# yahoo/TensorFlowOnSpark

Hardware: AMD Instinct MI355X
Metric: images/sec (whole node) ResNet-50 sync-SGD InputMode.SPARK (higher is better)
Workload: dtype bf16; 1 GPU; model=resnet50, global_batch=1024, per_gpu_batch=1024, parallelism=dp1

## Files before the change

csrc/bindings.cpp:

```cpp
#include <torch/extension.h>
#include <c10/hip/HIPStream.h>
#include <hip/hip_runtime.h>
#include <climits>

extern "C" {
int tfosr_bn_fast_blocks(long, int, int, int);
void tfosr_bn_apply_dual(const void*, const void*, void*, unsigned char*,
                         const float*, const float*, const float*, const float*,
                         const float*, const float*, const float*, const float*,
                         int, long, int, hipStream_t);
void tfosr_bn_bwd_stats_dual(const void*, const void*, const void*,
                             const unsigned char*, const float*, const float*,
                             const float*, const float*, float*, int, int, long,
                             int, hipStream_t);
void tfosr_bn_bwd_merge_dual(const float*, int, float*, float*, float*, float*,
                             int, hipStream_t);
void tfosr_bn_bwd_dx_dual(const void*, const void*, const void*,
                          const unsigned char*, void*, void*, const float*,
                          const float*, const float*, const float*, const float*,
                          const float*, const float*, const float*, const float*,
                          int, long, int, hipStream_t);
void tfosr_bn_stats(const void*, int, int, float*, int, int, int, long, hipStream_t);
void tfosr_bn_finalize(const float*, int, const void*, int, int, long,
                       float*, float*, float*, float*,
                       long, int, float, float, hipStream_t);
void tfosr_bn_apply(const void*, const void*, void*, unsigned char*,
                    const float*, const float*,
                    const float*, const float*, int, int, int, long, int, long,
                    hipStream_t);
void tfosr_bn_bwd_stats(const void*, const void*, const void*,
                        const unsigned char*, void*,
                        const float*, const float*, float*, int, int, int,
                        int, int, int, long, hipStream_t);
void tfosr_bn_bwd_merge(const float*, int, float*, float*, int, hipStream_t);
void tfosr_bn_bwd_dx(const void*, const void*, const void*,
                     const unsigned char*, const float*,
                     const float*, const float*, const float*, const float*,
                     void*, int, int, int, long, int, long, hipStream_t);
int tfosr_xent_dense_grid(int, int, long, long, int, int);
void tfosr_xent_dense_fwd(int, const void*, const long*, float*, float*, float*,
                          int*, int, long, long, int, long, float, int,
                          hipStream_t);
void tfosr_xent_dense_finalize(const float*, const int*, int, int, float*, int*,
                               hipStream_t);
void tfosr_xent_dense_bwd(int, const void*, const float*, const long*,
                          const float*, const float*, const int*, int, void*,
                          int, long, long, int, long, float, int, hipStream_t);
void tfosr_nhwc_pack(const void*, void*, const float*, const float*, float, int,
                     int, long, int, long, hipStream_t);
void tfosr_sgd_step(float*, const float*, float*, float, float, float, int, long,
                    hipStream_t);
void tfosr_adam_step(float*, const float*, float*, float*, float, float, float,
                     float, float, int, int, long, hipStream_t);
void tfosr_gemm_bt(const void*, const void*, void*, int, int, int, int,
                   hipStream_t);
void tfosr_gemm_bt_acc(const void*, const void*, void*, int, int, int, int,
                       int, hipStream_t);
void tfosr_mfma_probe(const short*, const short*, float*, hipStream_t);
void tfosr_maxpool_fwd(const void*, void*, unsigned char*, int, int, int, int,
                       int, int, int, int, int, int, hipStream_t);
void tfosr_maxpool_bwd(const void*, const unsigned char*, void*, int, int, int,
                       int, int, int, int, int, int, int, hipStream_t);
void tfosr_conv3x3(const void*, const void*, const void*, void*, int, int, int,
                   int, int, int, int, int, int, int, hipStream_t);
void tfosr_conv_mfma(const void*, const void*, const void*, void*, int, int,
                     int, int, int, int, int, int, int, int, int, int, int,
                     int, int, hipStream_t);
void tfosr_conv_wrw(const void*, const void*, float*, int, int, int, int, int,
                    int, int, int, int, int, hipStream_t);
int tfosr_wrw2_split(int, int, long);
void tfosr_conv_wrw2(const void*, const void*, const void*, float*, float*,
                     int, int, int, int, int, int, int, int, int, int, int,
                     int, int, hipStream_t);
void tfosr_conv_stem(const void*, const void*, const void*, void*, int, int,
                     int, int, int, int, hipStream_t);
void tfosr_conv_par(const void*, const void*, const void*, void*, int, int,
                    int, int, int, int, int, int, int, unsigned long, int,
                    int, int, long, int, hipStream_t);
void tfosr_pack_bf16(const void*, const void*, int, void*, long, hipStream_t);
}

namespace tfosr {
uint32_t crc32c(const uint8_t*, size_t, uint32_t);
struct ScanResult {
  std::string buffer;
  std::vector<std::pair<size_t, size_t>> records;
};
ScanResult scan_file(const std::string&, bool);
void write_file(const std::string&, const std::vector<std::string>&, bool);
}

namespace {

hipStream_t cur_stream() {
  return c10::hip::getCurrentHIPStream().stream();
}

struct BNLayout {
  bool nhwc;
  int N, C;
  long HW;
};

BNLayout bn_layout(const at::Tensor& x) {
  TORCH_CHECK(x.dim() == 4, "expected 4-D NCHW tensor");
  BNLayout l;
  l.N = x.size(0);
  l.C = x.size(1);
  l.HW = (long)x.size(2) * x.size(3);
  if (x.is_contiguous(at::MemoryFormat::ChannelsLast)) {
    l.nhwc = true;
  } else {
    TORCH_CHECK(x.is_contiguous(), "input must be contiguous (NCHW or channels_last)");
    l.nhwc = false;
  }
  return l;
}

int dtype_flag(const at::Tensor& x) {
  TORCH_CHECK(x.is_cuda(), "bn: input must be a GPU tensor");
  if (x.scalar_type() == at::kBFloat16) return 1;
  TORCH_CHECK(x.scalar_type() == at::kFloat, "expected float32 or bfloat16");
  return 0;
}


void bn_check_channel_vec(const at::Tensor& t, const at::Tensor& x, int C,
                          const char* name) {
  TORCH_CHECK(t.device() == x.device(), "bn: ", name, " must be on ", x.device(),
              ", got ", t.device());
  TORCH_CHECK(t.scalar_type() == at::kFloat, "bn: ", name, " must be float32");
  TORCH_CHECK(t.dim() == 1 && t.size(0) == C, "bn: ", name,
              " must have shape [", C, "]");
  TORCH_CHECK(t.is_contiguous(), "bn: ", name, " must be contiguous");
}

void bn_check_like(const at::Tensor& t, const at::Tensor& x, bool nhwc,
                   bool same_layout, const char* name) {
  TORCH_CHECK(t.device() == x.device(), "bn: ", name, " must be on ", x.device(),
              ", got ", t.device());
  TORCH_CHECK(t.scalar_type() == x.scalar_type(), "bn: ", name,
              " must have the input's dtype");
  TORCH_CHECK(t.sizes() == x.sizes(), "bn: ", name,
              " must have the input's shape");
  if (same_layout) {
    TORCH_CHECK(nhwc ? t.is_contiguous(at::MemoryFormat::ChannelsLast)
                     : t.is_contiguous(),
                "bn: ", name, " must have the input's memory layout");
  }
}

std::vector<at::Tensor> bn_fwd_train(at::Tensor x, c10::optional<at::Tensor> res,
                                     at::Tensor w, at::Tensor b, at::Tensor rm,
                                     at::Tensor rv, double momentum, double eps,
                                     bool relu) {
  auto l = bn_layout(x);
  int bf = dtype_flag(x);
  const void* res_ptr = nullptr;
  if (res.has_value()) {
    bn_check_like(*res, x, l.nhwc, true, "res");
    res_ptr = res->data_ptr();
  }
  bn_check_channel_vec(w, x, l.C, "weight");
  bn_check_channel_vec(b, x, l.C, "bias");
  bn_check_channel_vec(rm, x, l.C, "running_mean");
  bn_check_channel_vec(rv, x, l.C, "running_var");
  auto opts = x.options().dtype(at::kFloat);
  long M = (long)l.N * l.HW;
  int nb = tfosr_bn_fast_blocks(M * l.C, l.C, bf, l.nhwc);
  auto ws = nb > 0 ? at::empty({(long)nb * 2 * l.C}, opts)
                   : at::zeros({2L * l.C}, opts);
  auto save_mean = at::empty({l.C}, opts);
  auto save_rstd = at::empty({l.C}, opts);
  auto y = at::empty_like(x);
  at::Tensor mask;
  unsigned char* mask_ptr = nullptr;
  if (relu && nb > 0) {
    long nvec = M * l.C / (bf ? 8 : 4);
    mask = at::empty({nvec}, x.options().dtype(at::kByte));
    mask_ptr = mask.data_ptr<unsigned char>();
  } else {
    mask = at::empty({0}, x.options().dtype(at::kByte));
  }
  auto s = cur_stream();
  tfosr_bn_stats(x.data_ptr(), bf, l.nhwc, ws.data_ptr<float>(), nb,
                 l.N, l.C, l.HW, s);
  tfosr_bn_finalize(ws.data_ptr<float>(), nb, x.data_ptr(), bf, l.nhwc, l.HW,
                    save_mean.data_ptr<float>(), save_rstd.data_ptr<float>(),
                    rm.data_ptr<float>(), rv.data_ptr<float>(), M, l.C,
                    (float)momentum, (float)eps, s);
  tfosr_bn_apply(x.data_ptr(), res_ptr, y.data_ptr(), mask_ptr,
                 save_mean.data_ptr<float>(),
                 save_rstd.data_ptr<float>(), w.data_ptr<float>(),
                 b.data_ptr<float>(), bf, l.nhwc, relu, M * l.C, l.C, l.HW, s);
  return {y, save_mean, save_rstd, mask};
}

at::Tensor bn_fwd_eval(at::Tensor x, c10::optional<at::Tensor> res, at::Tensor w,
                       at::Tensor b, at::Tensor rm, at::Tensor rv, double eps,
                       bool relu) {
  auto l = bn_layout(x);
  int bf = dtype_flag(x);
  const void* res_ptr = nullptr;
  if (res.has_value()) {
    bn_check_like(*res, x, l.nhwc, true, "res");
    res_ptr = res->data_ptr();
  }
  bn_check_channel_vec(w, x, l.C, "weight");
  bn_check_channel_vec(b, x, l.C, "bias");
  bn_check_channel_vec(rm, x, l.C, "running_mean");
  bn_check_channel_vec(rv, x, l.C, "running_var");
  auto rstd = at::rsqrt(rv + eps);
  auto y = at::empty_like(x);
  tfosr_bn_apply(x.data_ptr(), res_ptr, y.data_ptr(), nullptr,
                 rm.data_ptr<float>(),
                 rstd.data_ptr<float>(), w.data_ptr<float>(), b.data_ptr<float>(),
                 bf, l.nhwc, relu, (long)l.N * l.HW * l.C, l.C, l.HW,
                 cur_stream());
  return y;
}

std::vector<at::Tensor> bn_bwd(at::Tensor x, at::Tensor dy, at::Tensor y,
                               at::Tensor mask, at::Tensor w,
                               at::Tensor save_mean,
                               at::Tensor save_rstd, bool relu, bool grad_res) {
  auto l = bn_layout(x);
  int bf = dtype_flag(x);
  bn_check_like(dy, x, l.nhwc, false, "dy");
  bn_check_like(y, x, l.nhwc, true, "y");
  bn_check_channel_vec(w, x, l.C, "weight");
  bn_check_channel_vec(save_mean, x, l.C, "save_mean");
  bn_check_channel_vec(save_rstd, x, l.C, "save_rstd");
  dy = l.nhwc ? dy.contiguous(at::MemoryFormat::ChannelsLast) : dy.contiguous();
  auto opts = x.options().dtype(at::kFloat);
  long total = (long)l.N * l.HW * l.C;
  int nb = tfosr_bn_fast_blocks(total, l.C, bf, l.nhwc);
  auto ws = nb > 0 ? at::empty({(long)nb * 2 * l.C}, opts)
                   : at::zeros({2L * l.C}, opts);
  auto dg = at::empty({l.C}, opts);
  auto db = at::empty({l.C}, opts);
  auto dx = at::empty_like(x);
  at::Tensor gout;
  void* gout_ptr = nullptr;
  if (grad_res) {
    gout = at::empty_like(x);
    gout_ptr = gout.data_ptr();
  }
  auto s = cur_stream();
  const unsigned char* mask_ptr =
      mask.numel() ? mask.data_ptr<unsigned char>() : nullptr;
  TORCH_CHECK(!(relu && nb > 0) || mask_ptr != nullptr,
              "fast-path relu backward requires the forward bitmask");
  if (relu && nb > 0) {
    TORCH_CHECK(mask.device() == x.device() && mask.scalar_type() == at::kByte &&
                    mask.is_contiguous() && mask.numel() == total / (bf ? 8 : 4),
                "bn: mask must be the contiguous uint8 bitmask bn_fwd_train "
                "returned for this input");
  }
  tfosr_bn_bwd_stats(x.data_ptr(), dy.data_ptr(), y.data_ptr(), mask_ptr,
                     gout_ptr,
                     save_mean.data_ptr<float>(), save_rstd.data_ptr<float>(),
                     ws.data_ptr<float>(), nb, bf, l.nhwc,
                     relu, l.N, l.C, l.HW, s);
  tfosr_bn_bwd_merge(ws.data_ptr<float>(), nb, dg.data_ptr<float>(),
                     db.data_ptr<float>(), l.C, s);
  if (grad_res) {
    tfosr_bn_bwd_dx(x.data_ptr(), gout.data_ptr(), y.data_ptr(), nullptr,
                    save_mean.data_ptr<float>(), save_rstd.data_ptr<float>(),
                    w.data_ptr<float>(), dg.data_ptr<float>(), db.data_ptr<float>(),
                    dx.data_ptr(), bf, l.nhwc, 0, total, l.C, l.HW, s);
    return {dx, dg, db, gout};
  }
  tfosr_bn_bwd_dx(x.data_ptr(), dy.data_ptr(), y.data_ptr(), mask_ptr,
                  save_mean.data_ptr<float>(), save_rstd.data_ptr<float>(),
                  w.data_ptr<float>(), dg.data_ptr<float>(), db.data_ptr<float>(),
                  dx.data_ptr(), bf, l.nhwc, relu, total, l.C, l.HW, s);
  return {dx, dg, db};
}

bool bn_dual_eligible(const at::Tensor& xa, const at::Tensor& xb) {
  if (!xa.is_cuda() || !xb.is_cuda() || xa.dim() != 4) return false;
  if (xa.scalar_type() != at::kBFloat16 && xa.scalar_type() != at::kFloat)
    return false;
  if (xb.scalar_type() != xa.scalar_type() || xb.device() != xa.device() ||
      xb.sizes() != xa.sizes())
    return false;
  if (!xa.is_contiguous(at::MemoryFormat::ChannelsLast) ||
      !xb.is_contiguous(at::MemoryFormat::ChannelsLast))
    return false;
  return tfosr_bn_fast_blocks(xa.numel(), (int)xa.size(1),
                              xa.scalar_type() == at::kBFloat16, 1) > 0;
}

std::vector<at::Tensor> bn_dual_fwd_train(
    at::Tensor xa, at::Tensor xb, at::Tensor w_a, at::Tensor b_a,
    at::Tensor rm_a, at::Tensor rv_a, at::Tensor w_b, at::Tensor b_b,
    at::Tensor rm_b, at::Tensor rv_b, double momentum, double eps) {
  TORCH_CHECK(bn_dual_eligible(xa, xb),
              "bn_dual: needs two same-shape channels_last GPU tensors on the "
              "NHWC fast path");
  auto l = bn_layout(xa);
  int bf = dtype_flag(xa);
  const at::Tensor* vecs[] = {&w_a, &b_a, &rm_a, &rv_a, &w_b, &b_b, &rm_b, &rv_b};
  for (auto* t : vecs) bn_check_channel_vec(*t, xa, l.C, "per-channel vector");
  auto opts = xa.options().dtype(at::kFloat);
  long M = (long)l.N * l.HW;
  long total = M * l.C;
  int nb = tfosr_bn_fast_blocks(total, l.C, bf, 1);
  auto ws = at::empty({(long)nb * 2 * l.C}, opts);
  auto mean_a = at::empty({l.C}, opts), rstd_a = at::empty({l.C}, opts);
  auto mean_b = at::empty({l.C}, opts), rstd_b = at::empty({l.C}, opts);
  auto y = at::empty_like(xa);
  auto mask = at::empty({total / (bf ? 8 : 4)}, xa.options().dtype(at::kByte));
  auto s = cur_stream();
  auto f = [](at::Tensor& t) { return t.data_ptr<float>(); };
  tfosr_bn_stats(xa.data_ptr(), bf, 1, f(ws), nb, l.N, l.C, l.HW, s);
  tfosr_bn_finalize(f(ws), nb, xa.data_ptr(), bf, 1, l.HW, f(mean_a), f(rstd_a),
                    f(rm_a), f(rv_a), M, l.C, (float)momentum, (float)eps, s);
  tfosr_bn_stats(xb.data_ptr(), bf, 1, f(ws), nb, l.N, l.C, l.HW, s);
  tfosr_bn_finalize(f(ws), nb, xb.data_ptr(), bf, 1, l.HW, f(mean_b), f(rstd_b),
                    f(rm_b), f(rv_b), M, l.C, (float)momentum, (float)eps, s);
  tfosr_bn_apply_dual(xa.data_ptr(), xb.data_ptr(), y.data_ptr(),
                      mask.data_ptr<unsigned char>(), f(mean_a), f(rstd_a),
                      f(w_a), f(b_a), f(mean_b), f(rstd_b), f(w_b), f(b_b), bf,
                      total, l.C, s);
  return {y, mean_a, rstd_a, mean_b, rstd_b, mask};
}

std::vector<at::Tensor> bn_dual_bwd(at::Tensor xa, at::Tensor xb, at::Tensor dy,
                                    at::Tensor mask, at::Tensor w_a,
                                    at::Tensor mean_a, at::Tensor rstd_a,
                                    at::Tensor w_b, at::Tensor mean_b,
                                    at::Tensor rstd_b) {
  TORCH_CHECK(bn_dual_eligible(xa, xb),
              "bn_dual: needs two same-shape channels_last GPU tensors on the "
              "NHWC fast path");
  auto l = bn_layout(xa);
  int bf = dtype_flag(xa);
  bn_check_like(dy, xa, true, false, "dy");
  dy = dy.contiguous(at::MemoryFormat::ChannelsLast);
  const at::Tensor* vecs[] = {&w_a, &mean_a, &rstd_a, &w_b, &mean_b, &rstd_b};
  for (auto* t : vecs) bn_check_channel_vec(*t, xa, l.C, "per-channel vector");
  long total = (long)l.N * l.HW * l.C;
  TORCH_CHECK(mask.device() == xa.device() && mask.scalar_type() == at::kByte &&
                  mask.is_contiguous() && mask.numel() == total / (bf ? 8 : 4),
              "bn_dual: mask must be the contiguous uint8 bitmask "
              "bn_dual_fwd_train returned for these inputs");
  auto opts = xa.options().dtype(at::kFloat);
  int nb = tfosr_bn_fast_blocks(total, l.C, bf, 1);
  auto ws = at::empty({(long)nb * 3 * l.C}, opts);
  auto dg_a = at::empty({l.C}, opts), dg_b = at::empty({l.C}, opts);
  auto db_a = at::empty({l.C}, opts), db_b = at::empty({l.C}, opts);
  auto dxa = at::empty_like(xa), dxb = at::empty_like(xb);
  auto s = cur_stream();
  auto f = [](at::Tensor& t) { return t.data_ptr<float>(); };
  const unsigned char* mask_ptr = mask.data_ptr<unsigned char>();
  tfosr_bn_bwd_stats_dual(xa.data_ptr(), xb.data_ptr(), dy.data_ptr(), mask_ptr,
                          f(mean_a), f(rstd_a), f(mean_b), f(rstd_b), f(ws), nb,
                          bf, total, l.C, s);
  tfosr_bn_bwd_merge_dual(f(ws), nb, f(dg_a), f(dg_b), f(db_a), f(db_b), l.C, s);
  tfosr_bn_bwd_dx_dual(xa.data_ptr(), xb.data_ptr(), dy.data_ptr(), mask_ptr,
                       dxa.data_ptr(), dxb.data_ptr(), f(mean_a), f(rstd_a),
                       f(w_a), f(dg_a), f(mean_b), f(rstd_b), f(w_b), f(dg_b),
                       f(db_a), bf, total, l.C, s);
  return {dxa, dxb, dg_a, dg_b, db_a, db_b};
}

void bn_stage(int family, at::Tensor x, c10::optional<at::Tensor> other,
              c10::optional<at::Tensor> out, c10::optional<at::Tensor> mask,
              at::Tensor ws, std::vector<at::Tensor> p, bool relu) {
  auto l = bn_layout(x);
  int bf = dtype_flag(x);
  long total = (long)l.N * l.HW * l.C;
  int nb = tfosr_bn_fast_blocks(total, l.C, bf, l.nhwc);
  TORCH_CHECK(nb > 0, "bn_stage: shape is not on the NHWC fast path");
  const size_t need[4] = {0, 4, 2, 5};
  TORCH_CHECK(family >= 0 && family < 4, "bn_stage: family must be 0..3");
  TORCH_CHECK(p.size() == need[family], "bn_stage: family ", family, " takes ",
              need[family], " per-channel vectors");
  for (auto& t : p) bn_check_channel_vec(t, x, l.C, "per-channel vector");
  TORCH_CHECK(ws.device() == x.device() && ws.scalar_type() == at::kFloat &&
                  ws.is_contiguous() && ws.numel() >= (long)nb * 2 * l.C,
              "bn_stage: ws must hold bn_fast_blocks() * 2C floats");
  const void* other_ptr = nullptr;
  if (other.has_value()) {
    bn_check_like(*other, x, l.nhwc, true, "other");
    other_ptr = other->data_ptr();
  }
  void* out_ptr = nullptr;
  if (out.has_value()) {
    bn_check_like(*out, x, l.nhwc, true, "out");
    out_ptr = out->data_ptr();
  }
  unsigned char* mask_ptr = nullptr;
  if (mask.has_value()) {
    TORCH_CHECK(mask->device() == x.device() && mask->scalar_type() == at::kByte &&
                    mask->is_contiguous() && mask->numel() == total / (bf ? 8 : 4),
                "bn_stage: mask must be a contiguous uint8 tensor, one byte "
                "per 16 B vector");
    mask_ptr = mask->data_ptr<unsigned char>();
  }
  if (family != 0 && family != 1)
    TORCH_CHECK(other_ptr != nullptr, "bn_stage: dy is required");
  if (family == 1 || family == 3)
    TORCH_CHECK(out_ptr != nullptr, "bn_stage: out is required");
  if (family >= 2)
    TORCH_CHECK(!relu || mask_ptr != nullptr, "bn_stage: relu needs the mask");
  auto f = [&](size_t i) { return p[i].data_ptr<float>(); };
  auto s = cur_stream();
  switch (family) {
    case 0:
      tfosr_bn_stats(x.data_ptr(), bf, 1, ws.data_ptr<float>(), nb, l.N, l.C,
                     l.HW, s);
      break;
    case 1:
      tfosr_bn_apply(x.data_ptr(), other_ptr, out_ptr, mask_ptr, f(0), f(1),
                     f(2), f(3), bf, 1, relu, total, l.C, l.HW, s);
      break;
    case 2:
      tfosr_bn_bwd_stats(x.data_ptr(), other_ptr, nullptr, mask_ptr, out_ptr,
                         f(0), f(1), ws.data_ptr<float>(), nb, bf, 1, relu,
                         l.N, l.C, l.HW, s);
      break;
    default:
      tfosr_bn_bwd_dx(x.data_ptr(), other_ptr, nullptr, mask_ptr, f(0), f(1),
                      f(2), f(3), f(4), out_ptr, bf, 1, relu, total, l.C, l.HW,
                      s);
  }
}


enum { XENT_ROWS = 0, XENT_STRIDED = 1, XENT_TILE = 2 };
enum { XENT_NONE = 0, XENT_SUM = 1, XENT_MEAN = 2 };

struct XentLayout {
  int family;
  long P, S;
  int C;
};

XentLayout xent_layout(const at::Tensor& logits, const at::Tensor& target) {
  TORCH_CHECK(logits.is_cuda(), "xent: logits must be a GPU tensor");
  TORCH_CHECK(logits.scalar_type() == at::kFloat ||
                  logits.scalar_type() == at::kBFloat16,
              "xent: logits must be float32 or bfloat16");
  TORCH_CHECK(logits.dim() >= 2, "xent: logits must be (P, C) or (N, C, d1, ...)");
  TORCH_CHECK(target.device() == logits.device(),
              "xent: target must be on ", logits.device());
  TORCH_CHECK(target.scalar_type() == at::kLong, "xent: target must be int64");
  TORCH_CHECK(target.is_contiguous(), "xent: target must be contiguous");
  TORCH_CHECK(target.dim() == logits.dim() - 1 &&
                  target.size(0) == logits.size(0),
              "xent: target must have the logits' shape without the class dim");
  for (int64_t d = 2; d < logits.dim(); ++d)
    TORCH_CHECK(target.size(d - 1) == logits.size(d),
                "xent: target must have the logits' shape without the class dim");
  TORCH_CHECK(logits.size(1) >= 1 && logits.size(1) < (1L << 24),
              "xent: bad class count");
  XentLayout l;
  l.C = (int)logits.size(1);
  l.P = target.numel();
  l.S = 1;
  bool rows;
  if (logits.dim() == 2) {
    TORCH_CHECK(logits.is_contiguous(), "xent: 2-D logits must be contiguous");
    rows = true;
  } else if (logits.is_contiguous()) {
    rows = false;
    for (int64_t d = 2; d < logits.dim(); ++d) l.S *= logits.size(d);
  } else {
    TORCH_CHECK(logits.dim() == 4 &&
                    logits.is_contiguous(at::MemoryFormat::ChannelsLast),
                "xent: N-D logits must be contiguous or 4-D channels_last");
    rows = true;
  }
  l.family = rows ? (l.C >= 64 ? XENT_ROWS : XENT_TILE) : XENT_STRIDED;
  return l;
}

void xent_check_rowvec(const at::Tensor& t, const at::Tensor& logits, long P,
                       const char* name) {
  TORCH_CHECK(t.device() == logits.device() && t.scalar_type() == at::kFloat &&
                  t.is_contiguous() && t.numel() == P,
              "xent: ", name, " must be contiguous float32 with one value per "
              "row, on the logits' device");
}

std::vector<at::Tensor> xent_dense_fwd(at::Tensor logits, at::Tensor target,
                                       long ignore_index, double label_smoothing,
                                       long reduction, long max_grid) {
  auto l = xent_layout(logits, target);
  TORCH_CHECK(reduction >= XENT_NONE && reduction <= XENT_MEAN,
              "xent: reduction must be 0 (none), 1 (sum) or 2 (mean)");
  TORCH_CHECK(label_smoothing >= 0.0 && label_smoothing <= 1.0,
              "xent: label_smoothing must be in [0, 1]");
  TORCH_CHECK(max_grid >= 0, "xent: max_grid must be >= 0");
  int bf = dtype_flag(logits);
  auto fopts = logits.options().dtype(at::kFloat);
  auto iopts = logits.options().dtype(at::kInt);
  auto lse = at::empty({l.P}, fopts);
  auto s = cur_stream();
  if (reduction == XENT_NONE) {
    auto loss = at::empty(target.sizes(), fopts);
    tfosr_xent_dense_fwd(l.family, logits.data_ptr(), target.data_ptr<long>(),
                         loss.data_ptr<float>(), lse.data_ptr<float>(), nullptr,
                         nullptr, bf, l.P, l.S, l.C, ignore_index,
                         (float)label_smoothing, (int)max_grid, s);
    return {loss, lse, at::empty({0}, iopts)};
  }
  auto loss = at::zeros({}, fopts);
  auto nvalid = at::zeros({1}, iopts);
  if (l.P > 0) {
    int nb = tfosr_xent_dense_grid(l.family, bf, l.P, l.S, l.C, (int)max_grid);
    auto part_loss = at::empty({2L * nb}, fopts);
    auto part_cnt = at::empty({nb}, iopts);
    tfosr_xent_dense_fwd(l.family, logits.data_ptr(), target.data_ptr<long>(),
                         nullptr, lse.data_ptr<float>(),
                         part_loss.data_ptr<float>(), part_cnt.data_ptr<int>(),
                         bf, l.P, l.S, l.C, ignore_index,
                         (float)label_smoothing, (int)max_grid, s);
    tfosr_xent_dense_finalize(part_loss.data_ptr<float>(),
                              part_cnt.data_ptr<int>(), nb,
                              reduction == XENT_MEAN, loss.data_ptr<float>(),
                              nvalid.data_ptr<int>(), s);
  }
  return {loss, lse, nvalid};
}

at::Tensor xent_dense_bwd(at::Tensor logits, at::Tensor lse, at::Tensor target,
                          at::Tensor gout, c10::optional<at::Tensor> nvalid,
                          long ignore_index, double label_smoothing,
                          long reduction, long max_grid) {
  auto l = xent_layout(logits, target);
  TORCH_CHECK(reduction >= XENT_NONE && reduction <= XENT_MEAN,
              "xent: reduction must be 0 (none), 1 (sum) or 2 (mean)");
  TORCH_CHECK(max_grid >= 0, "xent: max_grid must be >= 0");
  int bf = dtype_flag(logits);
  xent_check_rowvec(lse, logits, l.P, "lse");
  const float* grows = nullptr;
  const float* gscalar = nullptr;
  const int* nv = nullptr;
  if (reduction == XENT_NONE) {
    xent_check_rowvec(gout, logits, l.P, "gout");
    grows = gout.data_ptr<float>();
  } else {
    TORCH_CHECK(gout.device() == logits.device() &&
                    gout.scalar_type() == at::kFloat && gout.numel() == 1,
                "xent: gout must be a one-element float32 device tensor");
    TORCH_CHECK(nvalid.has_value() && nvalid->device() == logits.device() &&
                    nvalid->scalar_type() == at::kInt && nvalid->numel() == 1,
                "xent: n_valid must be the int32[1] tensor the forward returned");
    gscalar = gout.data_ptr<float>();
    nv = nvalid->data_ptr<int>();
  }
  auto dlogits = at::empty_like(logits);
  tfosr_xent_dense_bwd(l.family, logits.data_ptr(), lse.data_ptr<float>(),
                       target.data_ptr<long>(), grows, gscalar, nv,
                       reduction == XENT_MEAN, dlogits.data_ptr(), bf, l.P, l.S,
                       l.C, ignore_index, (float)label_smoothing, (int)max_grid,
                       cur_stream());
  return dlogits;
}

std::vector<at::Tensor> softmax_xent_fwd(at::Tensor logits, at::Tensor target) {
  TORCH_CHECK(logits.dim() == 2 && logits.is_contiguous());
  TORCH_CHECK(target.scalar_type() == at::kLong && target.is_cuda() &&
              target.is_contiguous() && target.numel() == logits.size(0));
  long N = logits.size(0);
  int C = logits.size(1);
  auto opts = logits.options().dtype(at::kFloat);
  auto loss = at::empty({N}, opts);
  auto lse = at::empty({N}, opts);
  tfosr_xent_dense_fwd(XENT_ROWS, logits.data_ptr(), target.data_ptr<long>(),
                       loss.data_ptr<float>(), lse.data_ptr<float>(), nullptr,
                       nullptr, dtype_flag(logits), N, 1, C, -100, 0.f, 0,
                       cur_stream());
  return {loss, lse};
}

at::Tensor softmax_xent_bwd(at::Tensor logits, at::Tensor lse, at::Tensor target,
                            at::Tensor gout) {
  TORCH_CHECK(logits.dim() == 2 && logits.is_contiguous());
  TORCH_CHECK(target.scalar_type() == at::kLong && target.is_cuda() &&
              target.is_contiguous() && target.numel() == logits.size(0));
  long N = logits.size(0);
  int C = logits.size(1);
  gout = gout.contiguous();
  xent_check_rowvec(lse, logits, N, "lse");
  xent_check_rowvec(gout, logits, N, "gout");
  auto dlogits = at::empty_like(logits);
  tfosr_xent_dense_bwd(XENT_ROWS, logits.data_ptr(), lse.data_ptr<float>(),
                       target.data_ptr<long>(), gout.data_ptr<float>(), nullptr,
                       nullptr, 0, dlogits.data_ptr(), dtype_flag(logits), N, 1,
                       C, -100, 0.f, 0, cur_stream());
  return dlogits;
}

at::Tensor nhwc_pack(at::Tensor x, at::Tensor mean, at::Tensor std_, double scale,
                     bool out_bf16, bool channels_last) {
  TORCH_CHECK(x.dim() == 4 && x.scalar_type() == at::kByte && x.is_contiguous(),
              "nhwc_pack expects contiguous uint8 NHWC");
  TORCH_CHECK(x.is_cuda(), "nhwc_pack: images must be on the GPU");
  for (int d = 0; d < 4; ++d)
    TORCH_CHECK(x.size(d) <= INT_MAX, "nhwc_pack: dimension ", d, " too large");
  int N = x.size(0), H = x.size(1), W = x.size(2), C = x.size(3);
  long HW = (long)H * W;
  auto check_stat = [&](const at::Tensor& t, const char* name) {
    TORCH_CHECK(t.scalar_type() == at::kFloat && t.is_contiguous() &&
                    t.device() == x.device() && t.numel() == C,
                "nhwc_pack: ", name, " must be a contiguous fp32 tensor of C = ",
                C, " elements on the images' device");
  };
  check_stat(mean, "mean");
  check_stat(std_, "std");
  auto opts = x.options().dtype(out_bf16 ? at::kBFloat16 : at::kFloat);
  at::Tensor out;
  if (channels_last) {
    out = at::empty({N, C, H, W}, opts, at::MemoryFormat::ChannelsLast);
  } else {
    out = at::empty({N, C, H, W}, opts);
  }
  tfosr_nhwc_pack(x.data_ptr(), out.data_ptr(), mean.data_ptr<float>(),
                  std_.data_ptr<float>(), (float)scale, out_bf16, channels_last,
                  (long)N * C * HW, C, HW, cur_stream());
  return out;
}

void check_flat_state(const char* op, const at::Tensor& p,
                      std::initializer_list<const at::Tensor*> others) {
  TORCH_CHECK(p.is_cuda() && p.scalar_type() == at::kFloat && p.is_contiguous(),
              op, " expects contiguous fp32 params on the GPU");
  for (const at::Tensor* t : others)
    TORCH_CHECK(t->scalar_type() == at::kFloat && t->is_contiguous() &&
                    t->device() == p.device() && t->numel() == p.numel(),
                op, ": every tensor must be contiguous fp32 with the params' ",
                p.numel(), " elements on the params' device");
}

std::pair<long, long> check_pool_geometry(const char* op, const at::Tensor& t,
                                          long C, long N, long H, long W,
                                          long K, long S, long P) {
  TORCH_CHECK(t.is_cuda(), op, " expects a GPU tensor");
  TORCH_CHECK(t.scalar_type() == at::kBFloat16 || t.scalar_type() == at::kFloat,
              op, " expects bf16 or fp32");
  const long V = t.scalar_type() == at::kBFloat16 ? 8 : 4;
  TORCH_CHECK(C >= V && C % V == 0, op, ": C must be a multiple of ", V,
              " for this dtype, got ", C);
  TORCH_CHECK(K >= 1 && S >= 1 && K * K <= 256, op,
              ": need K >= 1, S >= 1 and K*K <= 256 (the saved tap index is "
              "one byte), got K=", K, " S=", S);
  TORCH_CHECK(P >= 0 && P <= K / 2, op, ": need 0 <= P <= K/2, got P=", P);
  TORCH_CHECK(N >= 0 && H >= 1 && W >= 1 && H <= INT_MAX && W <= INT_MAX &&
              N <= INT_MAX && C <= INT_MAX && S <= INT_MAX,
              op, ": empty or oversized dimension");
  TORCH_CHECK(H + 2 * P >= K && W + 2 * P >= K, op,
              ": the window does not fit the padded input");
  const long OH = (H + 2 * P - K) / S + 1, OW = (W + 2 * P - K) / S + 1;
  const long limit = 0xFFFFFFFFL - 2048L * 256L;
  auto fits = [&](long h, long w) {
    long n = N;
    for (long f : {h, w, C / V}) {
      if (n > limit / f) return false;
      n *= f;
    }
    return true;
  };
  TORCH_CHECK(fits(H, W) && fits(OH, OW), op,
              ": tensor too large for the kernels' 32-bit thread index");
  return {OH, OW};
}

void sgd_step(at::Tensor p, at::Tensor g, at::Tensor m, double lr, double mu,
              double wd, bool nesterov) {
  check_flat_state("sgd_step", p, {&g, &m});
  tfosr_sgd_step(p.data_ptr<float>(), g.data_ptr<float>(), m.data_ptr<float>(),
                 (float)lr, (float)mu, (float)wd, nesterov, p.numel(),
                 cur_stream());
}

at::Tensor gemm_bt(at::Tensor a, at::Tensor b, bool out_bf16) {
  TORCH_CHECK(a.dim() == 2 && b.dim() == 2 && a.size(1) == b.size(1),
              "gemm_bt: A[M,K], B[N,K]");
  TORCH_CHECK(a.scalar_type() == at::kBFloat16 && b.scalar_type() == at::kBFloat16);
  int M = a.size(0), N = b.size(0), K = a.size(1);
  if (K % 32 != 0) {
    int Kp = (K + 31) / 32 * 32;
    auto ap = at::zeros({M, Kp}, a.options());
    auto bp = at::zeros({N, Kp}, b.options());
    ap.narrow(1, 0, K).copy_(a);
    bp.narrow(1, 0, K).copy_(b);
    a = ap; b = bp; K = Kp;
  }
  a = a.contiguous();
  b = b.contiguous();
  auto out = at::empty({M, N}, a.options().dtype(out_bf16 ? at::kBFloat16
                                                          : at::kFloat));
  tfosr_gemm_bt(a.data_ptr(), b.data_ptr(), out.data_ptr(), out_bf16, M, N, K,
                cur_stream());
  return out;
}

at::Tensor gemm_bf16(at::Tensor a, at::Tensor b) {
  return gemm_bt(a, b.t().contiguous(), false);
}

at::Tensor mfma_probe(at::Tensor a, at::Tensor b) {
  TORCH_CHECK(a.sizes() == at::IntArrayRef({64, 8}) &&
              b.sizes() == at::IntArrayRef({64, 8}));
  auto c = at::empty({64, 4}, a.options().dtype(at::kFloat));
  tfosr_mfma_probe(a.contiguous().data_ptr<short>(),
                   b.contiguous().data_ptr<short>(), c.data_ptr<float>(),
                   cur_stream());
  return c;
}

}

#define TFOSR_API_VERSION 6

static constexpr long kMaxTapReach = 1L << 20;

PYBIND11_MODULE(TORCH_EXTENSION_NAME, m) {
  m.def("api_version", []() { return TFOSR_API_VERSION; });
  m.def("bn_fwd_train", &bn_fwd_train);
  m.def("bn_fwd_eval", &bn_fwd_eval);
  m.def("bn_bwd", &bn_bwd);
  m.def("bn_dual_eligible", &bn_dual_eligible);
  m.def("bn_dual_fwd_train", &bn_dual_fwd_train);
  m.def("bn_dual_bwd", &bn_dual_bwd);
  m.def("bn_fast_blocks", [](long total, int C, bool bf16, bool nhwc) {
    return tfosr_bn_fast_blocks(total, C, bf16, nhwc);
  });
  m.def("bn_stage", &bn_stage);
  m.def("softmax_xent_fwd", &softmax_xent_fwd);
  m.def("softmax_xent_bwd", &softmax_xent_bwd);
  m.def("xent_dense_fwd", &xent_dense_fwd, py::arg("logits"), py::arg("target"),
        py::arg("ignore_index") = -100, py::arg("label_smoothing") = 0.0,
        py::arg("reduction") = 0, py::arg("max_grid") = 0);
  m.def("xent_dense_bwd", &xent_dense_bwd, py::arg("logits"), py::arg("lse"),
        py::arg("target"), py::arg("gout"), py::arg("nvalid") = py::none(),
        py::arg("ignore_index") = -100, py::arg("label_smoothing") = 0.0,
        py::arg("reduction") = 0, py::arg("max_grid") = 0);
  m.def("nhwc_pack", &nhwc_pack);
  m.def("sgd_step", &sgd_step);
  m.def("adam_step", [](at::Tensor p, at::Tensor g, at::Tensor m, at::Tensor v,
                        double lr, double b1, double b2, double eps, double wd,
                        long step, bool decoupled) {
    check_flat_state("adam_step", p, {&g, &m, &v});
    TORCH_CHECK(step >= 1 && step <= INT_MAX,
                "adam_step: step counts from 1, got ", step);
    tfosr_adam_step(p.data_ptr<float>(), g.data_ptr<float>(),
                    m.data_ptr<float>(), v.data_ptr<float>(), lr, b1, b2, eps,
                    wd, (int)step, decoupled, p.numel(), cur_stream());
  });
  m.def("gemm_bt", &gemm_bt, py::arg("a"), py::arg("b"), py::arg("out_bf16") = false);
  m.def("gemm_bf16", &gemm_bf16);
  m.def("mfma_probe", &mfma_probe);
  m.def("maxpool_fwd", [](at::Tensor x, long K, long S, long P) {
    TORCH_CHECK(x.dim() == 4 && x.is_contiguous(at::MemoryFormat::ChannelsLast),
                "maxpool_fwd expects channels_last");
    auto ohw = check_pool_geometry("maxpool_fwd", x, x.size(1), x.size(0),
                                   x.size(2), x.size(3), K, S, P);
    int N = x.size(0), C = x.size(1), H = x.size(2), W = x.size(3);
    int OH = (int)ohw.first, OW = (int)ohw.second;
    auto y = at::empty({N, C, OH, OW}, x.options(),
                       at::MemoryFormat::ChannelsLast);
    auto idx = at::empty({N, OH, OW, C}, x.options().dtype(at::kByte));
    tfosr_maxpool_fwd(x.data_ptr(), y.data_ptr(), idx.data_ptr<unsigned char>(),
                      x.scalar_type() == at::kBFloat16, N, C, H, W, OH, OW,
                      K, S, P, cur_stream());
    return std::vector<at::Tensor>{y, idx};
  });
  m.def("conv3x3_fwd", [](at::Tensor x, at::Tensor w9, long Cout, long S,
                          long P) {
    TORCH_CHECK(x.dim() == 4 && x.is_contiguous(at::MemoryFormat::ChannelsLast),
                "conv3x3_fwd expects channels_last input");
    TORCH_CHECK(x.scalar_type() == at::kBFloat16 &&
                w9.scalar_type() == at::kBFloat16);
    int N = x.size(0), Cin = x.size(1), H = x.size(2), W = x.size(3);
    TORCH_CHECK(Cin % 32 == 0, "conv3x3 requires Cin % 32 == 0");
    TORCH_CHECK(w9.size(1) == 9 * Cin);
    int OH = (H + 2 * P - 3) / S + 1, OW = (W + 2 * P - 3) / S + 1;
    auto y = at::empty({N, Cout, OH, OW}, x.options(),
                       at::MemoryFormat::ChannelsLast);
    auto guard = at::zeros({64}, x.options());
    tfosr_conv3x3(x.data_ptr(), w9.contiguous().data_ptr(), guard.data_ptr(),
                  y.data_ptr(), 1, N, H, W, Cin, Cout, OH, OW,
                  S, P, cur_stream());
    return y;
  });
  m.def("conv_mfma", [](at::Tensor x, at::Tensor wk, long Cout, long fh,
                        long fw, long S, long P, long D, long OH, long OW,
                        long fd, bool out_f32) {
    TORCH_CHECK(x.dim() == 4 && x.is_contiguous(at::MemoryFormat::ChannelsLast),
                "conv_mfma expects channels_last input");
    TORCH_CHECK(x.scalar_type() == at::kBFloat16 &&
                wk.scalar_type() == at::kBFloat16);
    TORCH_CHECK(fh >= 1 && fw >= 1 && fh * fw <= 49, "bad filter dims");
    TORCH_CHECK(D == 1 || D == 2, "input dilation must be 1 or 2");
    TORCH_CHECK(fd >= 1, "conv_mfma: filter dilation fd must be >= 1, got ",
                fd);
    TORCH_CHECK(fd == 1 || D == 1,
                "conv_mfma: filter dilation fd > 1 requires input dilation "
                "D == 1");
    TORCH_CHECK(fd <= kMaxTapReach && fd * (fh - 1) <= kMaxTapReach &&
                    fd * (fw - 1) <= kMaxTapReach,
                "conv_mfma: fd, fd*(fh-1) and fd*(fw-1) must be <= ",
                kMaxTapReach);
    long taps = fh * fw;
    int N = x.size(0), Cin = x.size(1), H = x.size(2), W = x.size(3);
    TORCH_CHECK(Cin % 32 == 0, "conv_mfma requires Cin % 32 == 0");
    TORCH_CHECK(wk.size(1) == taps * Cin);
    if (OH < 0) {
      long HV = (H - 1) * D + 1, WV = (W - 1) * D + 1;
      long nh = HV + 2 * P - fd * (fh - 1) - 1;
      long nw = WV + 2 * P - fd * (fw - 1) - 1;
      TORCH_CHECK(nh >= 0 && nw >= 0,
                  "conv_mfma: the dilated filter does not fit the padded "
                  "input");
      OH = nh / S + 1;
      OW = nw / S + 1;
    }
    auto y = at::empty({N, Cout, OH, OW},
                       x.options().dtype(out_f32 ? at::kFloat : at::kBFloat16),
                       at::MemoryFormat::ChannelsLast);
    auto guard = at::zeros({64}, x.options());
    tfosr_conv_mfma(x.data_ptr(), wk.contiguous().data_ptr(), guard.data_ptr(),
                    y.data_ptr(), out_f32 ? 0 : 1, N, H, W, Cin,
                    Cout, OH, OW, S, P, taps, fw, D, 0, (int)fd, cur_stream());
    return y;
  }, py::arg("x"), py::arg("wk"), py::arg("Cout"), py::arg("fh"),
     py::arg("fw"), py::arg("S"), py::arg("P"), py::arg("D"), py::arg("OH"),
     py::arg("OW"), py::arg("fd") = 1, py::arg("out_f32") = false);
  m.def("conv_mfma_acc", [](at::Tensor x, at::Tensor wk, at::Tensor out,
                            long fh, long fw, long S, long P, long D) {
    TORCH_CHECK(x.is_contiguous(at::MemoryFormat::ChannelsLast) &&
                out.is_contiguous(at::MemoryFormat::ChannelsLast));
    TORCH_CHECK(x.scalar_type() == at::kBFloat16 &&
                wk.scalar_type() == at::kBFloat16 &&
                out.scalar_type() == at::kBFloat16);
    int N = x.size(0), Cin = x.size(1), H = x.size(2), W = x.size(3);
    TORCH_CHECK(Cin % 32 == 0, "conv_mfma requires Cin % 32 == 0");
    long taps = fh * fw;
    TORCH_CHECK(wk.size(1) == taps * Cin);
    long Cout = out.size(1), OH = out.size(2), OW = out.size(3);
    TORCH_CHECK(out.size(0) == N);
    auto guard = at::zeros({64}, x.options());
    tfosr_conv_mfma(x.data_ptr(), wk.contiguous().data_ptr(), guard.data_ptr(),
                    out.data_ptr(), 1, N, H, W, Cin, Cout, OH, OW,
                    S, P, taps, fw, D, 1, 1, cur_stream());
    return out;
  });
  m.def("gemm_bt_acc", [](at::Tensor a, at::Tensor b, at::Tensor c) {
    TORCH_CHECK(a.dim() == 2 && b.dim() == 2 && c.dim() == 2,
                "gemm_bt_acc: A[M,K], B[N,K], C[M,N] must be 2-D");
    TORCH_CHECK(a.is_cuda(), "gemm_bt_acc: a must be a GPU tensor");
    TORCH_CHECK(b.device() == a.device() && c.device() == a.device(),
                "gemm_bt_acc: b and c must be on ", a.device());
    TORCH_CHECK(a.is_contiguous() && b.is_contiguous() && c.is_contiguous(),
                "gemm_bt_acc: a, b and c must be contiguous");
    TORCH_CHECK(a.scalar_type() == at::kBFloat16 &&
                    b.scalar_type() == at::kBFloat16 &&
                    c.scalar_type() == at::kBFloat16,
                "gemm_bt_acc: a, b and c must be bfloat16");
    long M = a.size(0), K = a.size(1), Nn = b.size(0);
    TORCH_CHECK(b.size(1) == K && c.size(0) == M && c.size(1) == Nn,
                "gemm_bt_acc: A[M,K], B[N,K], C[M,N]");
    TORCH_CHECK(K % 32 == 0, "gemm_bt_acc: K must be a multiple of 32");
    tfosr_gemm_bt_acc(a.data_ptr(), b.data_ptr(), c.data_ptr(),
                      1, M, Nn, K, 1, cur_stream());
    return c;
  });
  m.def("conv_wrw2", [](at::Tensor dy, at::Tensor x, long R, long S_f,
                        long stride, long P, long fd) {
    TORCH_CHECK(dy.is_contiguous(at::MemoryFormat::ChannelsLast) &&
                x.is_contiguous(at::MemoryFormat::ChannelsLast));
    TORCH_CHECK(dy.scalar_type() == at::kBFloat16 &&
                x.scalar_type() == at::kBFloat16);
    int N = x.size(0), Cin = x.size(1), H = x.size(2), W = x.size(3);
    int Cout = dy.size(1), OH = dy.size(2), OW = dy.size(3);
    TORCH_CHECK(Cin % 8 == 0 && Cout % 8 == 0,
                "conv_wrw2 needs channel counts % 8 == 0");
    long taps = R * S_f;
    TORCH_CHECK(taps == 1 || taps == 9, "conv_wrw2 supports 1x1 and 3x3");
    TORCH_CHECK(fd >= 1, "conv_wrw2: filter dilation fd must be >= 1, got ",
                fd);
    TORCH_CHECK(taps != 1 || fd == 1,
                "conv_wrw2: a 1x1 filter has no dilation, fd must be 1");
    TORCH_CHECK(fd <= kMaxTapReach && fd * (R - 1) <= kMaxTapReach &&
                    fd * (S_f - 1) <= kMaxTapReach,
                "conv_wrw2: fd, fd*(R-1) and fd*(S_f-1) must be <= ",
                kMaxTapReach);
    long M = (long)N * OH * OW;
    int split = tfosr_wrw2_split(Cout, Cin, M);
    long K = taps * (long)Cin;
    auto ws = at::empty({(long)split, (long)Cout * K},
                        x.options().dtype(at::kFloat));
    auto dW = at::empty({(long)Cout, K}, x.options().dtype(at::kFloat));
    auto guard = at::zeros({64}, x.options());
    tfosr_conv_wrw2(dy.data_ptr(), x.data_ptr(), guard.data_ptr(),
                    ws.data_ptr<float>(), dW.data_ptr<float>(), N, H, W, Cin,
                    Cout, OH, OW, R, S_f, stride, P, split, (int)fd,
                    cur_stream());
    return dW;
  }, py::arg("dy"), py::arg("x"), py::arg("R"), py::arg("S_f"),
     py::arg("stride"), py::arg("P"), py::arg("fd") = 1);
  m.def("pack_bf16", [](at::Tensor descs, at::Tensor cum, long ndesc,
                        at::Tensor arena, long total) {
    TORCH_CHECK(descs.is_cuda() && cum.is_cuda() && arena.is_cuda() &&
                    descs.device() == arena.device() &&
                    cum.device() == arena.device(),
                "pack_bf16 expects descs, cum and arena on one GPU");
    TORCH_CHECK(arena.scalar_type() == at::kBFloat16 && arena.is_contiguous(),
                "pack_bf16 expects a contiguous bf16 arena");
    TORCH_CHECK(ndesc >= 0 && ndesc <= INT_MAX, "pack_bf16: bad ndesc ", ndesc);
    TORCH_CHECK(descs.scalar_type() == at::kByte && descs.is_contiguous() &&
                    descs.numel() == ndesc * 80,
                "pack_bf16: descs must hold ndesc * 80 contiguous bytes");
    TORCH_CHECK(cum.scalar_type() == at::kLong && cum.is_contiguous() &&
                    cum.numel() == ndesc + 1,
                "pack_bf16: cum must hold ndesc + 1 contiguous int64");
    TORCH_CHECK(total >= 0 && arena.numel() >= total,
                "pack_bf16: arena holds ", arena.numel(), " elements, total is ",
                total);
    if (total == 0) return;
    TORCH_CHECK(ndesc >= 1, "pack_bf16: no descriptor for ", total, " elements");
    tfosr_pack_bf16(descs.data_ptr(), cum.data_ptr(), (int)ndesc,
                    arena.data_ptr(), total, cur_stream());
  });
  m.def("conv_par", [](at::Tensor x, at::Tensor wk, at::Tensor out,
                       std::vector<long> taps_r, std::vector<long> taps_s,
                       long P, bool accum) {
    TORCH_CHECK(x.is_contiguous(at::MemoryFormat::ChannelsLast) &&
                out.is_contiguous(at::MemoryFormat::ChannelsLast));
    TORCH_CHECK(x.scalar_type() == at::kBFloat16 &&
                wk.scalar_type() == at::kBFloat16 &&
                out.scalar_type() == at::kBFloat16);
    int N = x.size(0), Cin = x.size(1), H = x.size(2), W = x.size(3);
    TORCH_CHECK(Cin % 32 == 0);
    long ntaps = (long)taps_r.size();
    TORCH_CHECK(ntaps >= 1 && ntaps <= 8 && taps_s.size() == (size_t)ntaps);
    TORCH_CHECK(wk.size(1) == ntaps * Cin);
    long Cout = out.size(1), OHr = out.size(2), OWr = out.size(3);
    long oh0 = ((P - taps_r[0]) % 2 + 2) % 2;
    long ow0 = ((P - taps_s[0]) % 2 + 2) % 2;
    long OHs = (OHr - oh0 + 1) / 2, OWs = (OWr - ow0 + 1) / 2;
    if (OHs <= 0 || OWs <= 0) return out;
    unsigned long pack = 0;
    for (long i = 0; i < ntaps; ++i)
      pack |= ((unsigned long)((taps_r[i] << 4) | taps_s[i])) << (i * 8);
    auto guard = at::zeros({64}, x.options());
    tfosr_conv_par(x.data_ptr(), wk.contiguous().data_ptr(), guard.data_ptr(),
                   out.data_ptr(), N, H, W, Cin, (int)Cout, (int)OHs,
                   (int)OWs, (int)P, (int)ntaps, pack, (int)oh0, (int)ow0,
                   (int)OWr, OHr * OWr, accum ? 1 : 0, cur_stream());
    return out;
  });
  m.def("conv_stem", [](at::Tensor x4, at::Tensor w224, long Cout) {
    TORCH_CHECK(x4.is_contiguous(at::MemoryFormat::ChannelsLast) &&
                x4.size(1) == 4, "conv_stem expects NHWC4 padded input");
    TORCH_CHECK(x4.scalar_type() == at::kBFloat16 &&
                w224.scalar_type() == at::kBFloat16);
    TORCH_CHECK(w224.size(1) == 224);
    int N = x4.size(0), Hp = x4.size(2), Wp = x4.size(3);
    int OH = (Hp - 7) / 2 + 1, OW = (Wp - 7) / 2 + 1;
    auto y = at::empty({N, Cout, OH, OW}, x4.options(),
                       at::MemoryFormat::ChannelsLast);
    auto guard = at::zeros({64}, x4.options());
    tfosr_conv_stem(x4.data_ptr(), w224.contiguous().data_ptr(),
                    guard.data_ptr(), y.data_ptr(), N, Hp, Wp, Cout, OH, OW,
                    cur_stream());
    return y;
  });
  m.def("conv_stem_wrw", [](at::Tensor dy, at::Tensor x4) {
    TORCH_CHECK(dy.is_contiguous(at::MemoryFormat::ChannelsLast) &&
                x4.is_contiguous(at::MemoryFormat::ChannelsLast));
    TORCH_CHECK(dy.scalar_type() == at::kBFloat16 &&
                x4.scalar_type() == at::kBFloat16 && x4.size(1) == 4);
    int N = x4.size(0), Hp = x4.size(2), Wp = x4.size(3);
    int Cout = dy.size(1), OH = dy.size(2), OW = dy.size(3);
    long M = (long)N * OH * OW;
    int split = tfosr_wrw2_split(Cout, 32, M);
    long K = 7L * 32;
    auto ws = at::empty({(long)split, (long)Cout * K},
                        x4.options().dtype(at::kFloat));
    auto dW = at::empty({(long)Cout, K}, x4.options().dtype(at::kFloat));
    auto guard = at::zeros({64}, x4.options());
    tfosr_conv_wrw2(dy.data_ptr(), x4.data_ptr(), guard.data_ptr(),
                    ws.data_ptr<float>(), dW.data_ptr<float>(), N, Hp, Wp,
                    32, Cout, OH, OW, 7, 1,
                    2, 0, split, 1, cur_stream());
    return dW;
  });
  m.def("conv_wrw", [](at::Tensor dy, at::Tensor x, long R, long S, long P) {
    TORCH_CHECK(dy.is_contiguous(at::MemoryFormat::ChannelsLast) &&
                x.is_contiguous(at::MemoryFormat::ChannelsLast));
    TORCH_CHECK(dy.scalar_type() == at::kBFloat16 &&
                x.scalar_type() == at::kBFloat16);
    int N = x.size(0), Cin = x.size(1), H = x.size(2), W = x.size(3);
    int Cout = dy.size(1), OH = dy.size(2), OW = dy.size(3);
    auto dW = at::zeros({Cout, R * S * (long)Cin},
                        x.options().dtype(at::kFloat));
    tfosr_conv_wrw(dy.data_ptr(), x.data_ptr(), dW.data_ptr<float>(), N, H, W,
                   Cin, Cout, OH, OW, R, S, P, cur_stream());
    return dW;
  });
  m.def("maxpool_bwd", [](at::Tensor dy, at::Tensor idx, long H, long W,
                          long K, long S, long P) {
    TORCH_CHECK(dy.dim() == 4, "maxpool_bwd expects a 4-D gradient");
    auto ohw = check_pool_geometry("maxpool_bwd", dy, dy.size(1), dy.size(0),
                                   H, W, K, S, P);
    TORCH_CHECK(dy.size(2) == ohw.first && dy.size(3) == ohw.second,
                "maxpool_bwd: a ", H, "x", W, " input pooled with K=", K,
                " S=", S, " P=", P, " gives ", ohw.first, "x", ohw.second,
                ", the gradient is ", dy.size(2), "x", dy.size(3));
    TORCH_CHECK(idx.scalar_type() == at::kByte && idx.is_contiguous() &&
                    idx.device() == dy.device() && idx.dim() == 4 &&
                    idx.size(0) == dy.size(0) && idx.size(1) == dy.size(2) &&
                    idx.size(2) == dy.size(3) && idx.size(3) == dy.size(1),
                "maxpool_bwd: idx must be the contiguous uint8 (N, OH, OW, C) "
                "tensor maxpool_fwd returned, on the gradient's device");
    dy = dy.contiguous(at::MemoryFormat::ChannelsLast);
    int N = dy.size(0), C = dy.size(1), OH = dy.size(2), OW = dy.size(3);
    auto dx = at::empty({N, C, H, W}, dy.options(),
                        at::MemoryFormat::ChannelsLast);
    tfosr_maxpool_bwd(dy.data_ptr(), idx.data_ptr<unsigned char>(),
                      dx.data_ptr(), dy.scalar_type() == at::kBFloat16,
                      N, C, H, W, OH, OW, K, S, P, cur_stream());
    return dx;
  });

  m.def("crc32c", [](py::bytes data) {
    std::string s = data;
    return tfosr::crc32c((const uint8_t*)s.data(), s.size(), 0);
  });
  m.def("tfrecord_read_file", [](const std::string& path, bool verify) {
    auto res = tfosr::scan_file(path, verify);
    py::list out;
    for (auto& [off, len] : res.records)
      out.append(py::bytes(res.buffer.data() + off, len));
    return out;
  }, py::arg("path"), py::arg("verify") = false);
  m.def("tfrecord_write_file",
        [](const std::string& path, const std::vector<std::string>& recs,
           bool append) { tfosr::write_file(path, recs, append); },
        py::arg("path"), py::arg("records"), py::arg("append") = false);
}
```

csrc/bn_relu.hip:

```cpp
#include "tfosr_common.h"

typedef unsigned int u32;


template <typename T>
struct VecIO;

template <>
struct VecIO<bf16_t> {
  static constexpr int V = 8;
  using vec_t = s8v;
  __device__ static void load(const bf16_t* p, float* out) {
    vec_t v = *(const vec_t*)p;
    #pragma unroll
    for (int j = 0; j < 8; ++j) {
      union { short s; bf16_t b; } u;
      u.s = v[j];
      out[j] = (float)u.b;
    }
  }
  __device__ static void store(bf16_t* p, const float* in) {
    vec_t v;
    #pragma unroll
    for (int j = 0; j < 8; ++j) {
      union { short s; bf16_t b; } u;
      u.b = (bf16_t)in[j];
      v[j] = u.s;
    }
    *(vec_t*)p = v;
  }
};

template <>
struct VecIO<float> {
  static constexpr int V = 4;
  using vec_t = f4v;
  __device__ static void load(const float* p, float* out) {
    f4v v = *(const f4v*)p;
    #pragma unroll
    for (int j = 0; j < 4; ++j) out[j] = v[j];
  }
  __device__ static void store(float* p, const float* in) {
    f4v v;
    #pragma unroll
    for (int j = 0; j < 4; ++j) v[j] = in[j];
    *(f4v*)p = v;
  }
};


template <int V>
__device__ __forceinline__ u32 channel_slot(u32 C) {
  return ((blockIdx.x * blockDim.x + threadIdx.x) * (u32)V) % C;
}

#define TFOSR_BN_SHIFT_PIXELS 32

template <typename T>
__device__ __forceinline__ float channel_shift(const T* __restrict__ x, int c,
                                               int C, long HW, bool nhwc,
                                               int n) {
  float s = 0.f;
  for (int m = 0; m < n; ++m)
    s += (float)x[nhwc ? (long)m * C + c : ((m / HW) * C + c) * HW + m % HW];
  return s / (float)n;
}

template <typename T>
__global__ void stats_nhwc_fast(const T* __restrict__ x,
                                float* __restrict__ partials, u32 nvec, u32 C) {
  extern __shared__ float lds[];
  constexpr int V = VecIO<T>::V;
  const u32 c0 = channel_slot<V>(C);
  for (u32 i = threadIdx.x; i < 2 * C; i += blockDim.x) lds[i] = 0.f;
  __syncthreads();
  float s[V], q[V], v[V], k[V];
  VecIO<T>::load(x + c0, k);
  #pragma unroll
  for (int j = 0; j < V; ++j) { s[j] = 0.f; q[j] = 0.f; }
  const u32 stride = gridDim.x * blockDim.x;
  for (u32 i = blockIdx.x * blockDim.x + threadIdx.x; i < nvec; i += stride) {
    VecIO<T>::load(x + (size_t)i * V, v);
    #pragma unroll
    for (int j = 0; j < V; ++j) { float d = v[j] - k[j]; s[j] += d; q[j] += d * d; }
  }
  #pragma unroll
  for (int j = 0; j < V; ++j) {
    atomicAdd(&lds[c0 + j], s[j]);
    atomicAdd(&lds[C + c0 + j], q[j]);
  }
  __syncthreads();
  float* out = partials + (size_t)blockIdx.x * 2 * C;
  for (u32 i = threadIdx.x; i < 2 * C; i += blockDim.x) out[i] = lds[i];
}

__global__ void stats_merge_finalize(const float* __restrict__ partials,
                                     int nblocks, u32 C,
                                     const void* __restrict__ x, int is_bf16,
                                     int is_nhwc, long HW, int nshift,
                                     float* __restrict__ save_mean,
                                     float* __restrict__ save_rstd,
                                     float* __restrict__ running_mean,
                                     float* __restrict__ running_var,
                                     long M, float momentum, float eps) {
  __shared__ float scratch[8];
  const u32 c = blockIdx.x;
  float s = 0.f, q = 0.f;
  for (int b = threadIdx.x; b < nblocks; b += blockDim.x) {
    s += partials[(size_t)b * 2 * C + c];
    q += partials[(size_t)b * 2 * C + C + c];
  }
  s = block_sum<256>(s, scratch);
  __syncthreads();
  q = block_sum<256>(q, scratch);
  if (threadIdx.x != 0) return;
  const float shift =
      is_bf16 ? channel_shift((const bf16_t*)x, (int)c, (int)C, HW, is_nhwc, nshift)
              : channel_shift((const float*)x, (int)c, (int)C, HW, is_nhwc, nshift);
  float dmean = s / (float)M;
  float var = fmaxf(q / (float)M - dmean * dmean, 0.f);
  float mean = shift + dmean;
  save_mean[c] = mean;
  save_rstd[c] = rsqrtf(var + eps);
  if (running_mean != nullptr) {
    float unbiased = (M > 1) ? var * (float)M / (float)(M - 1) : var;
    running_mean[c] = (1.f - momentum) * running_mean[c] + momentum * mean;
    running_var[c] = (1.f - momentum) * running_var[c] + momentum * unbiased;
  }
}

template <typename T, bool RELU, bool ADD>
__global__ void bn_apply_fast(const T* __restrict__ x, const T* __restrict__ res,
                              T* __restrict__ y, unsigned char* __restrict__ mask,
                              const float* __restrict__ mean,
                              const float* __restrict__ rstd,
                              const float* __restrict__ w,
                              const float* __restrict__ b, u32 nvec, u32 C) {
  constexpr int V = VecIO<T>::V;
  const u32 c0 = channel_slot<V>(C);
  float sc[V], mu[V], sh[V], v[V], r[V];
  #pragma unroll
  for (int j = 0; j < V; ++j) {
    sc[j] = w[c0 + j] * rstd[c0 + j];
    mu[j] = mean[c0 + j];
    sh[j] = b[c0 + j];
  }
  const u32 stride = gridDim.x * blockDim.x;
  for (u32 i = blockIdx.x * blockDim.x + threadIdx.x; i < nvec; i += stride) {
    VecIO<T>::load(x + (size_t)i * V, v);
    if (ADD) VecIO<T>::load(res + (size_t)i * V, r);
    unsigned char m = 0;
    #pragma unroll
    for (int j = 0; j < V; ++j) {
      float o = (v[j] - mu[j]) * sc[j] + sh[j];
      if (ADD) o += r[j];
      if (RELU) {
        if (o > 0.f) m |= (1u << j);
        o = fmaxf(o, 0.f);
      }
      v[j] = o;
    }
    VecIO<T>::store(y + (size_t)i * V, v);
    if (RELU && mask != nullptr) mask[i] = m;
  }
}

template <typename T, bool RELU, bool WRITE_G>
__global__ void bwd_stats_fast(const T* __restrict__ x, const T* __restrict__ dy,
                               const unsigned char* __restrict__ mask,
                               T* __restrict__ gout,
                               const float* __restrict__ mean,
                               const float* __restrict__ rstd,
                               float* __restrict__ partials, u32 nvec, u32 C) {
  extern __shared__ float lds[];
  constexpr int V = VecIO<T>::V;
  const u32 c0 = channel_slot<V>(C);
  for (u32 i = threadIdx.x; i < 2 * C; i += blockDim.x) lds[i] = 0.f;
  __syncthreads();
  float sg[V], sb[V], xv[V], dv[V];
  float mu[V], rs[V];
  #pragma unroll
  for (int j = 0; j < V; ++j) {
    sg[j] = 0.f; sb[j] = 0.f;
    mu[j] = mean[c0 + j]; rs[j] = rstd[c0 + j];
  }
  const u32 stride = gridDim.x * blockDim.x;
  for (u32 i = blockIdx.x * blockDim.x + threadIdx.x; i < nvec; i += stride) {
    VecIO<T>::load(x + (size_t)i * V, xv);
    VecIO<T>::load(dy + (size_t)i * V, dv);
    unsigned char m = RELU ? mask[i] : 0;
    #pragma unroll
    for (int j = 0; j < V; ++j) {
      float g = RELU ? (((m >> j) & 1) ? dv[j] : 0.f) : dv[j];
      sb[j] += g;
      sg[j] += g * (xv[j] - mu[j]) * rs[j];
      dv[j] = g;
    }
    if (WRITE_G) VecIO<T>::store(gout + (size_t)i * V, dv);
  }
  #pragma unroll
  for (int j = 0; j < V; ++j) {
    atomicAdd(&lds[c0 + j], sg[j]);
    atomicAdd(&lds[C + c0 + j], sb[j]);
  }
  __syncthreads();
  float* out = partials + (size_t)blockIdx.x * 2 * C;
  for (u32 i = threadIdx.x; i < 2 * C; i += blockDim.x) out[i] = lds[i];
}

__global__ void bwd_stats_merge(const float* __restrict__ partials, int nblocks,
                                u32 C, float* __restrict__ dg,
                                float* __restrict__ db) {
  __shared__ float scratch[8];
  const u32 c = blockIdx.x;
  float sg = 0.f, sb = 0.f;
  for (int b = threadIdx.x; b < nblocks; b += blockDim.x) {
    sg += partials[(size_t)b * 2 * C + c];
    sb += partials[(size_t)b * 2 * C + C + c];
  }
  sg = block_sum<256>(sg, scratch);
  __syncthreads();
  sb = block_sum<256>(sb, scratch);
  if (threadIdx.x == 0) {
    dg[c] = sg;
    db[c] = sb;
  }
}

template <typename T, bool RELU>
__global__ void bwd_dx_fast(const T* __restrict__ x, const T* __restrict__ dy,
                            const unsigned char* __restrict__ mask,
                            T* __restrict__ dx,
                            const float* __restrict__ mean,
                            const float* __restrict__ rstd,
                            const float* __restrict__ w,
                            const float* __restrict__ dg,
                            const float* __restrict__ db,
                            u32 nvec, u32 C, float invM) {
  constexpr int V = VecIO<T>::V;
  const u32 c0 = channel_slot<V>(C);
  float sc[V], mu[V], rs[V], dgm[V], dbm[V], xv[V], dv[V];
  #pragma unroll
  for (int j = 0; j < V; ++j) {
    mu[j] = mean[c0 + j]; rs[j] = rstd[c0 + j];
    sc[j] = w[c0 + j] * rs[j];
    dgm[j] = dg[c0 + j] * invM;
    dbm[j] = db[c0 + j] * invM;
  }
  const u32 stride = gridDim.x * blockDim.x;
  for (u32 i = blockIdx.x * blockDim.x + threadIdx.x; i < nvec; i += stride) {
    VecIO<T>::load(x + (size_t)i * V, xv);
    VecIO<T>::load(dy + (size_t)i * V, dv);
    unsigned char m = RELU ? mask[i] : 0;
    #pragma unroll
    for (int j = 0; j < V; ++j) {
      float g = RELU ? (((m >> j) & 1) ? dv[j] : 0.f) : dv[j];
      float xhat = (xv[j] - mu[j]) * rs[j];
      dv[j] = sc[j] * (g - dbm[j] - xhat * dgm[j]);
    }
    VecIO<T>::store(dx + (size_t)i * V, dv);
  }
}


template <typename T>
__global__ void bn_apply_dual_fast(const T* __restrict__ xa,
                                   const T* __restrict__ xb, T* __restrict__ y,
                                   unsigned char* __restrict__ mask,
                                   const float* __restrict__ mean_a,
                                   const float* __restrict__ rstd_a,
                                   const float* __restrict__ w_a,
                                   const float* __restrict__ b_a,
                                   const float* __restrict__ mean_b,
                                   const float* __restrict__ rstd_b,
                                   const float* __restrict__ w_b,
                                   const float* __restrict__ b_b,
                                   u32 nvec, u32 C) {
  constexpr int V = VecIO<T>::V;
  const u32 c0 = channel_slot<V>(C);
  float sca[V], mua[V], sha[V], scb[V], mub[V], shb[V], va[V], vb[V];
  #pragma unroll
  for (int j = 0; j < V; ++j) {
    sca[j] = w_a[c0 + j] * rstd_a[c0 + j];
    mua[j] = mean_a[c0 + j];
    sha[j] = b_a[c0 + j];
    scb[j] = w_b[c0 + j] * rstd_b[c0 + j];
    mub[j] = mean_b[c0 + j];
    shb[j] = b_b[c0 + j];
  }
  const u32 stride = gridDim.x * blockDim.x;
  for (u32 i = blockIdx.x * blockDim.x + threadIdx.x; i < nvec; i += stride) {
    VecIO<T>::load(xa + (size_t)i * V, va);
    VecIO<T>::load(xb + (size_t)i * V, vb);
    unsigned char m = 0;
    #pragma unroll
    for (int j = 0; j < V; ++j) {
      float o = (va[j] - mua[j]) * sca[j] + sha[j];
      o += (vb[j] - mub[j]) * scb[j] + shb[j];
      if (o > 0.f) m |= (1u << j);
      va[j] = fmaxf(o, 0.f);
    }
    VecIO<T>::store(y + (size_t)i * V, va);
    mask[i] = m;
  }
}

template <typename T>
__global__ void bwd_stats_dual_fast(const T* __restrict__ xa,
                                    const T* __restrict__ xb,
                                    const T* __restrict__ dy,
                                    const unsigned char* __restrict__ mask,
                                    const float* __restrict__ mean_a,
                                    const float* __restrict__ rstd_a,
                                    const float* __restrict__ mean_b,
                                    const float* __restrict__ rstd_b,
                                    float* __restrict__ partials, u32 nvec,
                                    u32 C) {
  extern __shared__ float lds[];
  constexpr int V = VecIO<T>::V;
  const u32 c0 = channel_slot<V>(C);
  for (u32 i = threadIdx.x; i < 3 * C; i += blockDim.x) lds[i] = 0.f;
  __syncthreads();
  float sga[V], sgb[V], sb[V], av[V], bv[V], dv[V];
  float mua[V], rsa[V], mub[V], rsb[V];
  #pragma unroll
  for (int j = 0; j < V; ++j) {
    sga[j] = 0.f; sgb[j] = 0.f; sb[j] = 0.f;
    mua[j] = mean_a[c0 + j]; rsa[j] = rstd_a[c0 + j];
    mub[j] = mean_b[c0 + j]; rsb[j] = rstd_b[c0 + j];
  }
  const u32 stride = gridDim.x * blockDim.x;
  for (u32 i = blockIdx.x * blockDim.x + threadIdx.x; i < nvec; i += stride) {
    VecIO<T>::load(xa + (size_t)i * V, av);
    VecIO<T>::load(xb + (size_t)i * V, bv);
    VecIO<T>::load(dy + (size_t)i * V, dv);
    unsigned char m = mask[i];
    #pragma unroll
    for (int j = 0; j < V; ++j) {
      float g = ((m >> j) & 1) ? dv[j] : 0.f;
      sb[j] += g;
      sga[j] += g * (av[j] - mua[j]) * rsa[j];
      sgb[j] += g * (bv[j] - mub[j]) * rsb[j];
    }
  }
  #pragma unroll
  for (int j = 0; j < V; ++j) {
    atomicAdd(&lds[c0 + j], sga[j]);
    atomicAdd(&lds[C + c0 + j], sgb[j]);
    atomicAdd(&lds[2 * C + c0 + j], sb[j]);
  }
  __syncthreads();
  float* out = partials + (size_t)blockIdx.x * 3 * C;
  for (u32 i = threadIdx.x; i < 3 * C; i += blockDim.x) out[i] = lds[i];
}

__global__ void bwd_stats_dual_merge(const float* __restrict__ partials,
                                     int nblocks, u32 C,
                                     float* __restrict__ dg_a,
                                     float* __restrict__ dg_b,
                                     float* __restrict__ db_a,
                                     float* __restrict__ db_b) {
  __shared__ float scratch[8];
  const u32 c = blockIdx.x;
  float sa = 0.f, sg = 0.f, sb = 0.f;
  for (int b = threadIdx.x; b < nblocks; b += blockDim.x) {
    sa += partials[(size_t)b * 3 * C + c];
    sg += partials[(size_t)b * 3 * C + C + c];
    sb += partials[(size_t)b * 3 * C + 2 * C + c];
  }
  sa = block_sum<256>(sa, scratch);
  __syncthreads();
  sg = block_sum<256>(sg, scratch);
  __syncthreads();
  sb = block_sum<256>(sb, scratch);
  if (threadIdx.x == 0) {
    dg_a[c] = sa;
    dg_b[c] = sg;
    db_a[c] = sb;
    db_b[c] = sb;
  }
}

template <typename T>
__global__ void bwd_dx_dual_fast(const T* __restrict__ xa,
                                 const T* __restrict__ xb,
                                 const T* __restrict__ dy,
                                 const unsigned char* __restrict__ mask,
                                 T* __restrict__ dxa, T* __restrict__ dxb,
                                 const float* __restrict__ mean_a,
                                 const float* __restrict__ rstd_a,
                                 const float* __restrict__ w_a,
                                 const float* __restrict__ dg_a,
                                 const float* __restrict__ mean_b,
                                 const float* __restrict__ rstd_b,
                                 const float* __restrict__ w_b,
                                 const float* __restrict__ dg_b,
                                 const float* __restrict__ db,
                                 u32 nvec, u32 C, float invM) {
  constexpr int V = VecIO<T>::V;
  const u32 c0 = channel_slot<V>(C);
  float sca[V], mua[V], rsa[V], dga[V], scb[V], mub[V], rsb[V], dgb[V], dbm[V];
  float av[V], bv[V], dv[V];
  #pragma unroll
  for (int j = 0; j < V; ++j) {
    mua[j] = mean_a[c0 + j]; rsa[j] = rstd_a[c0 + j];
    sca[j] = w_a[c0 + j] * rsa[j];
    dga[j] = dg_a[c0 + j] * invM;
    mub[j] = mean_b[c0 + j]; rsb[j] = rstd_b[c0 + j];
    scb[j] = w_b[c0 + j] * rsb[j];
    dgb[j] = dg_b[c0 + j] * invM;
    dbm[j] = db[c0 + j] * invM;
  }
  const u32 stride = gridDim.x * blockDim.x;
  for (u32 i = blockIdx.x * blockDim.x + threadIdx.x; i < nvec; i += stride) {
    VecIO<T>::load(xa + (size_t)i * V, av);
    VecIO<T>::load(xb + (size_t)i * V, bv);
    VecIO<T>::load(dy + (size_t)i * V, dv);
    unsigned char m = mask[i];
    #pragma unroll
    for (int j = 0; j < V; ++j) {
      float g = ((m >> j) & 1) ? dv[j] : 0.f;
      float xhat_a = (av[j] - mua[j]) * rsa[j];
      float xhat_b = (bv[j] - mub[j]) * rsb[j];
      av[j] = sca[j] * (g - dbm[j] - xhat_a * dga[j]);
      bv[j] = scb[j] * (g - dbm[j] - xhat_b * dgb[j]);
    }
    VecIO<T>::store(dxa + (size_t)i * V, av);
    VecIO<T>::store(dxb + (size_t)i * V, bv);
  }
}


#define TFOSR_BN_CHUNK 4096

template <bool NHWC>
__device__ __forceinline__ long pixel_index(long m, int c, int C, long HW) {
  return NHWC ? m * C + c : ((m / HW) * C + c) * HW + m % HW;
}

static inline dim3 generic_red_grid(long M, int C) {
  long chunks = (M + TFOSR_BN_CHUNK - 1) / TFOSR_BN_CHUNK;
  if (chunks > 1024) chunks = 1024;
  return dim3((unsigned)C, (unsigned)(chunks > 0 ? chunks : 1));
}

template <typename T, bool NHWC>
__global__ void stats_generic(const T* __restrict__ x, float* __restrict__ ws,
                              long M, int C, long HW) {
  __shared__ float scratch[8];
  __shared__ float shift;
  const int c = blockIdx.x;
  if (threadIdx.x == 0)
    shift = channel_shift(x, c, C, HW, NHWC,
                          M < TFOSR_BN_SHIFT_PIXELS ? (int)M : TFOSR_BN_SHIFT_PIXELS);
  __syncthreads();
  const float k = shift;
  float s = 0.f, q = 0.f;
  for (long m0 = (long)blockIdx.y * TFOSR_BN_CHUNK; m0 < M;
       m0 += (long)gridDim.y * TFOSR_BN_CHUNK) {
    const long m1 = m0 + TFOSR_BN_CHUNK < M ? m0 + TFOSR_BN_CHUNK : M;
    for (long m = m0 + threadIdx.x; m < m1; m += blockDim.x) {
      float d = (float)x[pixel_index<NHWC>(m, c, C, HW)] - k;
      s += d;
      q += d * d;
    }
  }
  s = block_sum<256>(s, scratch);
  __syncthreads();
  q = block_sum<256>(q, scratch);
  if (threadIdx.x == 0) {
    atomicAdd(&ws[c], s);
    atomicAdd(&ws[C + c], q);
  }
}

template <typename T, bool NHWC, bool RELU, bool ADD>
__global__ void bn_apply_generic(const T* __restrict__ x, const T* __restrict__ res,
                                 T* __restrict__ y,
                                 const float* __restrict__ mean,
                                 const float* __restrict__ rstd,
                                 const float* __restrict__ w,
                                 const float* __restrict__ b,
                                 long total, int C, long HW) {
  for (long idx = blockIdx.x * (long)blockDim.x + threadIdx.x; idx < total;
       idx += (long)gridDim.x * blockDim.x) {
    int c = NHWC ? (int)(idx % C) : (int)((idx / HW) % C);
    float o = ((float)x[idx] - mean[c]) * rstd[c] * w[c] + b[c];
    if (ADD) o += (float)res[idx];
    if (RELU) o = fmaxf(o, 0.f);
    y[idx] = (T)o;
  }
}

template <typename T, bool NHWC, bool RELU, bool WRITE_G>
__global__ void bwd_stats_generic(const T* __restrict__ x, const T* __restrict__ dy,
                                  const T* __restrict__ y, T* __restrict__ gout,
                                  const float* __restrict__ mean,
                                  const float* __restrict__ rstd,
                                  float* __restrict__ ws,
                                  long M, int C, long HW) {
  __shared__ float scratch[8];
  const int c = blockIdx.x;
  const float mu = mean[c], rs = rstd[c];
  float sg = 0.f, sb = 0.f;
  for (long m0 = (long)blockIdx.y * TFOSR_BN_CHUNK; m0 < M;
       m0 += (long)gridDim.y * TFOSR_BN_CHUNK) {
    const long m1 = m0 + TFOSR_BN_CHUNK < M ? m0 + TFOSR_BN_CHUNK : M;
    for (long m = m0 + threadIdx.x; m < m1; m += blockDim.x) {
      const long idx = pixel_index<NHWC>(m, c, C, HW);
      float g = (float)dy[idx];
      if (RELU) g = ((float)y[idx] > 0.f) ? g : 0.f;
      sb += g;
      sg += g * ((float)x[idx] - mu) * rs;
      if (WRITE_G) gout[idx] = (T)g;
    }
  }
  sg = block_sum<256>(sg, scratch);
  __syncthreads();
  sb = block_sum<256>(sb, scratch);
  if (threadIdx.x == 0) {
    atomicAdd(&ws[c], sg);
    atomicAdd(&ws[C + c], sb);
  }
}

template <typename T, bool NHWC, bool RELU>
__global__ void bwd_dx_generic(const T* __restrict__ x, const T* __restrict__ dy,
                               const T* __restrict__ y, T* __restrict__ dx,
                               const float* __restrict__ mean,
                               const float* __restrict__ rstd,
                               const float* __restrict__ w,
                               const float* __restrict__ dg,
                               const float* __restrict__ db,
                               long total, int C, long HW, float invM) {
  for (long idx = blockIdx.x * (long)blockDim.x + threadIdx.x; idx < total;
       idx += (long)gridDim.x * blockDim.x) {
    int c = NHWC ? (int)(idx % C) : (int)((idx / HW) % C);
    float g = (float)dy[idx];
    if (RELU) g = ((float)y[idx] > 0.f) ? g : 0.f;
    float xhat = ((float)x[idx] - mean[c]) * rstd[c];
    dx[idx] = (T)(w[c] * rstd[c] * (g - db[c] * invM - xhat * dg[c] * invM));
  }
}



static inline bool fast_ok(int is_nhwc, long total, int C, int vec) {
  return is_nhwc && total < (1L << 31) && C % vec == 0 && 2048 % C == 0;
}

static inline int grid_quantum(int C, int vec) {
  int row = 256 * vec;
  return C > row ? C / row : 1;
}

static inline int fast_grid(long nvec, int quantum) {
  long g = (nvec + 255) / 256;
  g = (g + quantum - 1) / quantum * quantum;
  if (g > TFOSR_MAX_GRID) g = TFOSR_MAX_GRID;
  return (int)(g > 0 ? g : quantum);
}

static inline int red_grid(long nvec, int quantum) {
  long g = nvec / (256 * 32);
  if (g < 64) g = 64;
  if (g > 1024) g = 1024;
  g -= g % quantum;
  return (int)g;
}

extern "C" {

int tfosr_bn_fast_blocks(long total, int C, int is_bf16, int is_nhwc) {
  int vec = is_bf16 ? 8 : 4;
  if (!fast_ok(is_nhwc, total, C, vec)) return 0;
  return red_grid(total / vec, grid_quantum(C, vec));
}

void tfosr_bn_stats(const void* x, int is_bf16, int is_nhwc, float* partials,
                    int nb, int N, int C, long HW, hipStream_t s) {
  const long total = (long)N * HW * C;
  if (nb > 0) {
    int vec = is_bf16 ? 8 : 4;
    u32 nvec = (u32)(total / vec);
    size_t lds = 2 * (size_t)C * sizeof(float);
    if (is_bf16)
      hipLaunchKernelGGL(stats_nhwc_fast<bf16_t>, dim3(nb), dim3(256), lds, s,
                         (const bf16_t*)x, partials, nvec, (u32)C);
    else
      hipLaunchKernelGGL(stats_nhwc_fast<float>, dim3(nb), dim3(256), lds, s,
                         (const float*)x, partials, nvec, (u32)C);
    return;
  }
  const long M = (long)N * HW;
  dim3 grid = generic_red_grid(M, C);
#define SG(T, L) hipLaunchKernelGGL((stats_generic<T, L>), grid, dim3(256), \
                                    0, s, (const T*)x, partials, M, C, HW)
  if (is_bf16) { if (is_nhwc) SG(bf16_t, true); else SG(bf16_t, false); }
  else { if (is_nhwc) SG(float, true); else SG(float, false); }
#undef SG
}

void tfosr_bn_finalize(const float* partials, int nb, const void* x,
                       int is_bf16, int is_nhwc, long HW, float* save_mean,
                       float* save_rstd, float* running_mean, float* running_var,
                       long M, int C, float momentum, float eps, hipStream_t s) {
  hipLaunchKernelGGL(stats_merge_finalize, dim3(C), dim3(256), 0, s,
                     partials, nb > 0 ? nb : 1, (u32)C, x, is_bf16, is_nhwc, HW,
                     nb > 0 ? 1 : (int)(M < TFOSR_BN_SHIFT_PIXELS ? M : TFOSR_BN_SHIFT_PIXELS),
                     save_mean, save_rstd,
                     running_mean, running_var, M, momentum, eps);
}

void tfosr_bn_apply(const void* x, const void* res, void* y, unsigned char* mask,
                    const float* mean,
                    const float* rstd, const float* w, const float* b,
                    int is_bf16, int is_nhwc, int relu, long total, int C,
                    long HW, hipStream_t s) {
  int vec = is_bf16 ? 8 : 4;
  const bool add = res != nullptr;
  if (fast_ok(is_nhwc, total, C, vec)) {
    u32 nvec = (u32)(total / vec);
    int grid = fast_grid(nvec, grid_quantum(C, vec));
#define APPLY_FAST(T, R, A) \
    hipLaunchKernelGGL((bn_apply_fast<T, R, A>), dim3(grid), dim3(256), 0, s, \
                       (const T*)x, (const T*)res, (T*)y, mask, mean, rstd, w, b, \
                       nvec, (u32)C)
    if (is_bf16) {
      if (relu) { if (add) APPLY_FAST(bf16_t, true, true); else APPLY_FAST(bf16_t, true, false); }
      else      { if (add) APPLY_FAST(bf16_t, false, true); else APPLY_FAST(bf16_t, false, false); }
    } else {
      if (relu) { if (add) APPLY_FAST(float, true, true); else APPLY_FAST(float, true, false); }
      else      { if (add) APPLY_FAST(float, false, true); else APPLY_FAST(float, false, false); }
    }
#undef APPLY_FAST
    return;
  }
  int grid = tfosr_grid(total, 256);
#define APPLY_GEN(T, L, R, A) \
  hipLaunchKernelGGL((bn_apply_generic<T, L, R, A>), dim3(grid), dim3(256), 0, s, \
                     (const T*)x, (const T*)res, (T*)y, mean, rstd, w, b, \
                     total, C, HW)
  if (is_bf16) {
    if (is_nhwc) { if (relu) { if (add) APPLY_GEN(bf16_t, true, true, true); else APPLY_GEN(bf16_t, true, true, false); }
                   else { if (add) APPLY_GEN(bf16_t, true, false, true); else APPLY_GEN(bf16_t, true, false, false); } }
    else { if (relu) { if (add) APPLY_GEN(bf16_t, false, true, true); else APPLY_GEN(bf16_t, false, true, false); }
           else { if (add) APPLY_GEN(bf16_t, false, false, true); else APPLY_GEN(bf16_t, false, false, false); } }
  } else {
    if (is_nhwc) { if (relu) { if (add) APPLY_GEN(float, true, true, true); else APPLY_GEN(float, true, true, false); }
                   else { if (add) APPLY_GEN(float, true, false, true); else APPLY_GEN(float, true, false, false); } }
    else { if (relu) { if (add) APPLY_GEN(float, false, true, true); else APPLY_GEN(float, false, true, false); }
           else { if (add) APPLY_GEN(float, false, false, true); else APPLY_GEN(float, false, false, false); } }
  }
#undef APPLY_GEN
}

void tfosr_bn_bwd_stats(const void* x, const void* dy, const void* y,
                        const unsigned char* mask, void* gout,
                        const float* mean, const float* rstd, float* partials,
                        int nb, int is_bf16, int is_nhwc, int relu, int N, int C,
                        long HW, hipStream_t s) {
  const long total = (long)N * HW * C;
  const bool wg = gout != nullptr;
  if (nb > 0) {
    int vec = is_bf16 ? 8 : 4;
    u32 nvec = (u32)(total / vec);
    size_t lds = 2 * (size_t)C * sizeof(float);
#define BS_FAST(T, R, W) \
    hipLaunchKernelGGL((bwd_stats_fast<T, R, W>), dim3(nb), dim3(256), lds, s, \
                       (const T*)x, (const T*)dy, mask, (T*)gout, \
                       mean, rstd, partials, nvec, (u32)C)
    if (is_bf16) {
      if (relu) { if (wg) BS_FAST(bf16_t, true, true); else BS_FAST(bf16_t, true, false); }
      else      { if (wg) BS_FAST(bf16_t, false, true); else BS_FAST(bf16_t, false, false); }
    } else {
      if (relu) { if (wg) BS_FAST(float, true, true); else BS_FAST(float, true, false); }
      else      { if (wg) BS_FAST(float, false, true); else BS_FAST(float, false, false); }
    }
#undef BS_FAST
    return;
  }
  const long M = (long)N * HW;
  dim3 grid = generic_red_grid(M, C);
#define BS_GEN(T, L, R, W) \
  hipLaunchKernelGGL((bwd_stats_generic<T, L, R, W>), grid, dim3(256), 0, s, \
                     (const T*)x, (const T*)dy, (const T*)y, (T*)gout, \
                     mean, rstd, partials, M, C, HW)
  if (is_bf16) {
    if (is_nhwc) { if (relu) { if (wg) BS_GEN(bf16_t, true, true, true); else BS_GEN(bf16_t, true, true, false); }
                   else { if (wg) BS_GEN(bf16_t, true, false, true); else BS_GEN(bf16_t, true, false, false); } }
    else { if (relu) { if (wg) BS_GEN(bf16_t, false, true, true); else BS_GEN(bf16_t, false, true, false); }
           else { if (wg) BS_GEN(bf16_t, false, false, true); else BS_GEN(bf16_t, false, false, false); } }
  } else {
    if (is_nhwc) { if (relu) { if (wg) BS_GEN(float, true, true, true); else BS_GEN(float, true, true, false); }
                   else { if (wg) BS_GEN(float, true, false, true); else BS_GEN(float, true, false, false); } }
    else { if (relu) { if (wg) BS_GEN(float, false, true, true); else BS_GEN(float, false, true, false); }
           else { if (wg) BS_GEN(float, false, false, true); else BS_GEN(float, false, false, false); } }
  }
#undef BS_GEN
}

void tfosr_bn_bwd_merge(const float* partials, int nb, float* dg, float* db,
                        int C, hipStream_t s) {
  hipLaunchKernelGGL(bwd_stats_merge, dim3(C), dim3(256), 0, s,
                     partials, nb > 0 ? nb : 1, (u32)C, dg, db);
}

void tfosr_bn_bwd_dx(const void* x, const void* dy, const void* y,
                     const unsigned char* mask,
                     const float* mean, const float* rstd, const float* w,
                     const float* dg, const float* db, void* dx, int is_bf16,
                     int is_nhwc, int relu, long total, int C, long HW,
                     hipStream_t s) {
  const float invM = 1.f / (float)(total / C);
  int vec = is_bf16 ? 8 : 4;
  if (fast_ok(is_nhwc, total, C, vec)) {
    u32 nvec = (u32)(total / vec);
    int grid = fast_grid(nvec, grid_quantum(C, vec));
#define DX_FAST(T, R) \
    hipLaunchKernelGGL((bwd_dx_fast<T, R>), dim3(grid), dim3(256), 0, s, \
                       (const T*)x, (const T*)dy, mask, (T*)dx, \
                       mean, rstd, w, dg, db, nvec, (u32)C, invM)
    if (is_bf16) { if (relu) DX_FAST(bf16_t, true); else DX_FAST(bf16_t, false); }
    else { if (relu) DX_FAST(float, true); else DX_FAST(float, false); }
#undef DX_FAST
    return;
  }
  int grid = tfosr_grid(total, 256);
#define DX_GEN(T, L, R) \
  hipLaunchKernelGGL((bwd_dx_generic<T, L, R>), dim3(grid), dim3(256), 0, s, \
                     (const T*)x, (const T*)dy, (const T*)y, (T*)dx, \
                     mean, rstd, w, dg, db, total, C, HW, invM)
  if (is_bf16) {
    if (is_nhwc) { if (relu) DX_GEN(bf16_t, true, true); else DX_GEN(bf16_t, true, false); }
    else { if (relu) DX_GEN(bf16_t, false, true); else DX_GEN(bf16_t, false, false); }
  } else {
    if (is_nhwc) { if (relu) DX_GEN(float, true, true); else DX_GEN(float, true, false); }
    else { if (relu) DX_GEN(float, false, true); else DX_GEN(float, false, false); }
  }
#undef DX_GEN
}


void tfosr_bn_apply_dual(const void* xa, const void* xb, void* y,
                         unsigned char* mask, const float* mean_a,
                         const float* rstd_a, const float* w_a,
                         const float* b_a, const float* mean_b,
                         const float* rstd_b, const float* w_b,
                         const float* b_b, int is_bf16, long total, int C,
                         hipStream_t s) {
  int vec = is_bf16 ? 8 : 4;
  u32 nvec = (u32)(total / vec);
  int grid = fast_grid(nvec, grid_quantum(C, vec));
#define APPLY_DUAL(T) \
  hipLaunchKernelGGL((bn_apply_dual_fast<T>), dim3(grid), dim3(256), 0, s, \
                     (const T*)xa, (const T*)xb, (T*)y, mask, mean_a, rstd_a, \
                     w_a, b_a, mean_b, rstd_b, w_b, b_b, nvec, (u32)C)
  if (is_bf16) APPLY_DUAL(bf16_t); else APPLY_DUAL(float);
#undef APPLY_DUAL
}

void tfosr_bn_bwd_stats_dual(const void* xa, const void* xb, const void* dy,
                             const unsigned char* mask, const float* mean_a,
                             const float* rstd_a, const float* mean_b,
                             const float* rstd_b, float* partials, int nb,
                             int is_bf16, long total, int C, hipStream_t s) {
  int vec = is_bf16 ? 8 : 4;
  u32 nvec = (u32)(total / vec);
  size_t lds = 3 * (size_t)C * sizeof(float);
#define BS_DUAL(T) \
  hipLaunchKernelGGL((bwd_stats_dual_fast<T>), dim3(nb), dim3(256), lds, s, \
                     (const T*)xa, (const T*)xb, (const T*)dy, mask, mean_a, \
                     rstd_a, mean_b, rstd_b, partials, nvec, (u32)C)
  if (is_bf16) BS_DUAL(bf16_t); else BS_DUAL(float);
#undef BS_DUAL
}

void tfosr_bn_bwd_merge_dual(const float* partials, int nb, float* dg_a,
                             float* dg_b, float* db_a, float* db_b, int C,
                             hipStream_t s) {
  hipLaunchKernelGGL(bwd_stats_dual_merge, dim3(C), dim3(256), 0, s,
                     partials, nb, (u32)C, dg_a, dg_b, db_a, db_b);
}

void tfosr_bn_bwd_dx_dual(const void* xa, const void* xb, const void* dy,
                          const unsigned char* mask, void* dxa, void* dxb,
                          const float* mean_a, const float* rstd_a,
                          const float* w_a, const float* dg_a,
                          const float* mean_b, const float* rstd_b,
                          const float* w_b, const float* dg_b, const float* db,
                          int is_bf16, long total, int C, hipStream_t s) {
  const float invM = 1.f / (float)(total / C);
  int vec = is_bf16 ? 8 : 4;
  u32 nvec = (u32)(total / vec);
  int grid = fast_grid(nvec, grid_quantum(C, vec));
#define DX_DUAL(T) \
  hipLaunchKernelGGL((bwd_dx_dual_fast<T>), dim3(grid), dim3(256), 0, s, \
                     (const T*)xa, (const T*)xb, (const T*)dy, mask, (T*)dxa, \
                     (T*)dxb, mean_a, rstd_a, w_a, dg_a, mean_b, rstd_b, w_b, \
                     dg_b, db, nvec, (u32)C, invM)
  if (is_bf16) DX_DUAL(bf16_t); else DX_DUAL(float);
#undef DX_DUAL
}

}
```

csrc/conv3x3_mfma.hip:

```cpp
#include "tfosr_common.h"

typedef short bf16x8 __attribute__((ext_vector_type(8)));
typedef float f32x4 __attribute__((ext_vector_type(4)));

#define C3_BK 32
#define C3_SWZ(l) ((l) ^ ((((l) >> 7) & 7) << 4))

__device__ __forceinline__ void c3_stage16(const char* src,
                                           __attribute__((address_space(3))) char* dst) {
  __builtin_amdgcn_global_load_lds(
      (const __attribute__((address_space(1))) void*)src,
      (__attribute__((address_space(3))) void*)dst, 16, 0, 0);
}

template <typename OT, int WRG, int WCG, int MI, int D = 1, bool ACC = false,
          bool PAR = false>
__global__ __launch_bounds__(512, 1) void conv3x3_kernel(
    const bf16_t* __restrict__ X, const bf16_t* __restrict__ W9,
    const bf16_t* __restrict__ guard, OT* __restrict__ C,
    int Nn, int H, int Wd, int Cin, int Cout, int OH, int OW, int S, int P,
    int taps, int fw, int pixst, unsigned long tap_pack, int oh0, int ow0,
    int OWr, long OHOWr, int fd) {
  constexpr int BM = WRG * MI * 16;
  constexpr int BN = WCG * 64;
  constexpr int ABYTES = BM * C3_BK * 2;
  constexpr int BBYTES = BN * C3_BK * 2;
  constexpr int ACHUNK = ABYTES / 16 / 512;
  constexpr int BCHUNK = BBYTES / 16 / 512;
  constexpr int SLOT = ABYTES + BBYTES;
  __shared__ char lds[4 * SLOT];
  __attribute__((address_space(3))) char* lds3 =
      (__attribute__((address_space(3))) char*)lds;

  const int K = taps * Cin;
  const long M = (long)Nn * OH * OW;
  const int ntn = (Cout + BN - 1) / BN;
  const int nwg = gridDim.x;
  int wgid = blockIdx.x;
  {
    const int q = nwg / 8, r = nwg % 8;
    const int xcd = wgid % 8, pos = wgid / 8;
    wgid = (xcd < r ? xcd * (q + 1) : r * (q + 1) + (xcd - r) * q) + pos;
  }
  const long tile_m = (long)(wgid / ntn) * BM;
  const long tile_n = (long)(wgid % ntn) * BN;

  const int t = threadIdx.x;
  const int lane = t & 63;
  const int wave = t >> 6;
  const int wr = wave / WCG, wc = wave % WCG;

  int a_ohS[ACHUNK], a_owS[ACHUNK];
  long a_pix[ACHUNK];
  int a_col[ACHUNK];
  long a_n[ACHUNK];
  #pragma unroll
  for (int u = 0; u < ACHUNK; ++u) {
    int d = (t + u * 512) * 16;
    int sl = C3_SWZ(d);
    long row = sl >> 6;
    long m = tile_m + row;
    bool ok = m < M;
    if (!ok) m = 0;
    long n = m / ((long)OH * OW);
    long rem = m - n * (long)OH * OW;
    int oh = (int)(rem / OW), ow = (int)(rem - (long)(rem / OW) * OW);
    a_n[u] = ok ? n : -1;
    a_ohS[u] = (PAR ? oh * 2 + oh0 : oh) * S - P;
    a_owS[u] = (PAR ? ow * 2 + ow0 : ow) * S - P;
    a_pix[u] = n * (long)H * Wd;
    a_col[u] = sl & 63;
  }
  long srcB[BCHUNK];
  const long Kb = (long)K * 2;
  #pragma unroll
  for (int u = 0; u < BCHUNK; ++u) {
    int d = (t + u * 512) * 16;
    int sl = C3_SWZ(d);
    long row = sl >> 6;
    srcB[u] = ((tile_n + row < Cout) ? (tile_n + row) : (Cout - 1)) * Kb
              + (sl & 63);
  }

  int t_rs = 0, t_s = 0, t_dh = 0, t_dw = 0, t_cin0 = 0;
  auto stage_tile = [&](int slot, int kt) {
    const int k0 = kt * C3_BK;
    const int dh = PAR ? (int)((tap_pack >> (t_rs * 8 + 4)) & 15) : t_dh;
    const int dw = PAR ? (int)((tap_pack >> (t_rs * 8)) & 15) : t_dw;
    const int cin0 = t_cin0;
    t_cin0 += C3_BK;
    if (t_cin0 == Cin) {
      t_cin0 = 0;
      ++t_rs;
      ++t_s;
      t_dw += fd;
      if (t_s == fw) {
        t_s = 0;
        t_dw = 0;
        t_dh += fd;
      }
    }
    __attribute__((address_space(3))) char* la = lds3 + slot * SLOT;
    __attribute__((address_space(3))) char* lb = la + ABYTES;
    #pragma unroll
    for (int u = 0; u < ACHUNK; ++u) {
      int ih = a_ohS[u] + dh, iw = a_owS[u] + dw;
      bool ok = a_n[u] >= 0 && ih >= 0 && iw >= 0;
      if (D > 1) {
        ok = ok && (ih % D == 0) && (iw % D == 0);
        ih /= D;
        iw /= D;
      }
      const char* src;
      if (ok && ih < H && iw < Wd) {
        long pix = a_pix[u] + (long)ih * Wd + iw;
        src = (const char*)X + (pix * (long)pixst + cin0) * 2 + a_col[u];
      } else {
        src = (const char*)guard + a_col[u];
      }
      c3_stage16(src, la + (t + u * 512) * 16);
    }
    const long kbyte = (long)k0 * 2;
    #pragma unroll
    for (int u = 0; u < BCHUNK; ++u)
      c3_stage16((const char*)W9 + srcB[u] + kbyte, lb + (t + u * 512) * 16);
  };

  f32x4 acc[MI][4];
  #pragma unroll
  for (int i = 0; i < MI; ++i)
    #pragma unroll
    for (int j = 0; j < 4; ++j) acc[i][j] = {0.f, 0.f, 0.f, 0.f};

  const int nkt = K / C3_BK;
  stage_tile(0, 0);
  if (1 < nkt) stage_tile(1, 1);
  if (2 < nkt) stage_tile(2, 2);

  const int frow = lane & 15;
  const int kslot = lane >> 4;
  constexpr int INFLIGHT = 2 * (ACHUNK + BCHUNK);

  for (int kt = 0; kt < nkt; ++kt) {
    if (kt + 2 < nkt)
      asm volatile("s_waitcnt vmcnt(%0)" ::"i"(INFLIGHT) : "memory");
    else
      asm volatile("s_waitcnt vmcnt(0)" ::: "memory");
    __builtin_amdgcn_sched_barrier(0);
    __syncthreads();
    if (kt + 3 < nkt) stage_tile((kt + 3) & 3, kt + 3);

    __attribute__((address_space(3))) char* la = lds3 + (kt & 3) * SLOT;
    __attribute__((address_space(3))) char* lb = la + ABYTES;

    bf16x8 afrag[MI], bfrag[4];
    #pragma unroll
    for (int nj = 0; nj < 4; ++nj) {
      int l = (wc * 64 + nj * 16 + frow) * 64 + kslot * 16;
      bfrag[nj] = *(__attribute__((address_space(3))) bf16x8*)(lb + C3_SWZ(l));
    }
    #pragma unroll
    for (int mi = 0; mi < MI; ++mi) {
      int l = (wr * MI * 16 + mi * 16 + frow) * 64 + kslot * 16;
      afrag[mi] = *(__attribute__((address_space(3))) bf16x8*)(la + C3_SWZ(l));
    }
    __builtin_amdgcn_s_setprio(1);
    #pragma unroll
    for (int mi = 0; mi < MI; ++mi)
      #pragma unroll
      for (int nj = 0; nj < 4; ++nj)
        acc[mi][nj] = __builtin_amdgcn_mfma_f32_16x16x32_bf16(
            afrag[mi], bfrag[nj], acc[mi][nj], 0, 0, 0);
    __builtin_amdgcn_s_setprio(0);
    __syncthreads();
  }

  const int ccol = lane & 15;
  const int crow0 = (lane >> 4) * 4;
  #pragma unroll
  for (int mi = 0; mi < MI; ++mi) {
    #pragma unroll
    for (int r = 0; r < 4; ++r) {
      long m = tile_m + wr * MI * 16 + mi * 16 + crow0 + r;
      if (m >= M) continue;
      if (PAR) {
        long n2 = m / ((long)OH * OW);
        long rem = m - n2 * (long)OH * OW;
        int oh = (int)(rem / OW), ow = (int)(rem - (long)(rem / OW) * OW);
        m = n2 * OHOWr + (long)(oh * 2 + oh0) * OWr + (ow * 2 + ow0);
      }
      #pragma unroll
      for (int nj = 0; nj < 4; ++nj) {
        long n = tile_n + wc * 64 + nj * 16 + ccol;
        if (n < Cout)
          C[m * Cout + n] = ACC
              ? (OT)((float)C[m * Cout + n] + acc[mi][nj][r])
              : (OT)acc[mi][nj][r];
      }
    }
  }
}

template <int D, bool ACC>
static void launch_conv(const void* X, const void* W9, const void* guard,
                        void* Y, int out_bf16, int N, int H, int W, int Cin,
                        int Cout, int OH, int OW, int S, int P, int taps,
                        int fw, int pixst, int fd, hipStream_t s) {
  const long M = (long)N * OH * OW;
  if (Cout >= 192) {
    int ntm = (int)((M + 255) / 256), ntn = (Cout + 255) / 256;
    dim3 grid(ntm * ntn);
    if (out_bf16)
      hipLaunchKernelGGL((conv3x3_kernel<bf16_t, 2, 4, 8, D, ACC>), grid,
                         dim3(512), 0, s, (const bf16_t*)X, (const bf16_t*)W9,
                         (const bf16_t*)guard, (bf16_t*)Y, N, H, W, Cin, Cout,
                         OH, OW, S, P, taps, fw, pixst, 0UL, 0, 0, OW, (long)OH * OW,
                         fd);
    else
      hipLaunchKernelGGL((conv3x3_kernel<float, 2, 4, 8, D, ACC>), grid,
                         dim3(512), 0, s, (const bf16_t*)X, (const bf16_t*)W9,
                         (const bf16_t*)guard, (float*)Y, N, H, W, Cin, Cout,
                         OH, OW, S, P, taps, fw, pixst, 0UL, 0, 0, OW, (long)OH * OW,
                         fd);
    return;
  }
  int ntm = (int)((M + 255) / 256), ntn = (Cout + 127) / 128;
  dim3 grid(ntm * ntn);
  if (out_bf16)
    hipLaunchKernelGGL((conv3x3_kernel<bf16_t, 4, 2, 4, D, ACC>), grid,
                       dim3(512), 0, s, (const bf16_t*)X, (const bf16_t*)W9,
                       (const bf16_t*)guard, (bf16_t*)Y, N, H, W, Cin, Cout,
                       OH, OW, S, P, taps, fw, pixst, 0UL, 0, 0, OW, (long)OH * OW,
                         fd);
  else
    hipLaunchKernelGGL((conv3x3_kernel<float, 4, 2, 4, D, ACC>), grid,
                       dim3(512), 0, s, (const bf16_t*)X, (const bf16_t*)W9,
                       (const bf16_t*)guard, (float*)Y, N, H, W, Cin, Cout,
                       OH, OW, S, P, taps, fw, pixst, 0UL, 0, 0, OW, (long)OH * OW,
                         fd);
}

extern "C" {

void tfosr_conv3x3(const void* X, const void* W9, const void* guard, void* Y,
                   int out_bf16, int N, int H, int W, int Cin, int Cout,
                   int OH, int OW, int S, int P, hipStream_t s) {
  launch_conv<1, false>(X, W9, guard, Y, out_bf16, N, H, W, Cin, Cout, OH, OW,
                        S, P, 9, 3, Cin, 1, s);
}

void tfosr_conv_mfma(const void* X, const void* W9, const void* guard, void* Y,
                     int out_bf16, int N, int H, int W, int Cin, int Cout,
                     int OH, int OW, int S, int P, int taps, int fw, int Dil,
                     int accum, int fd, hipStream_t s) {
  if (Dil == 2) {
    if (accum)
      launch_conv<2, true>(X, W9, guard, Y, out_bf16, N, H, W, Cin, Cout, OH,
                           OW, S, P, taps, fw, Cin, 1, s);
    else
      launch_conv<2, false>(X, W9, guard, Y, out_bf16, N, H, W, Cin, Cout, OH,
                            OW, S, P, taps, fw, Cin, 1, s);
  } else {
    if (accum)
      launch_conv<1, true>(X, W9, guard, Y, out_bf16, N, H, W, Cin, Cout, OH,
                           OW, S, P, taps, fw, Cin, 1, s);
    else
      launch_conv<1, false>(X, W9, guard, Y, out_bf16, N, H, W, Cin, Cout, OH,
                            OW, S, P, taps, fw, Cin, fd, s);
  }
}

void tfosr_conv_par(const void* X, const void* Wk, const void* guard, void* Y,
                    int N, int H, int W, int Cin, int Cout, int OHs, int OWs,
                    int P, int ntaps, unsigned long tap_pack, int oh0, int ow0,
                    int OWr, long OHOWr, int accum, hipStream_t s) {
  const long M = (long)N * OHs * OWs;
  if (Cout >= 192) {
    int ntm = (int)((M + 255) / 256), ntn = (Cout + 255) / 256;
    dim3 grid(ntm * ntn);
    if (accum)
      hipLaunchKernelGGL((conv3x3_kernel<bf16_t, 2, 4, 8, 2, true, true>),
                         grid, dim3(512), 0, s, (const bf16_t*)X,
                         (const bf16_t*)Wk, (const bf16_t*)guard, (bf16_t*)Y,
                         N, H, W, Cin, Cout, OHs, OWs, 1, P, ntaps, 1, Cin,
                         tap_pack, oh0, ow0, OWr, OHOWr, 1);
    else
      hipLaunchKernelGGL((conv3x3_kernel<bf16_t, 2, 4, 8, 2, false, true>),
                         grid, dim3(512), 0, s, (const bf16_t*)X,
                         (const bf16_t*)Wk, (const bf16_t*)guard, (bf16_t*)Y,
                         N, H, W, Cin, Cout, OHs, OWs, 1, P, ntaps, 1, Cin,
                         tap_pack, oh0, ow0, OWr, OHOWr, 1);
    return;
  }
  int ntm = (int)((M + 255) / 256), ntn = (Cout + 127) / 128;
  dim3 grid(ntm * ntn);
  if (accum)
    hipLaunchKernelGGL((conv3x3_kernel<bf16_t, 4, 2, 4, 2, true, true>), grid,
                       dim3(512), 0, s, (const bf16_t*)X, (const bf16_t*)Wk,
                       (const bf16_t*)guard, (bf16_t*)Y, N, H, W, Cin, Cout,
                       OHs, OWs, 1, P, ntaps, 1, Cin, tap_pack, oh0, ow0,
                       OWr, OHOWr, 1);
  else
    hipLaunchKernelGGL((conv3x3_kernel<bf16_t, 4, 2, 4, 2, false, true>), grid,
                       dim3(512), 0, s, (const bf16_t*)X, (const bf16_t*)Wk,
                       (const bf16_t*)guard, (bf16_t*)Y, N, H, W, Cin, Cout,
                       OHs, OWs, 1, P, ntaps, 1, Cin, tap_pack, oh0, ow0,
                       OWr, OHOWr, 1);
}

void tfosr_conv_stem(const void* X4, const void* W224, const void* guard,
                     void* Y, int N, int Hp, int Wp, int Cout, int OH, int OW,
                     hipStream_t s) {
  launch_conv<1, false>(X4, W224, guard, Y, 1, N, Hp, Wp, 32,
                        Cout, OH, OW, 2, 0, 7, 1, 4, 1, s);
}

}
```

csrc/gemm_mfma.hip:

```cpp
#include "tfosr_common.h"
#include <type_traits>
#include <cstdlib>
#include <cstring>

typedef short bf16x8 __attribute__((ext_vector_type(8)));
typedef float f32x4 __attribute__((ext_vector_type(4)));

#define BK 32
#define AS_LDS(T) __attribute__((address_space(3))) T
#define LDS_SWZ(l) ((l) ^ ((((l) >> 7) & 7) << 4))

__device__ __forceinline__ void stage16(const char* src,
                                        __attribute__((address_space(3))) char* dst) {
  __builtin_amdgcn_global_load_lds(
      (const __attribute__((address_space(1))) void*)src,
      (__attribute__((address_space(3))) void*)dst, 16, 0, 0);
}

template <typename OT, int WGM, int WGN, bool ACC = false>
__global__ __launch_bounds__(256, 2) void gemm_bt_kernel(
    const bf16_t* __restrict__ A, const bf16_t* __restrict__ B,
    OT* __restrict__ C, int M, int N, int K) {
  constexpr int BM = WGM * 64;
  constexpr int BN = WGN * 64;
  constexpr int ABYTES = BM * BK * 2;
  constexpr int BBYTES = BN * BK * 2;
  constexpr int ACHUNK = ABYTES / 16 / 256;
  constexpr int BCHUNK = BBYTES / 16 / 256;
  __shared__ char lds[2 * (ABYTES + BBYTES)];
  __attribute__((address_space(3))) char* lds3 =
      (__attribute__((address_space(3))) char*)lds;

  const int ntn = (N + BN - 1) / BN;
  const int nwg = gridDim.x;
  int wgid = blockIdx.x;
  {
    const int q = nwg / 8, r = nwg % 8;
    const int xcd = wgid % 8, pos = wgid / 8;
    wgid = (xcd < r ? xcd * (q + 1) : r * (q + 1) + (xcd - r) * q) + pos;
  }
  const long tile_m = (long)(wgid / ntn) * BM;
  const long tile_n = (long)(wgid % ntn) * BN;

  const int t = threadIdx.x;
  const int lane = t & 63;
  const int wave = t >> 6;
  const int wr = wave / WGN, wc = wave % WGN;

  long srcA[ACHUNK], srcB[BCHUNK];
  const long Kb = (long)K * 2;
  #pragma unroll
  for (int u = 0; u < ACHUNK; ++u) {
    int d = (t + u * 256) * 16;
    int sl = LDS_SWZ(d);
    long row = sl >> 6;
    srcA[u] = ((tile_m + row < M) ? (tile_m + row) : (M - 1)) * Kb + (sl & 63);
  }
  #pragma unroll
  for (int u = 0; u < BCHUNK; ++u) {
    int d = (t + u * 256) * 16;
    int sl = LDS_SWZ(d);
    long row = sl >> 6;
    srcB[u] = ((tile_n + row < N) ? (tile_n + row) : (N - 1)) * Kb + (sl & 63);
  }

  auto stage_tile = [&](int buf, int kt) {
    const long kbyte = (long)kt * BK * 2;
    __attribute__((address_space(3))) char* la = lds3 + buf * (ABYTES + BBYTES);
    __attribute__((address_space(3))) char* lb = la + ABYTES;
    #pragma unroll
    for (int u = 0; u < ACHUNK; ++u)
      stage16((const char*)A + srcA[u] + kbyte, la + (t + u * 256) * 16);
    #pragma unroll
    for (int u = 0; u < BCHUNK; ++u)
      stage16((const char*)B + srcB[u] + kbyte, lb + (t + u * 256) * 16);
  };

  f32x4 acc[4][4];
  #pragma unroll
  for (int i = 0; i < 4; ++i)
    #pragma unroll
    for (int j = 0; j < 4; ++j) acc[i][j] = {0.f, 0.f, 0.f, 0.f};

  const int nkt = K / BK;
  int cur = 0;
  stage_tile(0, 0);

  const int frow = lane & 15;
  const int kslot = lane >> 4;

  for (int kt = 0; kt < nkt; ++kt) {
    asm volatile("s_waitcnt vmcnt(0)" ::: "memory");
    __syncthreads();
    if (kt + 1 < nkt) stage_tile(cur ^ 1, kt + 1);

    __attribute__((address_space(3))) char* la = lds3 + cur * (ABYTES + BBYTES);
    __attribute__((address_space(3))) char* lb = la + ABYTES;

    bf16x8 afrag[4], bfrag[4];
    #pragma unroll
    for (int mi = 0; mi < 4; ++mi) {
      int l = (wr * 64 + mi * 16 + frow) * 64 + kslot * 16;
      afrag[mi] = *(__attribute__((address_space(3))) bf16x8*)(la + LDS_SWZ(l));
    }
    #pragma unroll
    for (int nj = 0; nj < 4; ++nj) {
      int l = (wc * 64 + nj * 16 + frow) * 64 + kslot * 16;
      bfrag[nj] = *(__attribute__((address_space(3))) bf16x8*)(lb + LDS_SWZ(l));
    }
    #pragma unroll
    for (int mi = 0; mi < 4; ++mi)
      #pragma unroll
      for (int nj = 0; nj < 4; ++nj)
        acc[mi][nj] = __builtin_amdgcn_mfma_f32_16x16x32_bf16(
            afrag[mi], bfrag[nj], acc[mi][nj], 0, 0, 0);

    cur ^= 1;
    __syncthreads();
  }

  const int ccol = lane & 15;
  const int crow0 = (lane >> 4) * 4;
  if constexpr (ACC && std::is_same<OT, bf16_t>::value) {
    __syncthreads();
    AS_LDS(char*) myl = lds3 + wave * 8192;
    #pragma unroll
    for (int mi = 0; mi < 4; ++mi)
      #pragma unroll
      for (int r = 0; r < 4; ++r)
        #pragma unroll
        for (int nj = 0; nj < 4; ++nj) {
          bf16_t v = (bf16_t)acc[mi][nj][r];
          short sv;
          __builtin_memcpy(&sv, &v, 2);
          *(AS_LDS(short*))(myl +
              ((mi * 16 + crow0 + r) * 64 + nj * 16 + ccol) * 2) = sv;
        }
    asm volatile("s_waitcnt lgkmcnt(0)" ::: "memory");
    typedef short s16x8 __attribute__((ext_vector_type(8)));
    #pragma unroll
    for (int i = 0; i < 8; ++i) {
      int c = i * 64 + lane;
      int row = c >> 3, col0 = (c & 7) * 8;
      long m = tile_m + wr * 64 + row;
      long n = tile_n + wc * 64 + col0;
      if (m >= M || n + 7 >= N) {
        if (m < M)
          for (int j = 0; j < 8 && n + j < N; ++j) {
            short sv = *(AS_LDS(short*))(myl + (row * 64 + col0 + j) * 2);
            bf16_t v;
            __builtin_memcpy(&v, &sv, 2);
            C[m * N + n + j] =
                (OT)((float)C[m * N + n + j] + (float)v);
          }
        continue;
      }
      s16x8 add = *(AS_LDS(s16x8*))(myl + (row * 64 + col0) * 2);
      s16x8 old = *(s16x8*)((char*)C + (m * N + n) * 2);
      s16x8 out;
      #pragma unroll
      for (int j = 0; j < 8; ++j) {
        short sa = add[j], sb = old[j];
        bf16_t a, b;
        __builtin_memcpy(&a, &sa, 2);
        __builtin_memcpy(&b, &sb, 2);
        bf16_t o = (bf16_t)((float)a + (float)b);
        short so;
        __builtin_memcpy(&so, &o, 2);
        out[j] = so;
      }
      *(s16x8*)((char*)C + (m * N + n) * 2) = out;
    }
    return;
  }
  #pragma unroll
  for (int mi = 0; mi < 4; ++mi) {
    #pragma unroll
    for (int r = 0; r < 4; ++r) {
      long m = tile_m + wr * 64 + mi * 16 + crow0 + r;
      if (m >= M) continue;
      #pragma unroll
      for (int nj = 0; nj < 4; ++nj) {
        long n = tile_n + wc * 64 + nj * 16 + ccol;
        if (n < N)
          C[m * N + n] = ACC ? (OT)((float)C[m * N + n] + acc[mi][nj][r])
                             : (OT)acc[mi][nj][r];
      }
    }
  }
}


#define B2_BM 256
#define B2_BN 256
#define B2_TILE_BYTES (B2_BM * BK * 2)
#define B2_SLOT (2 * B2_TILE_BYTES)

template <typename OT, bool ACC = false>
__global__ __launch_bounds__(512, 1) void gemm_bt256_kernel(
    const bf16_t* __restrict__ A, const bf16_t* __restrict__ B,
    OT* __restrict__ C, int M, int N, int K) {
  __shared__ char lds[4 * B2_SLOT];
  __attribute__((address_space(3))) char* lds3 =
      (__attribute__((address_space(3))) char*)lds;

  const int ntn = (N + B2_BN - 1) / B2_BN;
  const int nwg = gridDim.x;
  int wgid = blockIdx.x;
  {
    const int q = nwg / 8, r = nwg % 8;
    const int xcd = wgid % 8, pos = wgid / 8;
    wgid = (xcd < r ? xcd * (q + 1) : r * (q + 1) + (xcd - r) * q) + pos;
  }
  const long tile_m = (long)(wgid / ntn) * B2_BM;
  const long tile_n = (long)(wgid % ntn) * B2_BN;

  const int t = threadIdx.x;
  const int lane = t & 63;
  const int wave = t >> 6;
  const int wr = wave >> 2;
  const int wc = wave & 3;

  const long Kb = (long)K * 2;
  long srcA[2], srcB[2];
  #pragma unroll
  for (int u = 0; u < 2; ++u) {
    int d = (t + u * 512) * 16;
    int sl = LDS_SWZ(d);
    long row = sl >> 6;
    srcA[u] = ((tile_m + row < M) ? (tile_m + row) : (M - 1)) * Kb + (sl & 63);
    srcB[u] = ((tile_n + row < N) ? (tile_n + row) : (N - 1)) * Kb + (sl & 63);
  }

  auto stage_tile = [&](int slot, int kt) {
    const long kbyte = (long)kt * BK * 2;
    __attribute__((address_space(3))) char* la = lds3 + slot * B2_SLOT;
    __attribute__((address_space(3))) char* lb = la + B2_TILE_BYTES;
    #pragma unroll
    for (int u = 0; u < 2; ++u)
      stage16((const char*)A + srcA[u] + kbyte, la + (t + u * 512) * 16);
    #pragma unroll
    for (int u = 0; u < 2; ++u)
      stage16((const char*)B + srcB[u] + kbyte, lb + (t + u * 512) * 16);
  };

  f32x4 acc[8][4];
  #pragma unroll
  for (int i = 0; i < 8; ++i)
    #pragma unroll
    for (int j = 0; j < 4; ++j) acc[i][j] = {0.f, 0.f, 0.f, 0.f};

  const int nkt = K / BK;
  stage_tile(0, 0);
  if (1 < nkt) stage_tile(1, 1);
  if (2 < nkt) stage_tile(2, 2);

  const int frow = lane & 15;
  const int kslot = lane >> 4;

  for (int kt = 0; kt < nkt; ++kt) {
    if (kt + 2 < nkt)
      asm volatile("s_waitcnt vmcnt(8)" ::: "memory");
    else
      asm volatile("s_waitcnt vmcnt(0)" ::: "memory");
    __builtin_amdgcn_sched_barrier(0);
    __syncthreads();
    if (kt + 3 < nkt) stage_tile((kt + 3) & 3, kt + 3);

    __attribute__((address_space(3))) char* la = lds3 + (kt & 3) * B2_SLOT;
    __attribute__((address_space(3))) char* lb = la + B2_TILE_BYTES;

    bf16x8 afrag[8], bfrag[4];
    #pragma unroll
    for (int nj = 0; nj < 4; ++nj) {
      int l = (wc * 64 + nj * 16 + frow) * 64 + kslot * 16;
      bfrag[nj] = *(__attribute__((address_space(3))) bf16x8*)(lb + LDS_SWZ(l));
    }
    #pragma unroll
    for (int mi = 0; mi < 8; ++mi) {
      int l = (wr * 128 + mi * 16 + frow) * 64 + kslot * 16;
      afrag[mi] = *(__attribute__((address_space(3))) bf16x8*)(la + LDS_SWZ(l));
    }
    __builtin_amdgcn_s_setprio(1);
    #pragma unroll
    for (int mi = 0; mi < 8; ++mi)
      #pragma unroll
      for (int nj = 0; nj < 4; ++nj)
        acc[mi][nj] = __builtin_amdgcn_mfma_f32_16x16x32_bf16(
            afrag[mi], bfrag[nj], acc[mi][nj], 0, 0, 0);
    __builtin_amdgcn_s_setprio(0);
    __syncthreads();
  }

  const int ccol = lane & 15;
  const int crow0 = (lane >> 4) * 4;
  #pragma unroll
  for (int mi = 0; mi < 8; ++mi) {
    #pragma unroll
    for (int r = 0; r < 4; ++r) {
      long m = tile_m + wr * 128 + mi * 16 + crow0 + r;
      if (m >= M) continue;
      #pragma unroll
      for (int nj = 0; nj < 4; ++nj) {
        long n = tile_n + wc * 64 + nj * 16 + ccol;
        if (n < N)
          C[m * N + n] = ACC ? (OT)((float)C[m * N + n] + acc[mi][nj][r])
                             : (OT)acc[mi][nj][r];
      }
    }
  }
}

__global__ void mfma_probe_kernel(const short* __restrict__ a,
                                  const short* __restrict__ b,
                                  float* __restrict__ c) {
  int l = threadIdx.x;
  bf16x8 av = *(const bf16x8*)(a + l * 8);
  bf16x8 bv = *(const bf16x8*)(b + l * 8);
  f32x4 acc = {0.f, 0.f, 0.f, 0.f};
  acc = __builtin_amdgcn_mfma_f32_16x16x32_bf16(av, bv, acc, 0, 0, 0);
  #pragma unroll
  for (int r = 0; r < 4; ++r) c[l * 4 + r] = acc[r];
}

extern "C" {

void tfosr_gemm_bt_acc(const void*, const void*, void*, int, int, int, int,
                       int, hipStream_t);

void tfosr_gemm_bt(const void* A, const void* B, void* C, int out_bf16,
                   int M, int N, int K, hipStream_t s) {
  tfosr_gemm_bt_acc(A, B, C, out_bf16, M, N, K, 0, s);
}

void tfosr_gemm_bt_acc(const void* A, const void* B, void* C, int out_bf16,
                       int M, int N, int K, int accum, hipStream_t s) {
  static int use256 = -1;
  if (use256 < 0) {
    const char* e = getenv("TFOS_GEMM256");
    use256 = (e == nullptr || strcmp(e, "off") != 0) ? 1 : 0;
  }
  if (use256 && M >= 1024 && N >= 192 && K >= 1024) {
    int ntm = (M + B2_BM - 1) / B2_BM, ntn = (N + B2_BN - 1) / B2_BN;
    dim3 grid(ntm * ntn);
    if (out_bf16) {
      if (accum)
        hipLaunchKernelGGL((gemm_bt256_kernel<bf16_t, true>), grid, dim3(512),
                           0, s, (const bf16_t*)A, (const bf16_t*)B,
                           (bf16_t*)C, M, N, K);
      else
        hipLaunchKernelGGL((gemm_bt256_kernel<bf16_t, false>), grid, dim3(512),
                           0, s, (const bf16_t*)A, (const bf16_t*)B,
                           (bf16_t*)C, M, N, K);
    } else {
      hipLaunchKernelGGL((gemm_bt256_kernel<float, false>), grid, dim3(512), 0,
                         s, (const bf16_t*)A, (const bf16_t*)B, (float*)C, M,
                         N, K);
    }
    return;
  }
  const bool skinny = (N % 128 != 0) && (N % 64 == 0 || N <= 64);
  if (skinny) {
    int ntm = (M + 255) / 256, ntn = (N + 63) / 64;
    dim3 grid(ntm * ntn);
    if (out_bf16) {
      if (accum)
        hipLaunchKernelGGL((gemm_bt_kernel<bf16_t, 4, 1, true>), grid,
                           dim3(256), 0, s, (const bf16_t*)A,
                           (const bf16_t*)B, (bf16_t*)C, M, N, K);
      else
        hipLaunchKernelGGL((gemm_bt_kernel<bf16_t, 4, 1, false>), grid,
                           dim3(256), 0, s, (const bf16_t*)A,
                           (const bf16_t*)B, (bf16_t*)C, M, N, K);
    } else {
      hipLaunchKernelGGL((gemm_bt_kernel<float, 4, 1>), grid, dim3(256), 0, s,
                         (const bf16_t*)A, (const bf16_t*)B, (float*)C, M, N,
                         K);
    }
    return;
  }
  int ntm = (M + 127) / 128, ntn = (N + 127) / 128;
  dim3 grid(ntm * ntn);
  if (out_bf16) {
    if (accum)
      hipLaunchKernelGGL((gemm_bt_kernel<bf16_t, 2, 2, true>), grid, dim3(256),
                         0, s, (const bf16_t*)A, (const bf16_t*)B, (bf16_t*)C,
                         M, N, K);
    else
      hipLaunchKernelGGL((gemm_bt_kernel<bf16_t, 2, 2, false>), grid,
                         dim3(256), 0, s, (const bf16_t*)A, (const bf16_t*)B,
                         (bf16_t*)C, M, N, K);
  } else {
    hipLaunchKernelGGL((gemm_bt_kernel<float, 2, 2>), grid, dim3(256), 0, s,
                       (const bf16_t*)A, (const bf16_t*)B, (float*)C, M, N, K);
  }
}

void tfosr_mfma_probe(const short* a, const short* b, float* c, hipStream_t s) {
  hipLaunchKernelGGL(mfma_probe_kernel, dim3(1), dim3(64), 0, s, a, b, c);
}

}
```

tensorflowonspark_amd/ops/__init__.py:

```python

import glob
import logging
import os

import torch

logger = logging.getLogger(__name__)

API_VERSION = 6

_ext = None
_ext_checked = False


def _find_ext_path():
    here = os.path.dirname(os.path.abspath(__file__))
    for pat in ("tfosr_hip_ops*.so",):
        hits = glob.glob(os.path.join(here, pat))
        if hits:
            return hits[0]
    return None


def get_ext(required=False):
    global _ext, _ext_checked
    if not _ext_checked:
        _ext_checked = True
        path = _find_ext_path()
        if path is not None:
            try:
                import importlib.util
                spec = importlib.util.spec_from_file_location("tfosr_hip_ops", path)
                mod = importlib.util.module_from_spec(spec)
                spec.loader.exec_module(mod)
                got = mod.api_version() if hasattr(mod, "api_version") else 0
                if got != API_VERSION:
                    raise RuntimeError(
                        "tfosr_hip_ops.so is stale (api {} != {}): rebuild "
                        "with `python __graft_entry__.py`".format(
                            got, API_VERSION))
                _ext = mod
                logger.info("loaded HIP ops extension: %s", path)
            except Exception as e:
                logger.error("failed to load HIP ops extension %s: %s", path, e)
                _ext = None
    if required and _ext is None:
        if os.environ.get("TFOS_ALLOW_EAGER_FALLBACK"):
            return None
        raise RuntimeError(
            "tfosr_hip_ops extension not built but a CUDA tensor hit a fused op. "
            "Run __graft_entry__.build() (hipcc --offload-arch=gfx950) first, or "
            "set TFOS_ALLOW_EAGER_FALLBACK=1 to debug with eager PyTorch.")
    return _ext


def hip_available(x=None):
    if x is not None and not x.is_cuda:
        return False
    if not torch.cuda.is_available():
        return False
    return get_ext(required=True) is not None
```

tensorflowonspark_amd/ops/modules.py:

```python

import torch
import torch.nn as nn
import torch.nn.functional as F

from . import get_ext




def _use_wrw2(k, cin, cout):
    import os
    mode = os.environ.get("TFOS_WRW", "auto")
    if mode == "mfma2":
        return True
    if mode in ("miopen", "mfma"):
        return False
    return k == 3 and cin <= 64 and cout <= 64



class _FusedBNFn(torch.autograd.Function):

    @staticmethod
    def forward(ctx, x, res, weight, bias, running_mean, running_var,
# ... 602 lines not shown
    def forward(ctx, x, weight):
        Cout, Cin = weight.shape[0], weight.shape[1]
        wc = weight[:, :, 1, 1].contiguous().view(Cout, Cin, 1, 1)
        return _Conv1x1Fn.forward(ctx, x, wc)

    @staticmethod
    def backward(ctx, dy):
        dx, dwc = _Conv1x1Fn.backward(ctx, dy)
        dw = dwc.new_zeros(dwc.shape[0], dwc.shape[1], 3, 3)
        dw[:, :, 1, 1] = dwc[:, :, 0, 0]
        return dx, dw


class DilatedConv3x3(nn.Conv2d):

    def __init__(self, in_channels, out_channels, dilation=2, device=None,
                 dtype=None):
        if int(dilation) < 2:
            raise ValueError("DilatedConv3x3 needs dilation >= 2 "
                             "(use Conv3x3 for an undilated conv)")
        super().__init__(in_channels, out_channels, 3, stride=1,
                         padding=int(dilation), dilation=int(dilation),
                         bias=False, device=device, dtype=dtype)
        self._eligible = in_channels % 32 == 0 and out_channels % 32 == 0 \
            and out_channels >= 64

    def forward(self, x):
        if x.is_cuda and self._eligible and x.dtype == torch.bfloat16 \
                and x.dim() == 4:
            fd = self.dilation[0]
            route = _atrous_route(x.shape[0], x.shape[2], x.shape[3],
                                  self.in_channels, self.out_channels, fd)
            if route is not None and get_ext(required=True) is not None:
                x = x.contiguous(memory_format=torch.channels_last)
                collapse, fwd_in_tree, dgrad_in_tree = route
                if collapse:
                    return _AtrousCollapsedFn.apply(x, self.weight)
                return _AtrousConv3x3Fn.apply(x, self.weight, fd,
                                              fwd_in_tree, dgrad_in_tree)
        return super().forward(x)

    def __prepare_scriptable__(self):
        _SCRIPT_CLONE_KEEPALIVE.append(self)
        new = nn.Conv2d(self.in_channels, self.out_channels, 3, stride=1,
                        padding=self.padding, dilation=self.dilation,
                        bias=False)
        new.weight = self.weight
        new.train(self.training)
        return new




def _conv_parity_packed(x, packs, prefix, out, k, pp, accum=False):
    ext = get_ext(required=True)
    from .packplan import _class_taps
    for (ph, pw), (rl, sl) in _class_taps(k, pp).items():
        if not rl or not sl or ph >= out.shape[2] or pw >= out.shape[3]:
            continue
        wk = packs["{}_{}{}".format(prefix, ph, pw)]
        oc = wk.shape[-4] if wk.dim() == 4 else wk.shape[0]
        wk2 = wk.reshape(oc, -1)
        taps_r = [r for r in rl for _ in sl]
        taps_s = [s2 for _ in rl for s2 in sl]
        ext.conv_par(x, wk2, out, taps_r, taps_s, pp, accum)
    return out


def _conv_parity(x, wperm, out, k, pp, accum=False):
    ext = get_ext(required=True)
    OC = wperm.shape[0]
    KC = wperm.shape[3]
    for ph in (0, 1):
        for pw in (0, 1):
            taps = [(r, s) for r in range(k) for s in range(k)
                    if (ph - pp + r) % 2 == 0 and (pw - pp + s) % 2 == 0]
            if not taps or ph >= out.shape[2] or pw >= out.shape[3]:
                continue
            wk = torch.stack([wperm[:, r, s, :] for r, s in taps], dim=1) \
                .reshape(OC, len(taps) * KC).contiguous()
            ext.conv_par(x, wk, out,
                         [r for r, _ in taps], [s for _, s in taps],
                         pp, accum)
    return out



class _ConvT2dFn(torch.autograd.Function):

    @staticmethod
    def forward(ctx, x, weight, stride, padding, output_padding):
        ext = get_ext(required=True)
        Cin, Cout, KH, KW = weight.shape
        if x.dtype != torch.bfloat16:
            x = x.to(torch.bfloat16)
        wperm = weight.flip(2, 3).permute(1, 2, 3, 0) \
            .to(torch.bfloat16).contiguous()
        H, W = x.shape[2], x.shape[3]
        OH = (H - 1) * stride - 2 * padding + KH + output_padding
        OW = (W - 1) * stride - 2 * padding + KW + output_padding
        y = torch.empty(x.shape[0], Cout, OH, OW, device=x.device,
                        dtype=torch.bfloat16) \
            .contiguous(memory_format=torch.channels_last)
        if KH % 2 == 0 and output_padding == 0:
            _conv_parity(x, wperm, y, KH, KH - 1 - padding)
        else:
            y.zero_()
            _conv_parity(x, wperm, y, KH, KH - 1 - padding)
        ctx.save_for_backward(x, weight)
        ctx.params = (stride, padding)
        return y

    @staticmethod
    def backward(ctx, dy):
        ext = get_ext(required=True)
        x, weight = ctx.saved_tensors
        S, P = ctx.params
        Cin, Cout, KH, KW = weight.shape
        dy = dy.contiguous(memory_format=torch.channels_last)
        if dy.dtype != torch.bfloat16:
            dy = dy.to(torch.bfloat16)
        wd = weight.permute(0, 2, 3, 1).reshape(Cin, KH * KW * Cout)             .to(torch.bfloat16).contiguous()
        dx = ext.conv_mfma(dy, wd, Cin, KH, KW, S, P, 1,
                           x.shape[2], x.shape[3])
        w4 = weight.to(torch.bfloat16).contiguous(
            memory_format=torch.channels_last)
        _, dw, _ = torch.ops.aten.convolution_backward(
            dy, x, w4, None, [S, S], [P, P], [1, 1], True, [0, 0], 1,
            [False, True, False])
        return dx, dw.to(weight.dtype), None, None, None


class ConvTranspose2dMFMA(nn.Module):

    def __init__(self, cin, cout, kernel_size=4, stride=2, padding=1,
                 output_padding=0):
        super().__init__()
        self.stride, self.padding = stride, padding
        self.output_padding = output_padding
        self.weight = nn.Parameter(torch.empty(cin, cout, kernel_size,
                                               kernel_size))
        nn.init.kaiming_normal_(self.weight, mode="fan_in", nonlinearity="relu")
        self._eligible = cin % 32 == 0 and cout % 32 == 0 and stride == 2

    def forward(self, x):
        import os
        big = x.shape[0] * x.shape[2] * x.shape[3] * 4 >= 32768
        if x.is_cuda and self._eligible and big \
                and x.dtype == torch.bfloat16 \
                and os.environ.get("TFOS_CONVT", "mfma") == "mfma" \
                and get_ext(required=True) is not None:
            x = x.contiguous(memory_format=torch.channels_last)
            return _ConvT2dFn.apply(x, self.weight, self.stride, self.padding,
                                    self.output_padding)
        return F.conv_transpose2d(x, self.weight.to(x.dtype),
                                  stride=self.stride, padding=self.padding,
                                  output_padding=self.output_padding)

    def extra_repr(self):
        return "{}->{} k{} s{} p{} (implicit-GEMM MFMA)".format(
            self.weight.shape[0], self.weight.shape[1], self.weight.shape[2],
            self.stride, self.padding)



def gemm_bf16(a, b):
    if a.is_cuda:
        ext = get_ext(required=True)
        if ext is not None:
            return ext.gemm_bf16(a.contiguous(), b.contiguous())
    return (a.float() @ b.float())


class _GemmBTFn(torch.autograd.Function):

    @staticmethod
    def forward(ctx, a, b):
        ext = get_ext(required=True)
        a = a.to(torch.bfloat16).contiguous()
        b = b.to(torch.bfloat16).contiguous()
        ctx.save_for_backward(a, b)
        return ext.gemm_bt(a, b, True)

    @staticmethod
    def backward(ctx, dc):
        ext = get_ext(required=True)
        a, b = ctx.saved_tensors
        dc = dc.to(torch.bfloat16).contiguous()
        da = ext.gemm_bt(dc, b.t().contiguous(), True)
        db = (dc.float().t() @ a.float()).to(b.dtype)
        return da, db


class DenseMFMA(nn.Module):

    def __init__(self, in_features, out_features, bias=True):
        super().__init__()
        self.weight = nn.Parameter(torch.empty(out_features, in_features))
        self.bias = nn.Parameter(torch.zeros(out_features)) if bias else None
        nn.init.kaiming_uniform_(self.weight, a=5 ** 0.5)

    def forward(self, x):
        if x.is_cuda and x.dtype == torch.bfloat16 \
                and self.weight.shape[1] % 32 == 0 \
                and get_ext(required=True) is not None:
            y = _GemmBTFn.apply(x, self.weight)
            if self.bias is not None:
                y = y + self.bias.to(y.dtype)
            return y
        return F.linear(x, self.weight.to(x.dtype),
                        None if self.bias is None else self.bias.to(x.dtype))

    def __prepare_scriptable__(self):
        m = nn.Linear(self.weight.shape[1], self.weight.shape[0],
                      bias=self.bias is not None)
        m.weight = self.weight
        if self.bias is not None:
            m.bias = self.bias
        m.train(self.training)
        return m


class Conv2dIm2colMFMA(nn.Module):

    def __init__(self, cin, cout, kernel_size, bias=True):
        super().__init__()
        self.k = kernel_size
        self.weight = nn.Parameter(torch.empty(cout, cin, kernel_size,
                                               kernel_size))
        self.bias = nn.Parameter(torch.zeros(cout)) if bias else None
        nn.init.kaiming_uniform_(self.weight, a=5 ** 0.5)

    def forward(self, x):
        if x.is_cuda and x.dtype == torch.bfloat16 \
                and get_ext(required=True) is not None:
            N, Cin, H, W = x.shape
            Cout = self.weight.shape[0]
            OH, OW = H - self.k + 1, W - self.k + 1
            K = Cin * self.k * self.k
            Kpad = (K + 31) // 32 * 32
            cols = F.unfold(x, self.k)
            a = cols.transpose(1, 2).reshape(-1, K)
            a = F.pad(a, (0, Kpad - K))
            w2 = F.pad(self.weight.view(Cout, K), (0, Kpad - K))
            y2 = _GemmBTFn.apply(a, w2)
            if self.bias is not None:
                y2 = y2 + self.bias.to(y2.dtype)
            return y2.view(N, OH * OW, Cout).transpose(1, 2)                 .reshape(N, Cout, OH, OW)
        b = None if self.bias is None else self.bias.to(x.dtype)
        return F.conv2d(x, self.weight.to(x.dtype), b)

    def __prepare_scriptable__(self):
        m = nn.Conv2d(self.weight.shape[1], self.weight.shape[0], self.k,
                      bias=self.bias is not None)
        m.weight = self.weight
        if self.bias is not None:
            m.bias = self.bias
        m.train(self.training)
        return m


class BucketAdam:

    def __init__(self, engine, lr=1e-3, betas=(0.9, 0.999), eps=1e-8,
                 weight_decay=0.0, decoupled=False):
        self.engine = engine
        self.lr = lr
        self.b1, self.b2 = betas
        self.eps = eps
        self.weight_decay = weight_decay
        self.decoupled = decoupled
        self.step_count = 0
        self._m = [torch.zeros_like(b.buffer) for b in engine._buckets]
        self._v = [torch.zeros_like(b.buffer) for b in engine._buckets]

    @torch.no_grad()
    def step(self):
        self.step_count += 1
        for bucket, m, v in zip(self.engine._buckets, self._m, self._v):
            pf = bucket.param_flat
            g = bucket.buffer
            assert pf is not None, "BucketAdam requires flatten_params=True"
            ext = get_ext(required=True) if g.is_cuda else None
            if ext is not None:
                ext.adam_step(pf, g, m, v, self.lr, self.b1, self.b2, self.eps,
                              self.weight_decay, self.step_count, self.decoupled)
                continue
            grad = g if self.decoupled or not self.weight_decay \
                else g.add(pf, alpha=self.weight_decay)
            m.mul_(self.b1).add_(grad, alpha=1 - self.b1)
            v.mul_(self.b2).addcmul_(grad, grad, value=1 - self.b2)
            bc1 = 1 - self.b1 ** self.step_count
            bc2 = 1 - self.b2 ** self.step_count
            upd = (m / bc1) / ((v / bc2).sqrt() + self.eps)
            if self.decoupled and self.weight_decay:
                upd = upd + self.weight_decay * pf
            pf.add_(upd, alpha=-self.lr)

    def zero_grad(self):
        self.engine.zero_grad()



class _BottleneckFn(torch.autograd.Function):

    @staticmethod
    def forward(ctx, x, w1, g1, b1, rm1, rv1, w2, g2, b2, rm2, rv2,
                w3, g3, b3, rm3, rv3, wd, gd, bd, rmd, rvd,
                stride, momentum, eps, packs=None):
        ext = get_ext(required=True)
        N, Cin, H, W = x.shape
        C1, C2, C3 = w1.shape[0], w2.shape[0], w3.shape[0]

        def as2d(t):
            return t.permute(0, 2, 3, 1).reshape(-1, t.shape[1])

        def as4d(t2, h, w):
            return t2.view(N, h, w, -1).permute(0, 3, 1, 2)

        if packs is not None:
            w1b = packs["w1b"].reshape(C1, Cin)
            w9 = packs["w9"].reshape(C2, 9 * C1)
            w3b = packs["w3b"].reshape(C3, C2)
        else:
            w1b = w1.view(C1, Cin).to(torch.bfloat16).contiguous()
            w9 = w2.permute(0, 2, 3, 1).reshape(C2, 9 * C1) \
                .to(torch.bfloat16).contiguous()
            w3b = w3.view(C3, C2).to(torch.bfloat16).contiguous()
        t1 = as4d(ext.gemm_bt(as2d(x), w1b, True), H, W)
        a1, m1, r1, k1 = ext.bn_fwd_train(t1, None, g1, b1, rm1, rv1,
                                          momentum, eps, True)
        t2 = ext.conv_mfma(a1, w9, C2, 3, 3, stride, 1, 1, -1, -1)
        a2, m2, r2, k2 = ext.bn_fwd_train(t2, None, g2, b2, rm2, rv2,
                                          momentum, eps, True)
        OH, OW = t2.shape[2], t2.shape[3]
        t3 = as4d(ext.gemm_bt(as2d(a2), w3b, True), OH, OW)

        if wd is not None:
            wdb = packs["wdb"].reshape(C3, Cin) if packs is not None \
                else wd.view(C3, Cin).to(torch.bfloat16).contiguous()
            if stride == 1:
                td = as4d(ext.gemm_bt(as2d(x), wdb, True), H, W)
            else:
                td = ext.conv_mfma(x, wdb, C3, 1, 1, stride, 0, 1, -1, -1)
            import os
            dual = os.environ.get("TFOS_BN_DUAL", "on") != "off" \
                and ext.bn_dual_eligible(t3, td)
            if dual:
                y, m3, r3, md, rd, k3 = ext.bn_dual_fwd_train(
                    t3, td, g3, b3, rm3, rv3, gd, bd, rmd, rvd, momentum, eps)
                opt = [td, md, rd]
            else:
                idn, md, rd, _kd = ext.bn_fwd_train(td, None, gd, bd, rmd,
                                                    rvd, momentum, eps, False)
                opt = [td, idn, md, rd]
        else:
            dual = False
            idn = x
            opt = []
        if not dual:
            y, m3, r3, k3 = ext.bn_fwd_train(t3, idn, g3, b3, rm3, rv3,
                                             momentum, eps, True)

        ctx.save_for_backward(x, w1, g1, t1, a1, m1, r1, k1,
                              w2, g2, t2, a2, m2, r2, k2,
                              w3, g3, t3, m3, r3, k3, y, wd, gd, *opt)
        ctx.meta = (stride, wd is not None, dual)
        ctx.packs = packs
        return y

    @staticmethod
    def backward(ctx, dy):
        ext = get_ext(required=True)
        (x, w1, g1, t1, a1, m1, r1, k1, w2, g2, t2, a2, m2, r2, k2,
         w3, g3, t3, m3, r3, k3, y, wd, gd, *opt) = ctx.saved_tensors
        stride, has_down, dual = ctx.meta
        packs = ctx.packs
        N, Cin, H, W = x.shape
        C1, C2, C3 = w1.shape[0], w2.shape[0], w3.shape[0]
        OH, OW = t2.shape[2], t2.shape[3]
        dy = dy.contiguous(memory_format=torch.channels_last)
        if dy.dtype != torch.bfloat16:
            dy = dy.to(torch.bfloat16)

        def as2d(t):
            return t.permute(0, 2, 3, 1).reshape(-1, t.shape[1])

        def as4d(t2d, h, w):
            return t2d.view(N, h, w, -1).permute(0, 3, 1, 2)

        def cl(t):
            return t.contiguous(memory_format=torch.channels_last)

        if dual:
            td, md, rd = opt
            dt3, dtd, dg3, dgd, db3, dbd = ext.bn_dual_bwd(
                t3, td, dy, k3, g3, m3, r3, gd, md, rd)
        else:
            dt3, dg3, db3, dres = ext.bn_bwd(t3, dy, y, k3, g3, m3, r3,
                                             True, True)
        dt3 = cl(dt3)

        def lib_wrw(dyt, xt, w4, s_, p_):
            w4 = w4.to(torch.bfloat16).contiguous(
                memory_format=torch.channels_last)
            _, dw, _ = torch.ops.aten.convolution_backward(
                dyt, xt, w4, None, [s_, s_], [p_, p_], [1, 1], False, [0, 0],
                1, [False, True, False])
            return dw

        w3bT = packs["w3bT"].reshape(C2, C3) if packs is not None \
            else w3.view(C3, C2).to(torch.bfloat16).t().contiguous()
        da2 = cl(as4d(ext.gemm_bt(as2d(dt3), w3bT, True), OH, OW))
        dw3 = ext.conv_wrw2(dt3, a2, 1, 1, 1, 0).view(C3, C2, 1, 1) \
            if _use_wrw2(1, C2, C3) \
            else lib_wrw(dt3, a2, w3.view(C3, C2, 1, 1), 1, 0)

        dt2, dg2, db2 = ext.bn_bwd(t2, da2, a2, k2, g2, m2, r2, True, False)
        dt2 = cl(dt2)

        if stride == 2:
            da1 = torch.empty(N, C1, H, W, device=x.device,
                              dtype=torch.bfloat16) \
                .contiguous(memory_format=torch.channels_last)
            if packs is not None:
                _conv_parity_packed(dt2, packs, "w9p", da1, 3, 1)
            else:
                wperm2 = w2.flip(2, 3).permute(1, 2, 3, 0) \
                    .to(torch.bfloat16).contiguous()
                _conv_parity(dt2, wperm2, da1, 3, 1)
        else:
            w9p = packs["w9p"].reshape(C1, 9 * C2) if packs is not None \
                else w2.flip(2, 3).permute(1, 2, 3, 0).reshape(C1, 9 * C2) \
                .to(torch.bfloat16).contiguous()
            da1 = ext.conv_mfma(dt2, w9p, C1, 3, 3, 1, 1, 1, H, W)
        if _use_wrw2(3, C1, C2):
            dw9 = ext.conv_wrw2(dt2, a1, 3, 3, stride, 1)
            dw2 = dw9.view(C2, 3, 3, C1).permute(0, 3, 1, 2).contiguous()
        else:
            dw2 = lib_wrw(dt2, a1, w2, stride, 1)

        dt1, dg1, db1 = ext.bn_bwd(t1, da1, a1, k1, g1, m1, r1, True, False)
        dt1 = cl(dt1)

        dw1 = ext.conv_wrw2(dt1, x, 1, 1, 1, 0).view(C1, Cin, 1, 1) \
            if _use_wrw2(1, Cin, C1) \
            else lib_wrw(dt1, x, w1.view(C1, Cin, 1, 1), 1, 0)

        w1bT = packs["w1bT"].reshape(Cin, C1) if packs is not None \
            else w1.view(C1, Cin).to(torch.bfloat16).t().contiguous()
        if has_down:
            if not dual:
                td, idn, md, rd = opt
                dtd, dgd, dbd = ext.bn_bwd(td, dres, idn,
                                           torch.empty(0, dtype=torch.uint8,
                                                       device=td.device),
                                           gd, md, rd, False, False)
            dtd = cl(dtd)
            dwd = ext.conv_wrw2(dtd, x, 1, 1, stride, 0) \
                .view(C3, Cin, 1, 1) if _use_wrw2(1, Cin, C3) \
                else lib_wrw(dtd, x, wd.view(C3, Cin, 1, 1), stride, 0)
            dx2d = ext.gemm_bt(as2d(dt1), w1bT, True)
            dx = cl(as4d(dx2d, H, W))
            wdbT = packs["wdbT"].reshape(Cin, C3) if packs is not None \
                else wd.view(C3, Cin).to(torch.bfloat16).t().contiguous()
            if stride == 1:
                ext.gemm_bt_acc(as2d(dtd), wdbT, as2d(dx))
            else:
                ext.conv_par(dtd, wdbT, dx, [0], [0], 0, True)
            dwd = dwd.to(wd.dtype)
            dgd_, dbd_ = dgd, dbd
        else:
            dx = dres
            ext.gemm_bt_acc(as2d(dt1), w1bT, as2d(dx))
            dwd = dgd_ = dbd_ = None

        return (dx, dw1.to(w1.dtype), dg1, db1, None, None,
                dw2.to(w2.dtype), dg2, db2, None, None,
                dw3.to(w3.dtype), dg3, db3, None, None,
                dwd, dgd_, dbd_, None, None,
                None, None, None, None)



class _StemConvFn(torch.autograd.Function):

    @staticmethod
    def forward(ctx, x, weight, w224=None):
        ext = get_ext(required=True)
        N, _, H, W = x.shape
        Cout = weight.shape[0]
        x4 = torch.zeros(N, 4, H + 6, W + 6, dtype=torch.bfloat16,
                         device=x.device) \
            .contiguous(memory_format=torch.channels_last)
        x4[:, :3, 3:H + 3, 3:W + 3] = x
        if w224 is None:
            w224 = torch.zeros(Cout, 7, 8, 4, dtype=torch.bfloat16,
                               device=x.device)
            w224[:, :, :7, :3] = weight.permute(0, 2, 3, 1).to(torch.bfloat16)
        y = ext.conv_stem(x4, w224.reshape(Cout, 224).contiguous(), Cout)
        ctx.save_for_backward(x4, weight)
        return y

    @staticmethod
    def backward(ctx, dy):
        ext = get_ext(required=True)
        x4, weight = ctx.saved_tensors
        dy = dy.contiguous(memory_format=torch.channels_last)
        if dy.dtype != torch.bfloat16:
            dy = dy.to(torch.bfloat16)
        dw224 = ext.conv_stem_wrw(dy, x4)
        Cout = weight.shape[0]
        dw = dw224.view(Cout, 7, 8, 4)[:, :, :7, :3].permute(0, 3, 1, 2)
        return None, dw.contiguous().to(weight.dtype), None


class StemConv7x7(nn.Module):

    def __init__(self, cin=3, cout=64):
        super().__init__()
        assert cin == 3
        self.weight = nn.Parameter(torch.empty(cout, cin, 7, 7))
        nn.init.kaiming_normal_(self.weight, mode="fan_out",
                                nonlinearity="relu")

    def forward(self, x):
        import os
        if x.is_cuda and x.dtype == torch.bfloat16 and not x.requires_grad \
                and os.environ.get("TFOS_STEM", "mfma") == "mfma" \
                and get_ext(required=True) is not None:
            x = x.contiguous(memory_format=torch.channels_last)
            packs = getattr(self, "_tfos_packs", None)
            return _StemConvFn.apply(x, self.weight,
                                     packs["w224"] if packs else None)
        return F.conv2d(x, self.weight.to(x.dtype), stride=2, padding=3)

    def extra_repr(self):
        return "3->{} 7x7 s2 (NHWC4 implicit-GEMM MFMA)".format(
            self.weight.shape[0])



_SCRIPT_CLONE_KEEPALIVE = []


def _bn_clone(src):
    _SCRIPT_CLONE_KEEPALIVE.append(src)
    bn = nn.BatchNorm2d(src.num_features, eps=src.eps, momentum=src.momentum)
    with torch.no_grad():
        bn.weight.copy_(src.weight)
        bn.bias.copy_(src.bias)
        bn.running_mean.copy_(src.running_mean)
        bn.running_var.copy_(src.running_var)
        bn.num_batches_tracked.copy_(src.num_batches_tracked)
    bn.train(src.training)
    return bn


def _conv_clone(m):
    if isinstance(m, nn.Conv2d):
        return m
    _SCRIPT_CLONE_KEEPALIVE.append(m)
    k = m.weight.shape[2]
    stride = getattr(m, "stride", 1)
    if isinstance(m, StemConv7x7):
        stride, pad = 2, 3
    else:
        pad = 1 if k == 3 else 0
    new = nn.Conv2d(m.weight.shape[1], m.weight.shape[0], k, stride=stride,
                    padding=pad, bias=False)
    new.weight = m.weight
    new.train(m.training)
    return new


def _convT_clone(m):
    if isinstance(m, nn.ConvTranspose2d):
        return m
    _SCRIPT_CLONE_KEEPALIVE.append(m)
    new = nn.ConvTranspose2d(m.weight.shape[0], m.weight.shape[1],
                             m.weight.shape[2], stride=m.stride,
                             padding=m.padding,
                             output_padding=m.output_padding, bias=False)
    new.weight = m.weight
    new.train(m.training)
    return new


def _fusedbn_prepare(self):
    _SCRIPT_CLONE_KEEPALIVE.append(self)
    bn = _bn_clone(self)
    if self.RELU:
        out = nn.Sequential(bn, nn.ReLU(inplace=True))
        out.train(self.training)
        return out
    return bn


def _maxpool_prepare(self):
    _SCRIPT_CLONE_KEEPALIVE.append(self)
    return nn.MaxPool2d(self.k, self.s, self.p)


FusedMaxPool2d.__prepare_scriptable__ = _maxpool_prepare
FusedBNReLU.__prepare_scriptable__ = _fusedbn_prepare
FusedBN.__prepare_scriptable__ = _fusedbn_prepare
Conv1x1.__prepare_scriptable__ = lambda self: _conv_clone(self)
Conv3x3.__prepare_scriptable__ = lambda self: _conv_clone(self)
StemConv7x7.__prepare_scriptable__ = lambda self: _conv_clone(self)
ConvTranspose2dMFMA.__prepare_scriptable__ = lambda self: _convT_clone(self)
```

Before: 10130 images/sec.

## Fuse BN batch-statistics partial reductions into GEMM and conv MFMA epilogues

Adds epilogue variants of the bf16 GEMM and MFMA conv kernels that compute per-tile shifted mean/M2 partials for each output channel while the accumulators are still in registers. New BN entry points then combine these tile partials with a finalize kernel instead of re-reading the activation in a separate stats pass. The aim is to remove one full read of each large conv output per BN layer in the bottleneck forward. In exchange the GEMM/conv epilogues gain extra LDS use, a sync and shuffle reductions, and a size heuristic decides when to use them.

```diff
diff --git a/csrc/bindings.cpp b/csrc/bindings.cpp
--- a/csrc/bindings.cpp
+++ b/csrc/bindings.cpp
@@ -78,6 +78,16 @@
                     int, int, int, int, int, int, int, unsigned long, int,
                     int, int, long, int, hipStream_t);
 void tfosr_pack_bf16(const void*, const void*, int, void*, long, hipStream_t);
+int tfosr_gemm_bt_stats_rows(int, int, int);
+void tfosr_gemm_bt_stats(const void*, const void*, void*, float*, int, int, int,
+                         hipStream_t);
+void tfosr_conv_mfma_stats(const void*, const void*, const void*, void*, float*,
+                           int, int, int, int, int, int, int, int, int, int, int,
+                           int, hipStream_t);
+int tfosr_bn_tile_ws_rows(int);
+void tfosr_bn_tile_finalize(const float*, int, int, float*, float*, float*,
+                            float*, float*, long, int, float, float,
+                            hipStream_t);
 }
 
 namespace tfosr {
@@ -323,6 +333,160 @@
   tfosr_bn_apply_dual(xa.data_ptr(), xb.data_ptr(), y.data_ptr(),
                       mask.data_ptr<unsigned char>(), f(mean_a), f(rstd_a),
                       f(w_a), f(b_a), f(mean_b), f(rstd_b), f(w_b), f(b_b), bf,
+                      total, l.C, s);
+  return {y, mean_a, rstd_a, mean_b, rstd_b, mask};
+}
+
+
+void bn_check_pre(const at::Tensor& x, const BNLayout& l, const at::Tensor& part,
+                  long rows_per_tile, const char* name) {
+  TORCH_CHECK(x.scalar_type() == at::kBFloat16 && l.nhwc &&
+                  tfosr_bn_fast_blocks(x.numel(), l.C, 1, 1) > 0,
+              "bn_pre: needs a bfloat16 channels_last tensor on the NHWC fast "
+              "path");
+  TORCH_CHECK(part.device() == x.device(), "bn_pre: ", name, " must be on ",
+              x.device(), ", got ", part.device());
+  TORCH_CHECK(part.scalar_type() == at::kFloat, "bn_pre: ", name,
+              " must be float32");
+  TORCH_CHECK(part.is_contiguous(), "bn_pre: ", name, " must be contiguous");
+  TORCH_CHECK(rows_per_tile >= 16 && rows_per_tile <= 4096,
+              "bn_pre: bad rows_per_tile ", rows_per_tile);
+  const long M = (long)l.N * l.HW;
+  const long ntm = (M + rows_per_tile - 1) / rows_per_tile;
+  TORCH_CHECK(part.dim() == 3 && part.size(0) == ntm && part.size(1) == 2 &&
+                  part.size(2) == l.C,
+              "bn_pre: ", name, " must have shape [", ntm, ", 2, ", l.C,
+              "] for this input and rows_per_tile ", rows_per_tile);
+}
+
+void bn_tile_finalize(const at::Tensor& part, long rows_per_tile,
+                      const BNLayout& l, at::Tensor& mean, at::Tensor& rstd,
+                      at::Tensor& rm, at::Tensor& rv, double momentum,
+                      double eps, hipStream_t s) {
+  const int ntm = (int)part.size(0);
+  auto ws = at::empty({(long)tfosr_bn_tile_ws_rows(ntm) * 3 * l.C},
+                      part.options());
+  tfosr_bn_tile_finalize(part.data_ptr<float>(), ntm, (int)rows_per_tile,
+                         ws.data_ptr<float>(), mean.data_ptr<float>(),
+                         rstd.data_ptr<float>(), rm.data_ptr<float>(),
+                         rv.data_ptr<float>(), (long)l.N * l.HW, l.C,
+                         (float)momentum, (float)eps, s);
+}
+
+void bn_stats_pass(const at::Tensor& x, int bf, const BNLayout& l,
+                   at::Tensor& mean, at::Tensor& rstd, at::Tensor& rm,
+                   at::Tensor& rv, double momentum, double eps, hipStream_t s) {
+  const long M = (long)l.N * l.HW;
+  const int nb = tfosr_bn_fast_blocks(M * l.C, l.C, bf, 1);
+  TORCH_CHECK(nb > 0, "bn: shape is not on the NHWC fast path");
+  auto ws = at::empty({(long)nb * 2 * l.C}, x.options().dtype(at::kFloat));
+  tfosr_bn_stats(x.data_ptr(), bf, 1, ws.data_ptr<float>(), nb, l.N, l.C, l.HW,
+                 s);
+  tfosr_bn_finalize(ws.data_ptr<float>(), nb, x.data_ptr(), bf, 1, l.HW,
+                    mean.data_ptr<float>(), rstd.data_ptr<float>(),
+                    rm.data_ptr<float>(), rv.data_ptr<float>(), M, l.C,
+                    (float)momentum, (float)eps, s);
+}
+
+std::vector<at::Tensor> bn_fwd_train_pre(at::Tensor x,
+                                         c10::optional<at::Tensor> res,
+                                         at::Tensor part, long rows_per_tile,
+                                         at::Tensor w, at::Tensor b,
+                                         at::Tensor rm, at::Tensor rv,
+                                         double momentum, double eps,
+                                         bool relu) {
+  auto l = bn_layout(x);
+  dtype_flag(x);
+  bn_check_pre(x, l, part, rows_per_tile, "part");
+  const void* res_ptr = nullptr;
+  if (res.has_value()) {
+    bn_check_like(*res, x, true, true, "res");
+    res_ptr = res->data_ptr();
+  }
+  bn_check_channel_vec(w, x, l.C, "weight");
+  bn_check_channel_vec(b, x, l.C, "bias");
+  bn_check_channel_vec(rm, x, l.C, "running_mean");
+  bn_check_channel_vec(rv, x, l.C, "running_var");
+  auto opts = x.options().dtype(at::kFloat);
+  long total = (long)l.N * l.HW * l.C;
+  auto save_mean = at::empty({l.C}, opts);
+  auto save_rstd = at::empty({l.C}, opts);
+  auto y = at::empty_like(x);
+  at::Tensor mask = at::empty({relu ? total / 8 : 0},
+                              x.options().dtype(at::kByte));
+  auto s = cur_stream();
+  bn_tile_finalize(part, rows_per_tile, l, save_mean, save_rstd, rm, rv,
+                   momentum, eps, s);
+  tfosr_bn_apply(x.data_ptr(), res_ptr, y.data_ptr(),
+                 relu ? mask.data_ptr<unsigned char>() : nullptr,
+                 save_mean.data_ptr<float>(), save_rstd.data_ptr<float>(),
+                 w.data_ptr<float>(), b.data_ptr<float>(), 1, 1, relu, total,
+                 l.C, l.HW, s);
+  return {y, save_mean, save_rstd, mask};
+}
+
+std::vector<at::Tensor> bn_batch_stats(at::Tensor x,
+                                       c10::optional<at::Tensor> part,
+                                       long rows_per_tile, at::Tensor rm,
+                                       at::Tensor rv, double momentum,
+                                       double eps) {
+  auto l = bn_layout(x);
+  int bf = dtype_flag(x);
+  bn_check_channel_vec(rm, x, l.C, "running_mean");
+  bn_check_channel_vec(rv, x, l.C, "running_var");
+  auto opts = x.options().dtype(at::kFloat);
+  auto mean = at::empty({l.C}, opts), rstd = at::empty({l.C}, opts);
+  auto s = cur_stream();
+  if (part.has_value()) {
+    bn_check_pre(x, l, *part, rows_per_tile, "part");
+    bn_tile_finalize(*part, rows_per_tile, l, mean, rstd, rm, rv, momentum,
+                     eps, s);
+    return {mean, rstd};
+  }
+  TORCH_CHECK(l.nhwc, "bn_batch_stats: expects a channels_last tensor");
+  bn_stats_pass(x, bf, l, mean, rstd, rm, rv, momentum, eps, s);
+  return {mean, rstd};
+}
+
+std::vector<at::Tensor> bn_dual_fwd_train_pre(
+    at::Tensor xa, at::Tensor xb, c10::optional<at::Tensor> part_a,
+    long rows_a, c10::optional<at::Tensor> part_b, long rows_b,
+    at::Tensor w_a, at::Tensor b_a, at::Tensor rm_a, at::Tensor rv_a,
+    at::Tensor w_b, at::Tensor b_b, at::Tensor rm_b, at::Tensor rv_b,
+    double momentum, double eps) {
+  TORCH_CHECK(bn_dual_eligible(xa, xb),
+              "bn_dual: needs two same-shape channels_last GPU tensors on the "
+              "NHWC fast path");
+  auto l = bn_layout(xa);
+  TORCH_CHECK(xa.scalar_type() == at::kBFloat16,
+              "bn_pre: needs bfloat16 tensors");
+  if (part_a.has_value()) bn_check_pre(xa, l, *part_a, rows_a, "part_a");
+  if (part_b.has_value()) bn_check_pre(xb, l, *part_b, rows_b, "part_b");
+  const at::Tensor* vecs[] = {&w_a, &b_a, &rm_a, &rv_a, &w_b, &b_b, &rm_b, &rv_b};
+  for (auto* t : vecs) bn_check_channel_vec(*t, xa, l.C, "per-channel vector");
+  auto opts = xa.options().dtype(at::kFloat);
+  long M = (long)l.N * l.HW;
+  long total = M * l.C;
+  auto mean_a = at::empty({l.C}, opts), rstd_a = at::empty({l.C}, opts);
+  auto mean_b = at::empty({l.C}, opts), rstd_b = at::empty({l.C}, opts);
+  auto y = at::empty_like(xa);
+  auto mask = at::empty({total / 8}, xa.options().dtype(at::kByte));
+  auto s = cur_stream();
+  auto f = [](at::Tensor& t) { return t.data_ptr<float>(); };
+  auto stats = [&](at::Tensor& x, c10::optional<at::Tensor>& part, long rows,
+                   at::Tensor& mean, at::Tensor& rstd, at::Tensor& rm,
+                   at::Tensor& rv) {
+    if (part.has_value()) {
+      bn_tile_finalize(*part, rows, l, mean, rstd, rm, rv, momentum, eps, s);
+      return;
+    }
+    bn_stats_pass(x, 1, l, mean, rstd, rm, rv, momentum, eps, s);
+  };
+  stats(xa, part_a, rows_a, mean_a, rstd_a, rm_a, rv_a);
+  stats(xb, part_b, rows_b, mean_b, rstd_b, rm_b, rv_b);
+  tfosr_bn_apply_dual(xa.data_ptr(), xb.data_ptr(), y.data_ptr(),
+                      mask.data_ptr<unsigned char>(), f(mean_a), f(rstd_a),
+                      f(w_a), f(b_a), f(mean_b), f(rstd_b), f(w_b), f(b_b), 1,
                       total, l.C, s);
   return {y, mean_a, rstd_a, mean_b, rstd_b, mask};
 }
@@ -700,6 +864,33 @@
   return out;
 }
 
+py::tuple gemm_bt_stats(at::Tensor a, at::Tensor b) {
+  TORCH_CHECK(a.dim() == 2 && b.dim() == 2 && a.size(1) == b.size(1),
+              "gemm_bt_stats: A[M,K], B[N,K]");
+  TORCH_CHECK(a.is_cuda(), "gemm_bt_stats: a must be a GPU tensor");
+  TORCH_CHECK(b.device() == a.device(), "gemm_bt_stats: b must be on ",
+              a.device());
+  TORCH_CHECK(a.scalar_type() == at::kBFloat16 &&
+                  b.scalar_type() == at::kBFloat16,
+              "gemm_bt_stats: a and b must be bfloat16");
+  const long M = a.size(0), N = b.size(0), K = a.size(1);
+  TORCH_CHECK(M >= 1 && N >= 1 && K >= 1 && M <= INT_MAX && N <= INT_MAX &&
+                  K <= INT_MAX, "gemm_bt_stats: bad sizes");
+  const int rows = K % 32 == 0
+      ? tfosr_gemm_bt_stats_rows((int)M, (int)N, (int)K) : 0;
+  if (rows == 0)
+    return py::make_tuple(gemm_bt(a, b, true), py::none(), 0);
+  a = a.contiguous();
+  b = b.contiguous();
+  auto out = at::empty({M, N}, a.options());
+  auto part = at::empty({(M + rows - 1) / rows, 2, N},
+                        a.options().dtype(at::kFloat));
+  tfosr_gemm_bt_stats(a.data_ptr(), b.data_ptr(), out.data_ptr(),
+                      part.data_ptr<float>(), (int)M, (int)N, (int)K,
+                      cur_stream());
+  return py::make_tuple(out, part, rows);
+}
+
 at::Tensor gemm_bf16(at::Tensor a, at::Tensor b) {
   return gemm_bt(a, b.t().contiguous(), false);
 }
@@ -716,9 +907,63 @@
 
 }
 
-#define TFOSR_API_VERSION 6
+#define TFOSR_API_VERSION 7
 
 static constexpr long kMaxTapReach = 1L << 20;
+
+static std::pair<at::Tensor, c10::optional<at::Tensor>> conv_mfma_impl(
+    at::Tensor x, at::Tensor wk, long Cout, long fh, long fw, long S, long P,
+    long D, long OH, long OW, long fd, bool out_f32, bool stats) {
+  TORCH_CHECK(x.dim() == 4 && x.is_contiguous(at::MemoryFormat::ChannelsLast),
+              "conv_mfma expects channels_last input");
+  TORCH_CHECK(x.scalar_type() == at::kBFloat16 &&
+              wk.scalar_type() == at::kBFloat16);
+  TORCH_CHECK(fh >= 1 && fw >= 1 && fh * fw <= 49, "bad filter dims");
+  TORCH_CHECK(D == 1 || D == 2, "input dilation must be 1 or 2");
+  TORCH_CHECK(fd >= 1, "conv_mfma: filter dilation fd must be >= 1, got ",
+              fd);
+  TORCH_CHECK(fd == 1 || D == 1,
+              "conv_mfma: filter dilation fd > 1 requires input dilation "
+              "D == 1");
+  TORCH_CHECK(fd <= kMaxTapReach && fd * (fh - 1) <= kMaxTapReach &&
+                  fd * (fw - 1) <= kMaxTapReach,
+              "conv_mfma: fd, fd*(fh-1) and fd*(fw-1) must be <= ",
+              kMaxTapReach);
+  long taps = fh * fw;
+  int N = x.size(0), Cin = x.size(1), H = x.size(2), W = x.size(3);
+  TORCH_CHECK(Cin % 32 == 0, "conv_mfma requires Cin % 32 == 0");
+  TORCH_CHECK(wk.size(1) == taps * Cin);
+  if (OH < 0) {
+    long HV = (H - 1) * D + 1, WV = (W - 1) * D + 1;
+    long nh = HV + 2 * P - fd * (fh - 1) - 1;
+    long nw = WV + 2 * P - fd * (fw - 1) - 1;
+    TORCH_CHECK(nh >= 0 && nw >= 0,
+                "conv_mfma: the dilated filter does not fit the padded "
+                "input");
+    OH = nh / S + 1;
+    OW = nw / S + 1;
+  }
+  auto y = at::empty({N, Cout, OH, OW},
+                     x.options().dtype(out_f32 ? at::kFloat : at::kBFloat16),
+                     at::MemoryFormat::ChannelsLast);
+  auto guard = at::zeros({64}, x.options());
+  if (stats && D == 1 && !out_f32) {
+    TORCH_CHECK(x.is_cuda() && wk.device() == x.device(),
+                "conv_mfma_stats: x and wk must be on one GPU");
+    const long M = (long)N * OH * OW;
+    auto part = at::empty({(M + 255) / 256, 2, Cout},
+                          x.options().dtype(at::kFloat));
+    tfosr_conv_mfma_stats(x.data_ptr(), wk.contiguous().data_ptr(),
+                          guard.data_ptr(), y.data_ptr(),
+                          part.data_ptr<float>(), N, H, W, Cin, Cout, OH, OW, S,
+                          P, taps, fw, (int)fd, cur_stream());
+    return {y, part};
+  }
+  tfosr_conv_mfma(x.data_ptr(), wk.contiguous().data_ptr(), guard.data_ptr(),
+                  y.data_ptr(), out_f32 ? 0 : 1, N, H, W, Cin,
+                  Cout, OH, OW, S, P, taps, fw, D, 0, (int)fd, cur_stream());
+  return {y, c10::nullopt};
+}
 
 PYBIND11_MODULE(TORCH_EXTENSION_NAME, m) {
   m.def("api_version", []() { return TFOSR_API_VERSION; });
@@ -792,46 +1037,25 @@
   m.def("conv_mfma", [](at::Tensor x, at::Tensor wk, long Cout, long fh,
                         long fw, long S, long P, long D, long OH, long OW,
                         long fd, bool out_f32) {
-    TORCH_CHECK(x.dim() == 4 && x.is_contiguous(at::MemoryFormat::ChannelsLast),
-                "conv_mfma expects channels_last input");
-    TORCH_CHECK(x.scalar_type() == at::kBFloat16 &&
-                wk.scalar_type() == at::kBFloat16);
-    TORCH_CHECK(fh >= 1 && fw >= 1 && fh * fw <= 49, "bad filter dims");
-    TORCH_CHECK(D == 1 || D == 2, "input dilation must be 1 or 2");
-    TORCH_CHECK(fd >= 1, "conv_mfma: filter dilation fd must be >= 1, got ",
-                fd);
-    TORCH_CHECK(fd == 1 || D == 1,
-                "conv_mfma: filter dilation fd > 1 requires input dilation "
-                "D == 1");
-    TORCH_CHECK(fd <= kMaxTapReach && fd * (fh - 1) <= kMaxTapReach &&
-                    fd * (fw - 1) <= kMaxTapReach,
-                "conv_mfma: fd, fd*(fh-1) and fd*(fw-1) must be <= ",
-                kMaxTapReach);
-    long taps = fh * fw;
-    int N = x.size(0), Cin = x.size(1), H = x.size(2), W = x.size(3);
-    TORCH_CHECK(Cin % 32 == 0, "conv_mfma requires Cin % 32 == 0");
-    TORCH_CHECK(wk.size(1) == taps * Cin);
-    if (OH < 0) {
-      long HV = (H - 1) * D + 1, WV = (W - 1) * D + 1;
-      long nh = HV + 2 * P - fd * (fh - 1) - 1;
-      long nw = WV + 2 * P - fd * (fw - 1) - 1;
-      TORCH_CHECK(nh >= 0 && nw >= 0,
-                  "conv_mfma: the dilated filter does not fit the padded "
-                  "input");
-      OH = nh / S + 1;
-      OW = nw / S + 1;
-    }
-    auto y = at::empty({N, Cout, OH, OW},
-                       x.options().dtype(out_f32 ? at::kFloat : at::kBFloat16),
-                       at::MemoryFormat::ChannelsLast);
-    auto guard = at::zeros({64}, x.options());
-    tfosr_conv_mfma(x.data_ptr(), wk.contiguous().data_ptr(), guard.data_ptr(),
-                    y.data_ptr(), out_f32 ? 0 : 1, N, H, W, Cin,
-                    Cout, OH, OW, S, P, taps, fw, D, 0, (int)fd, cur_stream());
-    return y;
+    return conv_mfma_impl(x, wk, Cout, fh, fw, S, P, D, OH, OW, fd, out_f32,
+                          false).first;
   }, py::arg("x"), py::arg("wk"), py::arg("Cout"), py::arg("fh"),
      py::arg("fw"), py::arg("S"), py::arg("P"), py::arg("D"), py::arg("OH"),
      py::arg("OW"), py::arg("fd") = 1, py::arg("out_f32") = false);
+  m.def("conv_mfma_stats", [](at::Tensor x, at::Tensor wk, long Cout, long fh,
+                              long fw, long S, long P, long D, long OH,
+                              long OW, long fd, bool out_f32) {
+    auto r = conv_mfma_impl(x, wk, Cout, fh, fw, S, P, D, OH, OW, fd, out_f32,
+                            true);
+    if (!r.second.has_value()) return py::make_tuple(r.first, py::none(), 0);
+    return py::make_tuple(r.first, *r.second, 256);
+  }, py::arg("x"), py::arg("wk"), py::arg("Cout"), py::arg("fh"),
+     py::arg("fw"), py::arg("S"), py::arg("P"), py::arg("D"), py::arg("OH"),
+     py::arg("OW"), py::arg("fd") = 1, py::arg("out_f32") = false);
+  m.def("gemm_bt_stats", &gemm_bt_stats, py::arg("a"), py::arg("b"));
+  m.def("bn_fwd_train_pre", &bn_fwd_train_pre);
+  m.def("bn_dual_fwd_train_pre", &bn_dual_fwd_train_pre);
+  m.def("bn_batch_stats", &bn_batch_stats);
   m.def("conv_mfma_acc", [](at::Tensor x, at::Tensor wk, at::Tensor out,
                             long fh, long fw, long S, long P, long D) {
     TORCH_CHECK(x.is_contiguous(at::MemoryFormat::ChannelsLast) &&
diff --git a/csrc/bn_relu.hip b/csrc/bn_relu.hip
--- a/csrc/bn_relu.hip
+++ b/csrc/bn_relu.hip
@@ -120,6 +120,90 @@
   float dmean = s / (float)M;
   float var = fmaxf(q / (float)M - dmean * dmean, 0.f);
   float mean = shift + dmean;
+  save_mean[c] = mean;
+  save_rstd[c] = rsqrtf(var + eps);
+  if (running_mean != nullptr) {
+    float unbiased = (M > 1) ? var * (float)M / (float)(M - 1) : var;
+    running_mean[c] = (1.f - momentum) * running_mean[c] + momentum * mean;
+    running_var[c] = (1.f - momentum) * running_var[c] + momentum * unbiased;
+  }
+}
+
+#define TFOSR_TILE_MERGE_ROWS 256
+
+static inline int tile_merge_chunk(int ntm) {
+  int chunk = (ntm + TFOSR_TILE_MERGE_ROWS - 1) / TFOSR_TILE_MERGE_ROWS;
+  if (chunk < 32) chunk = 32;
+  return (chunk + 3) / 4 * 4;
+}
+
+__device__ __forceinline__ void tile_merge_lanes(float (&v)[3],
+                                                 float (*lds)[4][64], u32 tx,
+                                                 u32 ty) {
+  #pragma unroll
+  for (int j = 0; j < 3; ++j) lds[j][ty][tx] = v[j];
+  __syncthreads();
+  if (ty == 0) {
+    #pragma unroll
+    for (int j = 0; j < 3; ++j)
+      v[j] = (lds[j][0][tx] + lds[j][1][tx]) + (lds[j][2][tx] + lds[j][3][tx]);
+  }
+}
+
+__global__ void tile_stats_reduce(const float* __restrict__ part, int ntm, u32 C,
+                                  int rows_per_tile, long M, int chunk,
+                                  float* __restrict__ ws) {
+  __shared__ float lds[3][4][64];
+  const u32 tx = threadIdx.x & 63, ty = threadIdx.x >> 6;
+  const u32 c = blockIdx.x * 64 + tx;
+  const int r0 = blockIdx.y * chunk;
+  const int r1 = r0 + chunk < ntm ? r0 + chunk : ntm;
+  float v[3] = {0.f, 0.f, 0.f};
+  if (c < C) {
+    const float m0 = part[c];
+    for (int r = r0 + (int)ty; r < r1; r += 4) {
+      const float* p = part + (size_t)r * 2 * C;
+      const long rem = M - (long)r * rows_per_tile;
+      const float n = (float)(rem < rows_per_tile ? rem : rows_per_tile);
+      const float d = p[c] - m0;
+      v[0] += n * d;
+      v[1] += n * d * d;
+      v[2] += p[C + c];
+    }
+  }
+  tile_merge_lanes(v, lds, tx, ty);
+  if (ty == 0 && c < C) {
+    float* out = ws + (size_t)blockIdx.y * 3 * C;
+    out[c] = v[0];
+    out[C + c] = v[1];
+    out[2 * C + c] = v[2];
+  }
+}
+
+__global__ void tile_stats_finalize(const float* __restrict__ ws, int nrows,
+                                    u32 C, const float* __restrict__ part,
+                                    float* __restrict__ save_mean,
+                                    float* __restrict__ save_rstd,
+                                    float* __restrict__ running_mean,
+                                    float* __restrict__ running_var, long M,
+                                    float momentum, float eps) {
+  __shared__ float lds[3][4][64];
+  const u32 tx = threadIdx.x & 63, ty = threadIdx.x >> 6;
+  const u32 c = blockIdx.x * 64 + tx;
+  float v[3] = {0.f, 0.f, 0.f};
+  if (c < C) {
+    for (int r = (int)ty; r < nrows; r += 4) {
+      const float* p = ws + (size_t)r * 3 * C;
+      v[0] += p[c];
+      v[1] += p[C + c];
+      v[2] += p[2 * C + c];
+    }
+  }
+  tile_merge_lanes(v, lds, tx, ty);
+  if (ty != 0 || c >= C) return;
+  const float dmean = v[0] / (float)M;
+  const float var = fmaxf((v[2] + v[1]) / (float)M - dmean * dmean, 0.f);
+  const float mean = part[c] + dmean;
   save_mean[c] = mean;
   save_rstd[c] = rsqrtf(var + eps);
   if (running_mean != nullptr) {
@@ -612,6 +696,25 @@
                      running_mean, running_var, M, momentum, eps);
 }
 
+int tfosr_bn_tile_ws_rows(int ntm) {
+  const int chunk = tile_merge_chunk(ntm);
+  return (ntm + chunk - 1) / chunk;
+}
+
+void tfosr_bn_tile_finalize(const float* part, int ntm, int rows_per_tile,
+                            float* ws, float* save_mean, float* save_rstd,
+                            float* running_mean, float* running_var, long M,
+                            int C, float momentum, float eps, hipStream_t s) {
+  const int chunk = tile_merge_chunk(ntm);
+  const int nrows = (ntm + chunk - 1) / chunk;
+  const int cgroups = (C + 63) / 64;
+  hipLaunchKernelGGL(tile_stats_reduce, dim3(cgroups, nrows), dim3(256), 0, s,
+                     part, ntm, (u32)C, rows_per_tile, M, chunk, ws);
+  hipLaunchKernelGGL(tile_stats_finalize, dim3(cgroups), dim3(256), 0, s, ws,
+                     nrows, (u32)C, part, save_mean, save_rstd, running_mean,
+                     running_var, M, momentum, eps);
+}
+
 void tfosr_bn_apply(const void* x, const void* res, void* y, unsigned char* mask,
                     const float* mean,
                     const float* rstd, const float* w, const float* b,
diff --git a/csrc/conv3x3_mfma.hip b/csrc/conv3x3_mfma.hip
--- a/csrc/conv3x3_mfma.hip
+++ b/csrc/conv3x3_mfma.hip
@@ -1,4 +1,6 @@
 #include "tfosr_common.h"
+#include "mfma_stats_epilogue.h"
+#include <type_traits>
 
 typedef short bf16x8 __attribute__((ext_vector_type(8)));
 typedef float f32x4 __attribute__((ext_vector_type(4)));
@@ -14,13 +16,16 @@
 }
 
 template <typename OT, int WRG, int WCG, int MI, int D = 1, bool ACC = false,
-          bool PAR = false>
+          bool PAR = false, bool STATS = false>
 __global__ __launch_bounds__(512, 1) void conv3x3_kernel(
     const bf16_t* __restrict__ X, const bf16_t* __restrict__ W9,
     const bf16_t* __restrict__ guard, OT* __restrict__ C,
     int Nn, int H, int Wd, int Cin, int Cout, int OH, int OW, int S, int P,
     int taps, int fw, int pixst, unsigned long tap_pack, int oh0, int ow0,
-    int OWr, long OHOWr, int fd) {
+    int OWr, long OHOWr, int fd, float* __restrict__ part) {
+  static_assert(!STATS || (D == 1 && !ACC && !PAR &&
+                           std::is_same<OT, bf16_t>::value),
+                "the statistics epilogue exists for the plain bf16 forward");
   constexpr int BM = WRG * MI * 16;
   constexpr int BN = WCG * 64;
   constexpr int ABYTES = BM * C3_BK * 2;
@@ -199,45 +204,54 @@
       }
     }
   }
-}
-
-template <int D, bool ACC>
+  if constexpr (STATS) {
+    static_assert(TFOSR_TILE_STATS_LDS_FLOATS(WRG, BN) * 4 <= sizeof(lds), "");
+    mfma_tile_stats<MI, WRG, BN>(acc, (float*)lds, wr, wc, lane, t, tile_m,
+                                 tile_n, M, Cout,
+                                 part + (tile_m / BM) * 2 * (long)Cout);
+  }
+}
+
+template <int D, bool ACC, bool STATS = false>
 static void launch_conv(const void* X, const void* W9, const void* guard,
                         void* Y, int out_bf16, int N, int H, int W, int Cin,
                         int Cout, int OH, int OW, int S, int P, int taps,
-                        int fw, int pixst, int fd, hipStream_t s) {
+                        int fw, int pixst, int fd, hipStream_t s,
+                        float* part = nullptr) {
   const long M = (long)N * OH * OW;
   if (Cout >= 192) {
     int ntm = (int)((M + 255) / 256), ntn = (Cout + 255) / 256;
     dim3 grid(ntm * ntn);
     if (out_bf16)
-      hipLaunchKernelGGL((conv3x3_kernel<bf16_t, 2, 4, 8, D, ACC>), grid,
+      hipLaunchKernelGGL((conv3x3_kernel<bf16_t, 2, 4, 8, D, ACC, false, STATS>),
+                         grid,
                          dim3(512), 0, s, (const bf16_t*)X, (const bf16_t*)W9,
                          (const bf16_t*)guard, (bf16_t*)Y, N, H, W, Cin, Cout,
                          OH, OW, S, P, taps, fw, pixst, 0UL, 0, 0, OW, (long)OH * OW,
-                         fd);
+                         fd, part);
     else
       hipLaunchKernelGGL((conv3x3_kernel<float, 2, 4, 8, D, ACC>), grid,
                          dim3(512), 0, s, (const bf16_t*)X, (const bf16_t*)W9,
                          (const bf16_t*)guard, (float*)Y, N, H, W, Cin, Cout,
                          OH, OW, S, P, taps, fw, pixst, 0UL, 0, 0, OW, (long)OH * OW,
-                         fd);
+                         fd, (float*)nullptr);
     return;
   }
   int ntm = (int)((M + 255) / 256), ntn = (Cout + 127) / 128;
   dim3 grid(ntm * ntn);
   if (out_bf16)
-    hipLaunchKernelGGL((conv3x3_kernel<bf16_t, 4, 2, 4, D, ACC>), grid,
+    hipLaunchKernelGGL((conv3x3_kernel<bf16_t, 4, 2, 4, D, ACC, false, STATS>),
+                       grid,
                        dim3(512), 0, s, (const bf16_t*)X, (const bf16_t*)W9,
                        (const bf16_t*)guard, (bf16_t*)Y, N, H, W, Cin, Cout,
                        OH, OW, S, P, taps, fw, pixst, 0UL, 0, 0, OW, (long)OH * OW,
-                         fd);
+                         fd, part);
   else
     hipLaunchKernelGGL((conv3x3_kernel<float, 4, 2, 4, D, ACC>), grid,
                        dim3(512), 0, s, (const bf16_t*)X, (const bf16_t*)W9,
                        (const bf16_t*)guard, (float*)Y, N, H, W, Cin, Cout,
                        OH, OW, S, P, taps, fw, pixst, 0UL, 0, 0, OW, (long)OH * OW,
-                         fd);
+                         fd, (float*)nullptr);
 }
 
 extern "C" {
@@ -268,6 +282,14 @@
       launch_conv<1, false>(X, W9, guard, Y, out_bf16, N, H, W, Cin, Cout, OH,
                             OW, S, P, taps, fw, Cin, fd, s);
   }
+}
+
+void tfosr_conv_mfma_stats(const void* X, const void* W9, const void* guard,
+                           void* Y, float* part, int N, int H, int W, int Cin,
+                           int Cout, int OH, int OW, int S, int P, int taps,
+                           int fw, int fd, hipStream_t s) {
+  launch_conv<1, false, true>(X, W9, guard, Y, 1, N, H, W, Cin,
+                              Cout, OH, OW, S, P, taps, fw, Cin, fd, s, part);
 }
 
 void tfosr_conv_par(const void* X, const void* Wk, const void* guard, void* Y,
@@ -283,13 +305,13 @@
                          grid, dim3(512), 0, s, (const bf16_t*)X,
                          (const bf16_t*)Wk, (const bf16_t*)guard, (bf16_t*)Y,
                          N, H, W, Cin, Cout, OHs, OWs, 1, P, ntaps, 1, Cin,
-                         tap_pack, oh0, ow0, OWr, OHOWr, 1);
+                         tap_pack, oh0, ow0, OWr, OHOWr, 1, (float*)nullptr);
     else
       hipLaunchKernelGGL((conv3x3_kernel<bf16_t, 2, 4, 8, 2, false, true>),
                          grid, dim3(512), 0, s, (const bf16_t*)X,
                          (const bf16_t*)Wk, (const bf16_t*)guard, (bf16_t*)Y,
                          N, H, W, Cin, Cout, OHs, OWs, 1, P, ntaps, 1, Cin,
-                         tap_pack, oh0, ow0, OWr, OHOWr, 1);
+                         tap_pack, oh0, ow0, OWr, OHOWr, 1, (float*)nullptr);
     return;
   }
   int ntm = (int)((M + 255) / 256), ntn = (Cout + 127) / 128;
@@ -299,13 +321,13 @@
                        dim3(512), 0, s, (const bf16_t*)X, (const bf16_t*)Wk,
                        (const bf16_t*)guard, (bf16_t*)Y, N, H, W, Cin, Cout,
                        OHs, OWs, 1, P, ntaps, 1, Cin, tap_pack, oh0, ow0,
-                       OWr, OHOWr, 1);
+                       OWr, OHOWr, 1, (float*)nullptr);
   else
     hipLaunchKernelGGL((conv3x3_kernel<bf16_t, 4, 2, 4, 2, false, true>), grid,
                        dim3(512), 0, s, (const bf16_t*)X, (const bf16_t*)Wk,
                        (const bf16_t*)guard, (bf16_t*)Y, N, H, W, Cin, Cout,
                        OHs, OWs, 1, P, ntaps, 1, Cin, tap_pack, oh0, ow0,
-                       OWr, OHOWr, 1);
+                       OWr, OHOWr, 1, (float*)nullptr);
 }
 
 void tfosr_conv_stem(const void* X4, const void* W224, const void* guard,
diff --git a/csrc/gemm_mfma.hip b/csrc/gemm_mfma.hip
--- a/csrc/gemm_mfma.hip
+++ b/csrc/gemm_mfma.hip
@@ -1,4 +1,5 @@
 #include "tfosr_common.h"
+#include "mfma_stats_epilogue.h"
 #include <type_traits>
 #include <cstdlib>
 #include <cstring>
@@ -17,10 +18,12 @@
       (__attribute__((address_space(3))) void*)dst, 16, 0, 0);
 }
 
-template <typename OT, int WGM, int WGN, bool ACC = false>
+template <typename OT, int WGM, int WGN, bool ACC = false, bool STATS = false>
 __global__ __launch_bounds__(256, 2) void gemm_bt_kernel(
     const bf16_t* __restrict__ A, const bf16_t* __restrict__ B,
-    OT* __restrict__ C, int M, int N, int K) {
+    OT* __restrict__ C, int M, int N, int K, float* __restrict__ part) {
+  static_assert(!STATS || (!ACC && std::is_same<OT, bf16_t>::value),
+                "the statistics epilogue exists for plain bf16 stores only");
   constexpr int BM = WGM * 64;
   constexpr int BN = WGN * 64;
   constexpr int ABYTES = BM * BK * 2;
@@ -188,6 +191,12 @@
       }
     }
   }
+  if constexpr (STATS) {
+    static_assert(TFOSR_TILE_STATS_LDS_FLOATS(WGM, BN) * 4 <= sizeof(lds), "");
+    mfma_tile_stats<4, WGM, BN>(acc, (float*)lds, wr, wc, lane, t, tile_m,
+                                tile_n, (long)M, N,
+                                part + (tile_m / BM) * 2 * (long)N);
+  }
 }
 
 
@@ -323,24 +332,52 @@
   for (int r = 0; r < 4; ++r) c[l * 4 + r] = acc[r];
 }
 
-extern "C" {
-
-void tfosr_gemm_bt_acc(const void*, const void*, void*, int, int, int, int,
-                       int, hipStream_t);
-
-void tfosr_gemm_bt(const void* A, const void* B, void* C, int out_bf16,
-                   int M, int N, int K, hipStream_t s) {
-  tfosr_gemm_bt_acc(A, B, C, out_bf16, M, N, K, 0, s);
-}
-
-void tfosr_gemm_bt_acc(const void* A, const void* B, void* C, int out_bf16,
-                       int M, int N, int K, int accum, hipStream_t s) {
+static bool gemm_route256(int M, int N, int K) {
   static int use256 = -1;
   if (use256 < 0) {
     const char* e = getenv("TFOS_GEMM256");
     use256 = (e == nullptr || strcmp(e, "off") != 0) ? 1 : 0;
   }
-  if (use256 && M >= 1024 && N >= 192 && K >= 1024) {
+  return use256 && M >= 1024 && N >= 192 && K >= 1024;
+}
+
+static bool gemm_route_skinny(int N) {
+  return (N % 128 != 0) && (N % 64 == 0 || N <= 64);
+}
+
+extern "C" {
+
+void tfosr_gemm_bt_acc(const void*, const void*, void*, int, int, int, int,
+                       int, hipStream_t);
+
+int tfosr_gemm_bt_stats_rows(int M, int N, int K) {
+  if (gemm_route256(M, N, K)) return 0;
+  return gemm_route_skinny(N) ? 256 : 128;
+}
+
+void tfosr_gemm_bt_stats(const void* A, const void* B, void* C, float* part,
+                         int M, int N, int K, hipStream_t s) {
+  if (gemm_route_skinny(N)) {
+    dim3 grid(((M + 255) / 256) * ((N + 63) / 64));
+    hipLaunchKernelGGL((gemm_bt_kernel<bf16_t, 4, 1, false, true>), grid,
+                       dim3(256), 0, s, (const bf16_t*)A, (const bf16_t*)B,
+                       (bf16_t*)C, M, N, K, part);
+    return;
+  }
+  dim3 grid(((M + 127) / 128) * ((N + 127) / 128));
+  hipLaunchKernelGGL((gemm_bt_kernel<bf16_t, 2, 2, false, true>), grid,
+                     dim3(256), 0, s, (const bf16_t*)A, (const bf16_t*)B,
+                     (bf16_t*)C, M, N, K, part);
+}
+
+void tfosr_gemm_bt(const void* A, const void* B, void* C, int out_bf16,
+                   int M, int N, int K, hipStream_t s) {
+  tfosr_gemm_bt_acc(A, B, C, out_bf16, M, N, K, 0, s);
+}
+
+void tfosr_gemm_bt_acc(const void* A, const void* B, void* C, int out_bf16,
+                       int M, int N, int K, int accum, hipStream_t s) {
+  if (gemm_route256(M, N, K)) {
     int ntm = (M + B2_BM - 1) / B2_BM, ntn = (N + B2_BN - 1) / B2_BN;
     dim3 grid(ntm * ntn);
     if (out_bf16) {
@@ -359,23 +396,22 @@
     }
     return;
   }
-  const bool skinny = (N % 128 != 0) && (N % 64 == 0 || N <= 64);
-  if (skinny) {
+  if (gemm_route_skinny(N)) {
     int ntm = (M + 255) / 256, ntn = (N + 63) / 64;
     dim3 grid(ntm * ntn);
     if (out_bf16) {
       if (accum)
         hipLaunchKernelGGL((gemm_bt_kernel<bf16_t, 4, 1, true>), grid,
                            dim3(256), 0, s, (const bf16_t*)A,
-                           (const bf16_t*)B, (bf16_t*)C, M, N, K);
+                           (const bf16_t*)B, (bf16_t*)C, M, N, K, nullptr);
       else
         hipLaunchKernelGGL((gemm_bt_kernel<bf16_t, 4, 1, false>), grid,
                            dim3(256), 0, s, (const bf16_t*)A,
-                           (const bf16_t*)B, (bf16_t*)C, M, N, K);
+                           (const bf16_t*)B, (bf16_t*)C, M, N, K, nullptr);
     } else {
       hipLaunchKernelGGL((gemm_bt_kernel<float, 4, 1>), grid, dim3(256), 0, s,
                          (const bf16_t*)A, (const bf16_t*)B, (float*)C, M, N,
-                         K);
+                         K, nullptr);
     }
     return;
   }
@@ -385,14 +421,14 @@
     if (accum)
       hipLaunchKernelGGL((gemm_bt_kernel<bf16_t, 2, 2, true>), grid, dim3(256),
                          0, s, (const bf16_t*)A, (const bf16_t*)B, (bf16_t*)C,
-                         M, N, K);
+                         M, N, K, nullptr);
     else
       hipLaunchKernelGGL((gemm_bt_kernel<bf16_t, 2, 2, false>), grid,
                          dim3(256), 0, s, (const bf16_t*)A, (const bf16_t*)B,
-                         (bf16_t*)C, M, N, K);
+                         (bf16_t*)C, M, N, K, nullptr);
   } else {
     hipLaunchKernelGGL((gemm_bt_kernel<float, 2, 2>), grid, dim3(256), 0, s,
-                       (const bf16_t*)A, (const bf16_t*)B, (float*)C, M, N, K);
+                       (const bf16_t*)A, (const bf16_t*)B, (float*)C, M, N, K, nullptr);
   }
 }
 
diff --git a/csrc/mfma_stats_epilogue.h b/csrc/mfma_stats_epilogue.h
--- /dev/null
+++ b/csrc/mfma_stats_epilogue.h
@@ -0,0 +1,82 @@
+#pragma once
+#include "tfosr_common.h"
+
+typedef float msf32x4 __attribute__((ext_vector_type(4)));
+
+#define TFOSR_TILE_STATS_LDS_FLOATS(WSTACK, BN) ((WSTACK) * 3 * (BN))
+
+template <int MI, int WSTACK, int BN>
+__device__ __forceinline__ void mfma_tile_stats(
+    const msf32x4 (&acc)[MI][4], float* lf, int wr, int wc, int lane, int t,
+    long tile_m, long tile_n, long M, int N, float* __restrict__ part_row) {
+  constexpr int WM = MI * 16;
+  const int ccol = lane & 15;
+  const long lrow0 = tile_m + (long)wr * WM + (lane >> 4) * 4;
+  float k[4], s[4], q[4];
+  #pragma unroll
+  for (int nj = 0; nj < 4; ++nj) {
+    k[nj] = __shfl((float)(bf16_t)acc[0][nj][0], ccol, 64);
+    s[nj] = 0.f;
+    q[nj] = 0.f;
+  }
+  #pragma unroll
+  for (int mi = 0; mi < MI; ++mi) {
+    float s4[4] = {0.f, 0.f, 0.f, 0.f}, q4[4] = {0.f, 0.f, 0.f, 0.f};
+    #pragma unroll
+    for (int r = 0; r < 4; ++r) {
+      const bool ok = lrow0 + mi * 16 + r < M;
+      #pragma unroll
+      for (int nj = 0; nj < 4; ++nj) {
+        float d = (float)(bf16_t)acc[mi][nj][r] - k[nj];
+        d = ok ? d : 0.f;
+        s4[nj] += d;
+        q4[nj] += d * d;
+      }
+    }
+    #pragma unroll
+    for (int nj = 0; nj < 4; ++nj) { s[nj] += s4[nj]; q[nj] += q4[nj]; }
+  }
+  #pragma unroll
+  for (int nj = 0; nj < 4; ++nj) {
+    s[nj] += __shfl_xor(s[nj], 16, 64);
+    q[nj] += __shfl_xor(q[nj], 16, 64);
+    s[nj] += __shfl_xor(s[nj], 32, 64);
+    q[nj] += __shfl_xor(q[nj], 32, 64);
+  }
+  if (lane < 16) {
+    #pragma unroll
+    for (int nj = 0; nj < 4; ++nj) {
+      const int col = wc * 64 + nj * 16 + ccol;
+      lf[(wr * 3 + 0) * BN + col] = k[nj];
+      lf[(wr * 3 + 1) * BN + col] = s[nj];
+      lf[(wr * 3 + 2) * BN + col] = q[nj];
+    }
+  }
+  __syncthreads();
+  if (t < BN && tile_n + t < N) {
+    float n = 0.f, mean = 0.f, m2 = 0.f;
+    #pragma unroll
+    for (int w = 0; w < WSTACK; ++w) {
+      const long rem = M - (tile_m + (long)w * WM);
+      if (rem <= 0) break;
+      const float nw = (float)(rem < WM ? rem : WM);
+      const float kw = lf[(w * 3 + 0) * BN + t];
+      const float sw = lf[(w * 3 + 1) * BN + t];
+      const float qw = lf[(w * 3 + 2) * BN + t];
+      const float dm = sw / nw;
+      const float mean_w = kw + dm;
+      const float m2_w = fmaxf(qw - sw * dm, 0.f);
+      if (w == 0) {
+        n = nw; mean = mean_w; m2 = m2_w;
+      } else {
+        const float delta = mean_w - mean;
+        const float nn = n + nw;
+        mean += delta * (nw / nn);
+        m2 += m2_w + delta * delta * (n * nw / nn);
+        n = nn;
+      }
+    }
+    part_row[tile_n + t] = mean;
+    part_row[(long)N + tile_n + t] = m2;
+  }
+}
diff --git a/tensorflowonspark_amd/ops/__init__.py b/tensorflowonspark_amd/ops/__init__.py
--- a/tensorflowonspark_amd/ops/__init__.py
+++ b/tensorflowonspark_amd/ops/__init__.py
@@ -7,7 +7,7 @@
 
 logger = logging.getLogger(__name__)
 
-API_VERSION = 6
+API_VERSION = 7
 
 _ext = None
 _ext_checked = False
diff --git a/tensorflowonspark_amd/ops/modules.py b/tensorflowonspark_amd/ops/modules.py
--- a/tensorflowonspark_amd/ops/modules.py
+++ b/tensorflowonspark_amd/ops/modules.py
@@ -928,6 +928,32 @@
 
 
 
+def _bn_epi_mode():
+    import os
+    mode = os.environ.get("TFOS_BN_EPI", "auto")
+    if mode not in ("auto", "off", "force"):
+        raise ValueError("TFOS_BN_EPI must be auto, off or force, got "
+                         + repr(mode))
+    return mode
+
+
+_BN_EPI_MIN_BYTES = 1024 * 512 * 7 * 7 * 2
+
+
+def _bn_epi_auto(kind, M, K, cout):
+    if M * cout * 2 < _BN_EPI_MIN_BYTES:
+        return False
+    return kind == "gemm" or cout >= 192
+
+
+def _bn_epi_route(mode, kind, M, K, cout, ext=None):
+    if mode == "off":
+        return False
+    if ext is not None and ext.bn_fast_blocks(M * cout, cout, True, True) <= 0:
+        return False
+    return mode == "force" or _bn_epi_auto(kind, M, K, cout)
+
+
 class _BottleneckFn(torch.autograd.Function):
 
     @staticmethod
@@ -953,40 +979,67 @@
             w9 = w2.permute(0, 2, 3, 1).reshape(C2, 9 * C1) \
                 .to(torch.bfloat16).contiguous()
             w3b = w3.view(C3, C2).to(torch.bfloat16).contiguous()
-        t1 = as4d(ext.gemm_bt(as2d(x), w1b, True), H, W)
-        a1, m1, r1, k1 = ext.bn_fwd_train(t1, None, g1, b1, rm1, rv1,
-                                          momentum, eps, True)
-        t2 = ext.conv_mfma(a1, w9, C2, 3, 3, stride, 1, 1, -1, -1)
-        a2, m2, r2, k2 = ext.bn_fwd_train(t2, None, g2, b2, rm2, rv2,
-                                          momentum, eps, True)
-        OH, OW = t2.shape[2], t2.shape[3]
-        t3 = as4d(ext.gemm_bt(as2d(a2), w3b, True), OH, OW)
+        epi = _bn_epi_mode()
+
+        def gemm(a2d, wb):
+            if _bn_epi_route(epi, "gemm", a2d.shape[0], wb.shape[1],
+                             wb.shape[0], ext):
+                return ext.gemm_bt_stats(a2d, wb)
+            return ext.gemm_bt(a2d, wb, True), None, 0
+
+        def conv(a, wk, cout, k, s, p, m_out):
+            if _bn_epi_route(epi, "conv", m_out, k * k * a.shape[1], cout,
+                             ext):
+                return ext.conv_mfma_stats(a, wk, cout, k, k, s, p, 1, -1, -1)
+            return ext.conv_mfma(a, wk, cout, k, k, s, p, 1, -1, -1), None, 0
+
+        def bn(t, res, part, rows, g, b, rm, rv, relu):
+            if part is not None:
+                return ext.bn_fwd_train_pre(t, res, part, rows, g, b, rm, rv,
+                                            momentum, eps, relu)
+            return ext.bn_fwd_train(t, res, g, b, rm, rv, momentum, eps, relu)
+
+        OH, OW = (H - 1) // stride + 1, (W - 1) // stride + 1
+        t1, p1, n1 = gemm(as2d(x), w1b)
+        t1 = as4d(t1, H, W)
+        a1, m1, r1, k1 = bn(t1, None, p1, n1, g1, b1, rm1, rv1, True)
+        t2, p2, n2 = conv(a1, w9, C2, 3, stride, 1, N * OH * OW)
+        a2, m2, r2, k2 = bn(t2, None, p2, n2, g2, b2, rm2, rv2, True)
+        assert (OH, OW) == (t2.shape[2], t2.shape[3])
+        t3, p3, n3 = gemm(as2d(a2), w3b)
+        t3 = as4d(t3, OH, OW)
 
         if wd is not None:
             wdb = packs["wdb"].reshape(C3, Cin) if packs is not None \
                 else wd.view(C3, Cin).to(torch.bfloat16).contiguous()
             if stride == 1:
-                td = as4d(ext.gemm_bt(as2d(x), wdb, True), H, W)
+                td, pd, nd = gemm(as2d(x), wdb)
+                td = as4d(td, H, W)
             else:
-                td = ext.conv_mfma(x, wdb, C3, 1, 1, stride, 0, 1, -1, -1)
+                td, pd, nd = conv(x, wdb, C3, 1, stride, 0, N * OH * OW)
             import os
             dual = os.environ.get("TFOS_BN_DUAL", "on") != "off" \
                 and ext.bn_dual_eligible(t3, td)
             if dual:
-                y, m3, r3, md, rd, k3 = ext.bn_dual_fwd_train(
-                    t3, td, g3, b3, rm3, rv3, gd, bd, rmd, rvd, momentum, eps)
+                if p3 is not None or pd is not None:
+                    y, m3, r3, md, rd, k3 = ext.bn_dual_fwd_train_pre(
+                        t3, td, p3, n3, pd, nd, g3, b3, rm3, rv3, gd, bd,
+                        rmd, rvd, momentum, eps)
+                else:
+                    y, m3, r3, md, rd, k3 = ext.bn_dual_fwd_train(
+                        t3, td, g3, b3, rm3, rv3, gd, bd, rmd, rvd, momentum,
+                        eps)
                 opt = [td, md, rd]
             else:
-                idn, md, rd, _kd = ext.bn_fwd_train(td, None, gd, bd, rmd,
-                                                    rvd, momentum, eps, False)
+                idn, md, rd, _kd = bn(td, None, pd, nd, gd, bd, rmd, rvd,
+                                      False)
                 opt = [td, idn, md, rd]
         else:
             dual = False
             idn = x
             opt = []
         if not dual:
-            y, m3, r3, k3 = ext.bn_fwd_train(t3, idn, g3, b3, rm3, rv3,
-                                             momentum, eps, True)
+            y, m3, r3, k3 = bn(t3, idn, p3, n3, g3, b3, rm3, rv3, True)
 
         ctx.save_for_backward(x, w1, g1, t1, a1, m1, r1, k1,
                               w2, g2, t2, a2, m2, r2, k2,
```

Result: faster. 10350 images/sec, median of 6 (+2.2%).
